# anhtu293/nndepth

Measured on AMD Instinct MI355X. Metric: stereo pairs/sec at 544x960, 32 iters (RAFT-Stereo), higher is better.
Workload: dtype f32 carried as 2 range-scaled fp16 pieces per operand (3 MFMA products, fp32 accumulate); 1 GPU; RAFT-Stereo base (ctx 64), 544x960, 32 iters, batch 1 per GPU, all 32 up_disp emitted; parallelism=single, launch=direct

## Files before the change

include/nndepth_amd.h:

```cpp
#ifndef NNDEPTH_AMD_H
#define NNDEPTH_AMD_H

#include <stddef.h>
#include <stdint.h>

#ifdef __cplusplus
extern "C" {
#endif

#define NND_VERSION 105

#define NND_FLAG_CALIBRATE 1
#define NND_FLAG_LAST_UPSAMPLE_ONLY 2

typedef enum {
    NND_OK = 0,
    NND_ERR_INVALID = -1,
    NND_ERR_HIP = -2,
    NND_ERR_UNSUPPORTED = -3,
    NND_ERR_NO_DEVICE = -4
} nnd_status;

int nnd_version(void);
const char* nnd_last_error(void);
// ... 187 lines not shown
                     void* stream);

int nnd_mbv3_depthwise(const float* x, const float* w, const float* bias, float* y, double* partial, int N, int C, int H, int W, int k,
                       int stride, int act, void* stream);
int64_t nnd_mbv3_se_partials(int N, int C, int H, int W);
int nnd_mbv3_se(float* y, const double* partial, const float* wr, const float* br, const float* we, const float* be, float* gate, int N,
                int C, int rd, int H, int W, void* stream);
int nnd_mbv3_stem(const float* x, const float* x1, int nsplit, const float* w, const float* bias, float* y, int N, int H, int W,
                  void* stream);
int64_t nnd_mbv3_pointwise_packed_floats(int Cout, int Cin, int k);
int nnd_mbv3_pointwise_pack(int Cout, int Cin, int k, const float* w, const float* bias, float* packed_host);
int nnd_mbv3_proj(const float* x, const float* w, const float* bias, float* y, int N, int Cin, int Cout, int H, int W, void* stream);
int nnd_mbv3_pointwise(int Cout, int Cin, int k, const float* packed_dev, const float* x, const float* residual, float* y, int N, int H,
                       int W, int act, void* stream);

#define NND_MIDAS_KEEP_PRE 1
typedef struct nnd_midas_desc {
    int32_t struct_size;
    int32_t feature_channels;
    int32_t flags;
} nnd_midas_desc;
int nnd_midas_num_tensors(const nnd_midas_desc* desc);
int64_t nnd_midas_packed_floats(const nnd_midas_desc* desc);
int64_t nnd_midas_workspace_floats(const nnd_midas_desc* desc, int B, int H, int W);
int64_t nnd_midas_workspace_offset(const nnd_midas_desc* desc, int which, int B, int H, int W);
int nnd_midas_pack(const nnd_midas_desc* desc, const float* const* tensors_host, float* packed_host);
int nnd_midas_forward(const nnd_midas_desc* desc, const float* packed_dev, const float* x, float* depth, float* workspace, int B, int H,
                      int W, void* stream);
int64_t nnd_midas_up2x_pw_packed_floats(int Cout, int Cin);
int nnd_midas_up2x_pw_pack(int Cout, int Cin, const float* w, const float* bias, float* packed_host);
int nnd_midas_up2x_pw(int Cout, int Cin, const float* packed_dev, const float* x, float* y, int N, int h, int w, void* stream);
int64_t nnd_midas_head_packed_floats(int C);
int nnd_midas_head_pack(int C, const float* w2, const float* b2, const float* w4, const float* b4, float* packed_host);
int nnd_midas_head(int C, const float* packed_dev, const float* t, float* depth, float* pre_relu, int N, int h, int w, void* stream);
int nnd_midas_conv_add(int Cout, int Cin, int k, const float* packed_dev, const float* x, const float* feat, float* y, int N, int H, int W,
                       void* stream);

int nnd_resize_normalize(const void* src, int src_is_u8_hwc, float* dst, int B, int C, int h, int w, int H, int W,
                         float sub, float div, void* stream);
int nnd_replicate_pad(const float* src, float* dst, int B, int C, int H, int W, int left, int right, int top, int bottom,
                      void* stream);

int64_t nnd_depth_eval_workspace_bytes(int B);
int nnd_depth_eval(const float* pred, const float* gt, const unsigned char* valid_mask, int B, int H, int W, float max_depth,
                   void* workspace, int64_t workspace_bytes, double* out, void* stream);
int nnd_depth_eval_accumulate(const double* metrics, double* sums, double* counts, void* stream);

int64_t nnd_midas_loss_workspace_bytes(int B, int H, int W);
int nnd_midas_loss(const float* pred, const float* target, const unsigned char* valid_mask, int B, int H, int W, int64_t pred_stride_b,
                   int64_t pred_stride_row, double trimmed_coef, double gradient_coef, void* workspace, int64_t workspace_bytes,
                   double* out, void* stream);
int nnd_midas_loss_accumulate(const double* values, double* sums, double* count, void* stream);

#define NND_STEREO_EVAL_MAX_OUTPUTS 64
#define NND_STEREO_EVAL_MAX_THRESHOLDS 8
typedef struct nnd_stereo_eval_output {
    const float* data;
    int32_t C, h, w;
    int32_t reserved;
    int64_t stride_b, stride_c, stride_row;
} nnd_stereo_eval_output;
typedef struct nnd_stereo_eval_desc {
    int32_t struct_size;
    int32_t flags;
    const float* gt;
    int32_t B, Cg, H, W;
    const unsigned char* mask;
    int32_t mask_h, mask_w;
    double gamma;
    float max_flow;
    int32_t n_above;
    float above[NND_STEREO_EVAL_MAX_THRESHOLDS];
    int32_t n_below;
    float below[NND_STEREO_EVAL_MAX_THRESHOLDS];
    int32_t num_outputs;
    nnd_stereo_eval_output outputs[NND_STEREO_EVAL_MAX_OUTPUTS];
} nnd_stereo_eval_desc;
int64_t nnd_stereo_eval_workspace_bytes(int num_outputs);
int nnd_stereo_eval(const nnd_stereo_eval_desc* desc, void* workspace, int64_t workspace_bytes, double* out, void* stream);
int nnd_stereo_eval_accumulate(const double* metrics, int n, double* sums, void* stream);
int nnd_min_pool_nearest(const float* gt, float* dst, int B, int C, int H, int W, int h, int w, void* stream);

int64_t nnd_view_range_workspace_bytes(int B);
int nnd_view_range(const float* data, const unsigned char* mask, int kind, int B, int C, int H, int W, void* workspace, float* range,
                   void* stream);
int nnd_colorize(const float* data, const unsigned char* mask, int kind, int B, int C, int H, int W, const float* range, int has_lo,
                 double lo, int has_hi, double hi, int reverse, const unsigned char* table, int N, unsigned char* out, void* stream);
int nnd_pool_abs(const float* src, float* dst, int64_t* indices, const unsigned char* mask, unsigned char* mask_out,
                 unsigned char* finite_out, int B, int C, int H, int W, int kh, int kw, int is_min, int negate, int rescale, float mul,
                 float div, void* stream);
int nnd_resize_bilinear(const void* src, int src_is_u8, float* dst, unsigned char* u8_out, int u8_mode, unsigned char* finite_out,
                        int planes, int h, int w, int H, int W, int align_corners, int rescale, float mul, float div, void* stream);
int nnd_depth_inverse(const float* src, float* dst, int64_t n, float eps, int has_max, float clip_max, int has_min, float clip_min,
                      void* stream);

int nnd_disparity_to_depth(const float* disp, int64_t disp_bstride, const unsigned char* mask_in, const float* cam, int cam_stride,
                           double baseline, int negative, float min_disp, int has_max, float max_depth, float* depth,
                           unsigned char* valid_out, int B, int H, int W, void* stream);
int nnd_depth_to_disparity(const float* depth, int64_t depth_bstride, const float* cam, int cam_stride, double baseline, int negative,
                           double eps, float* disp, int B, int H, int W, void* stream);
int nnd_depth_to_points(const float* depth, int64_t depth_bstride, const unsigned char* valid, const float* cam, int cam_stride,
                        float* points, int B, int H, int W, void* stream);
int64_t nnd_points_compact_workspace_bytes(int B, int H, int W);
int nnd_points_compact(const float* depth, int64_t depth_bstride, const unsigned char* valid, const float* cam, int cam_stride,
                       const float* features, int C, float* points, float* feats_out, int64_t* offsets, void* workspace,
                       int64_t workspace_bytes, int B, int H, int W, void* stream);
int nnd_lr_consistency(const float* disp_left, int64_t left_bstride, const float* disp_right, int64_t right_bstride, int left_negative,
                       int right_negative, int right_flipped, float threshold, unsigned char* occluded, float* err_out, int B, int H,
                       int W, void* stream);
int nnd_pair_both_views(const float* left, const float* right, float* frames1, float* frames2, int B, int C, int H, int W,
                        void* stream);

int64_t nnd_loftr_packed_floats(int d_model, int nhead);
int64_t nnd_loftr_workspace_floats(int d_model, int nhead, int N, int H, int W);
int nnd_loftr_pack(int d_model, int nhead, const float* const* tensors_host, float* packed_host);
int nnd_loftr_layer_forward(int d_model, int nhead, const float* packed_dev, const float* x, const float* source, float* out,
                            float* workspace, int N, int H, int W, void* stream);

int nnd_full_attention(const float* q, const float* k, const float* v, float* out, int N, int nhead, int L, int S, int64_t q_bs,
                       int64_t kv_bs, int64_t out_bs, void* stream);
int64_t nnd_loftr_full_workspace_floats(int d_model, int nhead, int N, int H, int W);
int nnd_loftr_full_layer_forward(int d_model, int nhead, const float* packed_dev, const float* x, const float* source, float* out,
                                 float* workspace, int N, int H, int W, void* stream);

typedef struct nnd_conv3d_desc {
    int32_t struct_size;
    int32_t Cout, Cin0, Cin1, stride;
    int32_t arithmetic;
    int32_t flags;
} nnd_conv3d_desc;
int64_t nnd_conv3d_packed_floats(const nnd_conv3d_desc* desc);
int nnd_conv3d_pack(const nnd_conv3d_desc* desc, const float* w_host, const float* bias_host, const float* bn_gamma,
                    const float* bn_beta, const float* bn_mean, const float* bn_var, float bn_eps, float* packed_host);
int nnd_conv3d_forward(const nnd_conv3d_desc* desc, const float* packed_dev, const float* x0, const float* x1, float* y,
                       int N, int D, int H, int W, float leaky_slope, void* stream);
int nnd_conv3d_calibration_finish(const nnd_conv3d_desc* desc, float* packed_dev, int32_t* status_dev, void* stream);
int nnd_conv3d_scale_slots(const nnd_conv3d_desc* desc, int64_t* offsets, int n);
const char* nnd_conv3d_scale_name(int which);
int nnd_volume_to_depth_major(const float* x, float* y, int N, int C, int D, int H, int W, void* stream);
int nnd_depth_major_to_volume(const float* x, float* y, int N, int C, int D, int H, int W, void* stream);
int nnd_volume_rows_to_depth_major(const float* x, float* y, int N, int C, int D, int H, int W, void* stream);
int nnd_depth_major_to_volume_rows(const float* x, float* y, int N, int C, int D, int H, int W, void* stream);
int nnd_volume_upsample2x(const float* x, float* y, int N, int C, int D, int H, int W, void* stream);
int nnd_volume_gate(float* vol, const float* logits, int N, int C, int D, int H, int W, void* stream);

int nnd_mask_upsample_forward(const float* packed_dev, const float* x, const float* flow, float* out,
                              int B, int Cin, int H, int W, int rate, void* stream);

int nnd_raft_stereo_refine(const nnd_update_block_desc* desc, const float* packed_dev,
                           const float* pyramid, int num_levels, int radius,
                           const float* net, const float* inp, const float* disp_init,
                           float* up_out, int64_t up_iter_stride, float* low_out, float* net_out,
                           float* workspace, int B, int H, int W, int rate, int iters, void* stream);
int nnd_raft_stereo_group_refine(const nnd_update_block_desc* desc, const float* packed_dev, const float* group_pyramid, int num_groups,
                                 int num_levels, int radius, const float* net, const float* inp, const float* disp_init, float* up_out,
                                 int64_t up_iter_stride, float* low_out, float* net_out, float* workspace, int B, int H, int W, int rate,
                                 int iters, void* stream);

int nnd_igev_refine_reads_interleaved(int num_groups, int num_levels, int radius);
int nnd_igev_stereo_refine(const nnd_update_block_desc* desc, const float* packed_dev,
                           const float* feat_pyramid, const float* geo_pyramid, const float* interleaved,
                           int num_groups, int num_levels, int radius,
                           const float* net, const float* inp, const float* disp_init,
                           float* up_out, int64_t up_iter_stride, float* low_out, float* net_out,
                           float* workspace, int B, int H, int W, int rate, int iters, void* stream);

int nnd_cre_stereo_refine(const nnd_update_block_desc* desc, const float* packed_dev,
                          const float* fmap1, const float* fmap2, int C, const float* extra_offset,
                          float* scratch, int64_t scratch_floats, const float* net, const float* inp, const float* flow_init,
                          float* up_out, int64_t up_iter_stride, float* low_out, float* net_out,
                          float* workspace, int B, int H, int W, int rate, int iters, void* stream);

int nnd_profile_conv(const nnd_update_block_desc* desc, const float* packed_dev, float* workspace,
                     int B, int H, int W, int which, int reps, void* stream,
                     float* ms_out, double* flops_out);
int nnd_profile_loop_conv(const nnd_update_block_desc* desc, const float* packed_dev, const float* pyramid,
                          int num_levels, int radius, const float* net, const float* inp, float* up_out,
                          float* workspace, int B, int H, int W, int rate, int iters, int which, void* stream,
                          float* ms_out);
int nnd_profile_loop_event_pair(const nnd_update_block_desc* desc, const float* packed_dev, const float* pyramid,
                                int num_levels, int radius, const float* net, const float* inp, float* up_out,
                                float* workspace, int B, int H, int W, int rate, int iters, int which, void* stream,
                                float* ms_out);
int nnd_profile_mfma_peak(int waves_per_simd, int iters, void* stream, float* scratch_dev, float* tflops_out);
int nnd_profile_mfma16_peak(int bf16, int waves_per_simd, float target_ms, void* stream, float* scratch_dev,
                            unsigned long long* clk_dev, float* tflops_out, float* ghz_out);
int nnd_num_convs(const nnd_update_block_desc* desc);
const char* nnd_conv_name(const nnd_update_block_desc* desc, int which);

#ifdef __cplusplus
}
#endif
#endif
```

nndepth_amd/_lib.py:

```python
import ctypes as C
import os

_HERE = os.path.dirname(os.path.abspath(__file__))
LIB_PATH = os.environ.get("NND_LIB") or os.path.join(_HERE, "libnndepth_amd.so")


class NndError(RuntimeError):
    pass


NND_FLAG_CALIBRATE = 1
NND_FLAG_LAST_UPSAMPLE_ONLY = 2


class _SizedDesc(C.Structure):

    def __init__(self, *args, **kwargs):
        super().__init__(C.sizeof(type(self)), *args, **kwargs)


class UpdateBlockDesc(_SizedDesc):
    _fields_ = [("struct_size", C.c_int32), ("hidden_dim", C.c_int32), ("context_dim", C.c_int32), ("cor_planes", C.c_int32),
                ("flow_channels", C.c_int32), ("mask_channels", C.c_int32), ("gru_kind", C.c_int32),
                ("arithmetic", C.c_int32), ("split_layers", C.c_int32), ("flags", C.c_int32)]


class ConvDesc(C.Structure):
    _fields_ = [("Cout", C.c_int32), ("Cin", C.c_int32), ("KH", C.c_int32), ("KW", C.c_int32), ("stride", C.c_int32)]


class Conv3dDesc(_SizedDesc):
    _fields_ = [("struct_size", C.c_int32), ("Cout", C.c_int32), ("Cin0", C.c_int32), ("Cin1", C.c_int32), ("stride", C.c_int32),
                ("arithmetic", C.c_int32), ("flags", C.c_int32)]


class EncoderDesc(_SizedDesc):
    _fields_ = [("struct_size", C.c_int32), ("output_dim", C.c_int32), ("norm", C.c_int32), ("cnet_dim", C.c_int32),
                ("arithmetic", C.c_int32), ("flags", C.c_int32)]


class RepViTDesc(_SizedDesc):
    _fields_ = [("struct_size", C.c_int32), ("stem_strides", C.c_int32 * 3), ("patch_size", C.c_int32),
                ("down_strides", C.c_int32 * 4), ("channels", C.c_int32 * 4), ("num_blocks", C.c_int32 * 4), ("mixer", C.c_int32 * 4),
                ("ffn_hidden", C.c_int32 * 4), ("cnet_dim", C.c_int32), ("fusion_dim", C.c_int32 * 2), ("flags", C.c_int32)]


class MobileNetV3Desc(_SizedDesc):
    _fields_ = [("struct_size", C.c_int32), ("fnet_dim", C.c_int32), ("cnet_dim", C.c_int32), ("flags", C.c_int32)]


NND_MIDAS_KEEP_PRE = 1


class MidasDesc(_SizedDesc):
    _fields_ = [("struct_size", C.c_int32), ("feature_channels", C.c_int32), ("flags", C.c_int32)]


NND_STEREO_EVAL_MAX_OUTPUTS = 64
NND_STEREO_EVAL_MAX_THRESHOLDS = 8


class StereoEvalOutput(C.Structure):
    _fields_ = [("data", C.c_void_p), ("C", C.c_int32), ("h", C.c_int32), ("w", C.c_int32), ("reserved", C.c_int32),
                ("stride_b", C.c_int64), ("stride_c", C.c_int64), ("stride_row", C.c_int64)]


class StereoEvalDesc(_SizedDesc):
    _fields_ = [("struct_size", C.c_int32), ("flags", C.c_int32), ("gt", C.c_void_p), ("B", C.c_int32), ("Cg", C.c_int32),
                ("H", C.c_int32), ("W", C.c_int32), ("mask", C.c_void_p), ("mask_h", C.c_int32), ("mask_w", C.c_int32),
                ("gamma", C.c_double), ("max_flow", C.c_float), ("n_above", C.c_int32),
                ("above", C.c_float * NND_STEREO_EVAL_MAX_THRESHOLDS), ("n_below", C.c_int32),
                ("below", C.c_float * NND_STEREO_EVAL_MAX_THRESHOLDS), ("num_outputs", C.c_int32),
                ("outputs", StereoEvalOutput * NND_STEREO_EVAL_MAX_OUTPUTS)]


_P = C.c_void_p
_I = C.c_int
SIGNATURES = {
    "nnd_version": (_I, []),
    "nnd_last_error": (C.c_char_p, []),
    "nnd_device_count": (_I, []),
    "nnd_corr1d_pyramid_layout": (_I, [_I, _I, _I, _I, C.POINTER(C.c_int64), C.POINTER(C.c_int32), C.POINTER(C.c_int64)]),
    "nnd_corr1d_build": (_I, [_P, _P, _P, _I, _I, _I, _I, _I, _P]),
    "nnd_corr1d_lookup": (_I, [_P, _P, _P, _I, _I, _I, _I, _I, _P]),
    "nnd_group_corr_build": (_I, [_P, _P, _P, _I, _I, _I, _I, _I, _I, _I, _P]),
    "nnd_group_corr_build_scaled": (_I, [_P, _P, _P, _I, _I, _I, _I, _I, _I, _I, C.c_float, _P]),
    "nnd_group_corr1d_lookup": (_I, [_P, _P, _P, _I, _I, _I, _I, _I, _I, _P]),
    "nnd_pyramid_from_level0": (_I, [_P, _I, _I, _I, _I, _P]),
    "nnd_igev_lookup": (_I, [_P, _P, _P, _P, _I, _I, _I, _I, _I, _I, _P]),
    "nnd_softargmin_disparity": (_I, [_P, _P, _I, _I, _I, _I, _P]),
    "nnd_igev_init_disparity": (_I, [_P, _P, _P, _P, _I, _I, _I, _I, _I, _P]),
    "nnd_igev_init_disparity_dev": (_I, [_P, _P, _P, _P, _I, _I, _I, _I, _I, _P]),
    "nnd_igev_init_disparity_supported": (_I, [_I, _I]),
    "nnd_igev_init_disparity_chunk": (_I, []),
    "nnd_igev_init_disparity_kernel": (C.c_char_p, [_I, _I, _I, _I, _I]),
    "nnd_convex_upsample": (_I, [_P, _P, _P, _I, _I, _I, _I, _I, _P]),
    "nnd_bilinear_sample": (_I, [_P, _P, _P, _I, _I, _I, _I, _I, _I, _P]),
    "nnd_agcl_corr_iter": (_I, [_P, _P, _P, _P, _P, _I, _I, _I, _I, _I, _P]),
    "nnd_agcl_corr_offset": (_I, [_P, _P, _P, _P, _P, _I, _I, _I, _I, _I, _P]),
    "nnd_agcl_corr_offset_nhwc": (_I, [_P, _P, _P, _P, _P, _I, _I, _I, _I, _I, _P]),
    "nnd_nchw_to_nhwc": (_I, [_P, _P, _I, _I, _I, _I, _P]),
    "nnd_update_block_num_tensors": (_I, [C.POINTER(UpdateBlockDesc)]),
    "nnd_update_block_packed_floats": (C.c_int64, [C.POINTER(UpdateBlockDesc)]),
    "nnd_update_block_pack": (_I, [C.POINTER(UpdateBlockDesc), C.POINTER(_P), _P]),
    "nnd_update_block_workspace_floats": (C.c_int64, [C.POINTER(UpdateBlockDesc), _I, _I, _I]),
    "nnd_update_block_forward": (_I, [C.POINTER(UpdateBlockDesc), _P, _P, _P, _P, _P, _P, _P, _P, _P, _I, _I, _I, _P]),
    "nnd_update_block_layer_forward": (_I, [C.POINTER(UpdateBlockDesc), _P, _I, _P, _P, _P, _I, _I, _I, _P]),
    "nnd_update_block_calibration_finish": (_I, [C.POINTER(UpdateBlockDesc), _P, _P, _P]),
    "nnd_update_block_scale_slots": (_I, [C.POINTER(UpdateBlockDesc), C.POINTER(C.c_int64), _I]),
    "nnd_conv2d_calibrate_ex": (_I, [_P, _P, _I, _I, _I, _I, _I, _I, _I, _I, _P, _P]),
    "nnd_conv2d_scale_slots_ex": (_I, [_I, _I, _I, _I, _I, C.POINTER(C.c_int64), _I]),
    "nnd_encoder_scale_slots": (_I, [C.POINTER(EncoderDesc), C.POINTER(C.c_int64), _I]),
    "nnd_encoder_scale_name": (C.c_char_p, [C.POINTER(EncoderDesc), _I]),
    "nnd_conv3d_scale_slots": (_I, [C.POINTER(Conv3dDesc), C.POINTER(C.c_int64), _I]),
    "nnd_conv3d_scale_name": (C.c_char_p, [_I]),
    "nnd_scales_read": (_I, [_P, C.POINTER(C.c_int64), _I, _P, _P, _I, _P]),
    "nnd_scales_write": (_I, [_P, C.POINTER(C.c_int64), _I, _P, _I, _P]),
    "nnd_nonfinite_flag": (_I, [_P, C.c_int64, _P, _P]),
    "nnd_encoder_forward2": (_I, [C.POINTER(EncoderDesc), _P, _P, _P, _I, _P, _P, _I, _P, _I, _I, _I, _P]),
    "nnd_pos_enc_sine_add": (_I, [_P, _P, _P, _P, _I, _I, _I, _I, _I, _P]),
    "nnd_encoder_calibration_finish": (_I, [C.POINTER(EncoderDesc), _P, _P, _P]),
    "nnd_conv3d_calibration_finish": (_I, [C.POINTER(Conv3dDesc), _P, _P, _P]),
    "nnd_conv2d_packed_floats": (C.c_int64, [_I, _I, _I, _I]),
    "nnd_conv2d_pack": (_I, [_P, _P, _I, _I, _I, _I, _P]),
    "nnd_conv2d_forward": (_I, [_P, _P, _P, _I, _I, _I, _I, _I, _I, _I, _I, _P]),
    "nnd_conv2d_packed_floats_ex": (C.c_int64, [_I, _I, _I, _I, _I]),
    "nnd_conv2d_pack_ex": (_I, [_P, _P, _I, _I, _I, _I, _I, _P]),
    "nnd_conv2d_forward_ex": (_I, [_P, _P, _P, _I, _I, _I, _I, _I, _I, _I, _I, _I, _P]),
    "nnd_conv2d_offset_forward": (_I, [_P, _P, _P, _I, _I, _I, _I, _I, _I, _I, C.c_float, _P]),
    "nnd_split_tanh_relu": (_I, [_P, _P, _P, _I, _I, _I, _I, _I, _P]),
    "nnd_avg_pool_2x_4x": (_I, [_P, _P, _P, _I, _I, _I, _I, _P]),
    "nnd_resize_bilinear_ac": (_I, [_P, _P, _I, _I, _I, _I, _I, _I, C.c_float, _P]),
    "nnd_resize_nearest_scaled": (_I, [_P, _P, _I, _I, _I, _I, _I, C.c_float, _P]),
    "nnd_mask_upsample_forward": (_I, [_P, _P, _P, _P, _I, _I, _I, _I, _I, _P]),
    "nnd_raft_stereo_refine": (_I, [C.POINTER(UpdateBlockDesc), _P, _P, _I, _I, _P, _P, _P, _P, C.c_int64, _P, _P, _P,
                                    _I, _I, _I, _I, _I, _P]),
    "nnd_raft_stereo_group_refine": (_I, [C.POINTER(UpdateBlockDesc), _P, _P, _I, _I, _I, _P, _P, _P, _P, C.c_int64, _P, _P, _P,
                                          _I, _I, _I, _I, _I, _P]),
    "nnd_igev_interleaved_floats": (C.c_int64, [_I, _I, _I, _I, _I]),
    "nnd_igev_interleave_pyramids": (_I, [_P, _P, _P, _I, _I, _I, _I, _I, _P]),
    "nnd_igev_interleave_level0_supported": (_I, [_I, _I, _I]),
    "nnd_igev_refine_reads_interleaved": (_I, [_I, _I, _I]),
    "nnd_igev_interleave_level0": (_I, [_P, _P, _P, _I, _I, _I, _I, _I, _P]),
    "nnd_igev_stereo_refine": (_I, [C.POINTER(UpdateBlockDesc), _P, _P, _P, _P, _I, _I, _I, _P, _P, _P, _P, C.c_int64, _P, _P, _P,
                                    _I, _I, _I, _I, _I, _P]),
    "nnd_cre_stereo_refine": (_I, [C.POINTER(UpdateBlockDesc), _P, _P, _P, _I, _P, _P, C.c_int64, _P, _P, _P, _P, C.c_int64, _P, _P, _P,
                                   _I, _I, _I, _I, _I, _P]),
    "nnd_conv_packed_floats": (C.c_int64, [C.POINTER(ConvDesc)]),
    "nnd_conv_pack": (_I, [C.POINTER(ConvDesc), _P, _P, _P, _P, _P, _P, C.c_float, _P]),
    "nnd_conv_forward": (_I, [C.POINTER(ConvDesc), _P, _P, _P, _P, _I, _I, _I, _I, _I, _P]),
    "nnd_conv_packed_floats_ex": (C.c_int64, [C.POINTER(ConvDesc), _I]),
    "nnd_conv_pack_ex": (_I, [C.POINTER(ConvDesc), _I, _P, _P, _P, _P, _P, _P, C.c_float, _P]),
    "nnd_conv_workspace_floats_ex": (C.c_int64, [C.POINTER(ConvDesc), _I, _I, _I]),
    "nnd_conv_forward_ex": (_I, [C.POINTER(ConvDesc), _I, _I, _P, _P, _P, _P, _P, _P, _I, _I, _I, _I, _I, _P]),
    "nnd_encoder_num_tensors": (_I, [C.POINTER(EncoderDesc)]),
    "nnd_encoder_packed_floats": (C.c_int64, [C.POINTER(EncoderDesc)]),
    "nnd_encoder_workspace_floats": (C.c_int64, [C.POINTER(EncoderDesc), _I, _I, _I]),
    "nnd_encoder_pack": (_I, [C.POINTER(EncoderDesc), C.POINTER(_P), C.c_float, _P]),
    "nnd_encoder_forward": (_I, [C.POINTER(EncoderDesc), _P, _P, _P, _P, _I, _P, _I, _I, _I, _P]),
    "nnd_repvit_num_tensors": (_I, [C.POINTER(RepViTDesc)]),
    "nnd_repvit_packed_floats": (C.c_int64, [C.POINTER(RepViTDesc)]),
    "nnd_repvit_workspace_floats": (C.c_int64, [C.POINTER(RepViTDesc), _I, _I, _I]),
    "nnd_repvit_pack": (_I, [C.POINTER(RepViTDesc), C.POINTER(_P), _P]),
    "nnd_repvit_forward": (_I, [C.POINTER(RepViTDesc), _P, _P, _P, _I, _P, _P, _P, _P, _P, _P, _P, _I, _I, _I, _P]),
    "nnd_repvit_depthwise": (_I, [_P, _P, _P, _P, _I, _I, _I, _I, _I, _I, _I, _P]),
    "nnd_repvit_stem": (_I, [_P, _P, _I, _P, _P, _P, _I, _I, _I, _I, _P]),
    "nnd_repvit_pointwise_packed_floats": (C.c_int64, [_I, _I, _I]),
    "nnd_repvit_pointwise_pack": (_I, [_I, _I, _I, _P, _P, _P, _P]),
    "nnd_repvit_pointwise": (_I, [_I, _I, _I, _P, _P, _P, _P, _I, _I, _I, _I, _P]),
    "nnd_repvit_linear_attention": (_I, [_P, _P, _I, _I, _I, _I, _P]),
    "nnd_repvit_upsample_add_relu": (_I, [_P, _P, _I, _I, _I, _I, _I, _I, _P]),
    "nnd_mbv3_num_tensors": (_I, [C.POINTER(MobileNetV3Desc)]),
    "nnd_mbv3_packed_floats": (C.c_int64, [C.POINTER(MobileNetV3Desc)]),
    "nnd_mbv3_workspace_floats": (C.c_int64, [C.POINTER(MobileNetV3Desc), _I, _I, _I]),
    "nnd_mbv3_pack": (_I, [C.POINTER(MobileNetV3Desc), C.POINTER(_P), _P]),
    "nnd_mbv3_forward": (_I, [C.POINTER(MobileNetV3Desc), _P, _P, _P, _P, _P, _P, _P, _P, _P, _P, _I, _I, _I, _P]),
    "nnd_mbv3_depthwise": (_I, [_P, _P, _P, _P, _P, _I, _I, _I, _I, _I, _I, _I, _P]),
    "nnd_mbv3_se_partials": (C.c_int64, [_I, _I, _I, _I]),
    "nnd_mbv3_se": (_I, [_P, _P, _P, _P, _P, _P, _P, _I, _I, _I, _I, _I, _P]),
    "nnd_mbv3_stem": (_I, [_P, _P, _I, _P, _P, _P, _I, _I, _I, _P]),
    "nnd_mbv3_proj": (_I, [_P, _P, _P, _P, _I, _I, _I, _I, _I, _P]),
    "nnd_mbv3_pointwise_packed_floats": (C.c_int64, [_I, _I, _I]),
    "nnd_mbv3_pointwise_pack": (_I, [_I, _I, _I, _P, _P, _P]),
    "nnd_mbv3_pointwise": (_I, [_I, _I, _I, _P, _P, _P, _P, _I, _I, _I, _I, _P]),
    "nnd_midas_num_tensors": (_I, [C.POINTER(MidasDesc)]),
    "nnd_midas_packed_floats": (C.c_int64, [C.POINTER(MidasDesc)]),
    "nnd_midas_workspace_floats": (C.c_int64, [C.POINTER(MidasDesc), _I, _I, _I]),
    "nnd_midas_workspace_offset": (C.c_int64, [C.POINTER(MidasDesc), _I, _I, _I, _I]),
    "nnd_midas_pack": (_I, [C.POINTER(MidasDesc), C.POINTER(_P), _P]),
    "nnd_midas_forward": (_I, [C.POINTER(MidasDesc), _P, _P, _P, _P, _I, _I, _I, _P]),
    "nnd_midas_up2x_pw_packed_floats": (C.c_int64, [_I, _I]),
    "nnd_midas_up2x_pw_pack": (_I, [_I, _I, _P, _P, _P]),
    "nnd_midas_up2x_pw": (_I, [_I, _I, _P, _P, _P, _I, _I, _I, _P]),
    "nnd_midas_head_packed_floats": (C.c_int64, [_I]),
    "nnd_midas_head_pack": (_I, [_I, _P, _P, _P, _P, _P]),
    "nnd_midas_head": (_I, [_I, _P, _P, _P, _P, _I, _I, _I, _P]),
    "nnd_midas_conv_add": (_I, [_I, _I, _I, _P, _P, _P, _P, _I, _I, _I, _P]),
    "nnd_resize_normalize": (_I, [_P, _I, _P, _I, _I, _I, _I, _I, _I, C.c_float, C.c_float, _P]),
    "nnd_replicate_pad": (_I, [_P, _P, _I, _I, _I, _I, _I, _I, _I, _I, _P]),
    "nnd_depth_eval_workspace_bytes": (C.c_int64, [_I]),
    "nnd_depth_eval": (_I, [_P, _P, _P, _I, _I, _I, C.c_float, _P, C.c_int64, _P, _P]),
    "nnd_depth_eval_accumulate": (_I, [_P, _P, _P, _P]),
    "nnd_midas_loss_workspace_bytes": (C.c_int64, [_I, _I, _I]),
    "nnd_midas_loss": (_I, [_P, _P, _P, _I, _I, _I, C.c_int64, C.c_int64, C.c_double, C.c_double, _P, C.c_int64, _P, _P]),
    "nnd_midas_loss_accumulate": (_I, [_P, _P, _P, _P]),
    "nnd_stereo_eval_workspace_bytes": (C.c_int64, [_I]),
    "nnd_stereo_eval": (_I, [C.POINTER(StereoEvalDesc), _P, C.c_int64, _P, _P]),
    "nnd_stereo_eval_accumulate": (_I, [_P, _I, _P, _P]),
    "nnd_min_pool_nearest": (_I, [_P, _P, _I, _I, _I, _I, _I, _I, _P]),
    "nnd_view_range_workspace_bytes": (C.c_int64, [_I]),
    "nnd_view_range": (_I, [_P, _P, _I, _I, _I, _I, _I, _P, _P, _P]),
    "nnd_colorize": (_I, [_P, _P, _I, _I, _I, _I, _I, _P, _I, C.c_double, _I, C.c_double, _I, _P, _I, _P, _P]),
    "nnd_pool_abs": (_I, [_P, _P, _P, _P, _P, _P, _I, _I, _I, _I, _I, _I, _I, _I, _I, C.c_float, C.c_float, _P]),
    "nnd_resize_bilinear": (_I, [_P, _I, _P, _P, _I, _P, _I, _I, _I, _I, _I, _I, _I, C.c_float, C.c_float, _P]),
    "nnd_depth_inverse": (_I, [_P, _P, C.c_int64, C.c_float, _I, C.c_float, _I, C.c_float, _P]),
    "nnd_disparity_to_depth": (_I, [_P, C.c_int64, _P, _P, _I, C.c_double, _I, C.c_float, _I, C.c_float, _P, _P, _I, _I, _I, _P]),
    "nnd_depth_to_disparity": (_I, [_P, C.c_int64, _P, _I, C.c_double, _I, C.c_double, _P, _I, _I, _I, _P]),
    "nnd_depth_to_points": (_I, [_P, C.c_int64, _P, _P, _I, _P, _I, _I, _I, _P]),
    "nnd_points_compact_workspace_bytes": (C.c_int64, [_I, _I, _I]),
    "nnd_points_compact": (_I, [_P, C.c_int64, _P, _P, _I, _P, _I, _P, _P, _P, _P, C.c_int64, _I, _I, _I, _P]),
    "nnd_lr_consistency": (_I, [_P, C.c_int64, _P, C.c_int64, _I, _I, _I, C.c_float, _P, _P, _I, _I, _I, _P]),
    "nnd_pair_both_views": (_I, [_P, _P, _P, _P, _I, _I, _I, _I, _P]),
    "nnd_loftr_packed_floats": (C.c_int64, [_I, _I]),
    "nnd_loftr_workspace_floats": (C.c_int64, [_I, _I, _I, _I, _I]),
    "nnd_loftr_pack": (_I, [_I, _I, C.POINTER(_P), _P]),
    "nnd_loftr_layer_forward": (_I, [_I, _I, _P, _P, _P, _P, _P, _I, _I, _I, _P]),
    "nnd_full_attention": (_I, [_P, _P, _P, _P, _I, _I, _I, _I, C.c_int64, C.c_int64, C.c_int64, _P]),
    "nnd_loftr_full_workspace_floats": (C.c_int64, [_I, _I, _I, _I, _I]),
    "nnd_loftr_full_layer_forward": (_I, [_I, _I, _P, _P, _P, _P, _P, _I, _I, _I, _P]),
    "nnd_conv3d_packed_floats": (C.c_int64, [C.POINTER(Conv3dDesc)]),
    "nnd_conv3d_pack": (_I, [C.POINTER(Conv3dDesc), _P, _P, _P, _P, _P, _P, C.c_float, _P]),
    "nnd_conv3d_forward": (_I, [C.POINTER(Conv3dDesc), _P, _P, _P, _P, _I, _I, _I, _I, C.c_float, _P]),
    "nnd_volume_to_depth_major": (_I, [_P, _P, _I, _I, _I, _I, _I, _P]),
    "nnd_depth_major_to_volume": (_I, [_P, _P, _I, _I, _I, _I, _I, _P]),
    "nnd_volume_rows_to_depth_major": (_I, [_P, _P, _I, _I, _I, _I, _I, _P]),
    "nnd_depth_major_to_volume_rows": (_I, [_P, _P, _I, _I, _I, _I, _I, _P]),
    "nnd_volume_upsample2x": (_I, [_P, _P, _I, _I, _I, _I, _I, _P]),
    "nnd_volume_gate": (_I, [_P, _P, _I, _I, _I, _I, _I, _P]),
    "nnd_profile_conv": (_I, [C.POINTER(UpdateBlockDesc), _P, _P, _I, _I, _I, _I, _I, _P, C.POINTER(C.c_float),
                              C.POINTER(C.c_double)]),
    "nnd_profile_loop_conv": (_I, [C.POINTER(UpdateBlockDesc), _P, _P, _I, _I, _P, _P, _P, _P, _I, _I, _I, _I, _I, _I, _P,
                                   C.POINTER(C.c_float)]),
    "nnd_profile_loop_event_pair": (_I, [C.POINTER(UpdateBlockDesc), _P, _P, _I, _I, _P, _P, _P, _P, _I, _I, _I, _I, _I, _I, _P,
                                         C.POINTER(C.c_float)]),
    "nnd_profile_mfma_peak": (_I, [_I, _I, _P, _P, C.POINTER(C.c_float)]),
    "nnd_profile_mfma16_peak": (_I, [_I, _I, C.c_float, _P, _P, _P, C.POINTER(C.c_float), C.POINTER(C.c_float)]),
    "nnd_reload_switches": (_I, []),
    "nnd_num_convs": (_I, [C.POINTER(UpdateBlockDesc)]),
    "nnd_conv_name": (C.c_char_p, [C.POINTER(UpdateBlockDesc), _I]),
}


def _load():
    if not os.path.exists(LIB_PATH):
        raise NndError(
            f"{LIB_PATH} not found: build it with `make -C nndepth_amd/csrc` (or __graft_entry__.build()). "
            "nndepth_amd has no CPU / PyTorch fallback.")
    lib = C.CDLL(LIB_PATH)
    for name, (res, args) in SIGNATURES.items():
        fn = getattr(lib, name)
        fn.restype = res
        fn.argtypes = args
    return lib


lib = _load()


def check(rc: int, what: str = ""):
    if rc != 0:
        msg = lib.nnd_last_error().decode("utf-8", "replace")
        raise NndError(f"{what or 'nndepth_amd'} failed (status {rc}): {msg}")
```

nndepth_amd/csrc/cascade.hip:

```cpp
#include "common.h"

#include <cmath>
#include "conv_epilogue.h"

namespace nnd {

__global__ void __launch_bounds__(256) split_tanh_relu_kernel(const float* __restrict__ x, float* __restrict__ net, float* __restrict__ inp,
                                                              int Cn, int Ci, long HW, long total) {
    const long idx = (long)blockIdx.x * 256 + threadIdx.x;
    if (idx >= total) return;
    const long per = (long)(Cn + Ci) * HW;
    const long b = idx / per, rem = idx - b * per;
    const float v = x[idx];
    if (rem < (long)Cn * HW) net[b * Cn * HW + rem] = tanhf_(v);
    else inp[b * Ci * HW + (rem - (long)Cn * HW)] = relu_nan(v);
}

__global__ void __launch_bounds__(256) avg_pool_2x_4x_kernel(const float* __restrict__ x, float* __restrict__ o2, float* __restrict__ o4,
                                                             int H, int W, int H2, int W2, int H4, int W4) {
    const int q4x = (W2 + 1) / 2, q4y = (H2 + 1) / 2;
    const long cell = (long)blockIdx.x * 256 + threadIdx.x;
    if (cell >= (long)q4x * q4y) return;
    const int cy = (int)(cell / q4x), cx = (int)(cell - (long)cy * q4x);
    const long plane = blockIdx.y;
    const float* src = x + plane * H * W;
#pragma unroll
    for (int iy = 0; iy < 2; ++iy)
#pragma unroll
        for (int ix = 0; ix < 2; ++ix) {
            const int y2 = cy * 2 + iy, x2 = cx * 2 + ix;
            if (y2 < H2 && x2 < W2) {
                const float* p = src + (long)(2 * y2) * W + 2 * x2;
                o2[plane * H2 * W2 + (long)y2 * W2 + x2] = (((p[0] + p[1]) + p[W]) + p[W + 1]) * 0.25f;
            }
        }
    if (cy < H4 && cx < W4) {
        const float* p = src + (long)(4 * cy) * W + 4 * cx;
        float s = 0.f;
#pragma unroll
        for (int iy = 0; iy < 4; ++iy)
#pragma unroll
            for (int ix = 0; ix < 4; ++ix) s += p[(long)iy * W + ix];
        o4[plane * H4 * W4 + (long)cy * W4 + cx] = s * 0.0625f;
    }
}

__global__ void __launch_bounds__(256) pos_enc_sine_add_kernel(const float* __restrict__ x0, const float* __restrict__ x1, float* __restrict__ y0,
                                                               float* __restrict__ y1, int C, int H, int W, float rate) {
    const long HW = (long)H * W;
    const long pix = (long)blockIdx.x * 256 + threadIdx.x;
    if (pix >= HW) return;
    const int c = blockIdx.y % C;
    const long off = (long)blockIdx.y * HW + pix;
    const float pos = (float)(((c & 2) ? (int)(pix / W) : (int)(pix % W)) + 1);
    const float arg = pos * expf((float)(2 * (c >> 2)) * rate);
    const float pe = (c & 1) ? cosf(arg) : sinf(arg);
    y0[off] = x0[off] + pe;
    if (x1) y1[off] = x1[off] + pe;
}

__global__ void __launch_bounds__(256) resize_bilinear_ac_kernel(const float* __restrict__ x, float* __restrict__ y, int h, int w, int H,
                                                                 int W, float mul) {
    const long idx = (long)blockIdx.x * 256 + threadIdx.x;
    if (idx >= (long)H * W) return;
    const long plane = blockIdx.y;
    const int oy = (int)(idx / W), ox = (int)(idx - (long)oy * W);
    const float sy = H > 1 ? (float)(h - 1) / (float)(H - 1) : 0.f, sx = W > 1 ? (float)(w - 1) / (float)(W - 1) : 0.f;
    const float ry = sy * (float)oy, rx = sx * (float)ox;
    const int y0 = min((int)ry, h - 1), x0 = min((int)rx, w - 1);
    const int y1 = y0 + (y0 < h - 1 ? 1 : 0), x1 = x0 + (x0 < w - 1 ? 1 : 0);
    const float ly1 = ry - (float)y0, lx1 = rx - (float)x0, ly0 = 1.f - ly1, lx0 = 1.f - lx1;
    const float* s = x + plane * h * w;
    const float t0 = fmaf(s[(long)y0 * w + x1], lx1, s[(long)y0 * w + x0] * lx0);
    const float t1 = fmaf(s[(long)y1 * w + x1], lx1, s[(long)y1 * w + x0] * lx0);
    y[plane * H * W + idx] = mul * fmaf(t1, ly1, t0 * ly0);
}

template <int V>
__global__ void __launch_bounds__(256) resize_nearest_scaled_kernel(const float* __restrict__ x, float* __restrict__ y, int h, int w, int H,
                                                                    int W, float mul, long total) {
    const long idx = (long)blockIdx.x * 256 + threadIdx.x;
    if (idx >= total) return;
    const int WV = W / V;
    const long row = idx / WV;
    const int ox = (int)(idx - row * WV) * V, oy = (int)(row % H);
    const long n = row / H;
    const float sy = (float)h / (float)H, sx = (float)w / (float)W;
    const float* src = x + (n * h + min((int)floorf((float)oy * sy), h - 1)) * w;
    float v[V];
#pragma unroll
    for (int i = 0; i < V; ++i) v[i] = mul * src[min((int)floorf((float)(ox + i) * sx), w - 1)];
    float* dst = y + row * W + ox;
    if (V == 4) *reinterpret_cast<float4*>(dst) = make_float4(v[0], v[1], v[2], v[3]);
    else dst[0] = v[0];
}

}

using namespace nnd;

extern "C" {

int nnd_split_tanh_relu(const float* x, float* net, float* inp, int B, int Cnet, int Cinp, int H, int W, void* stream) {
    NND_REQUIRE(x && net && inp && B > 0 && Cnet > 0 && Cinp > 0 && H > 0 && W > 0, "split_tanh_relu: bad argument");
    const long total = (long)B * (Cnet + Cinp) * H * W;
    hipLaunchKernelGGL(split_tanh_relu_kernel, dim3((unsigned)cdiv64(total, 256)), dim3(256), 0, (hipStream_t)stream, x, net, inp, Cnet,
                       Cinp, (long)H * W, total);
    NND_LAUNCH_CHECK();
    return NND_OK;
}

int nnd_avg_pool_2x_4x(const float* x, float* out2, float* out4, int N, int C, int H, int W, void* stream) {
    NND_REQUIRE(x && out2 && out4 && N > 0 && C > 0 && H >= 4 && W >= 4, "avg_pool_2x_4x: bad argument (H, W >= 4)");
    const int H2 = H / 2, W2 = W / 2, H4 = H / 4, W4 = W / 4;
    const long cells = (long)((W2 + 1) / 2) * ((H2 + 1) / 2);
    hipLaunchKernelGGL(avg_pool_2x_4x_kernel, dim3((unsigned)cdiv64(cells, 256), (unsigned)(N * C)), dim3(256), 0, (hipStream_t)stream, x,
                       out2, out4, H, W, H2, W2, H4, W4);
    NND_LAUNCH_CHECK();
    return NND_OK;
}

int nnd_pos_enc_sine_add(const float* x0, const float* x1, float* y0, float* y1, int N, int C, int H, int W, int temp_bug_fix,
                         void* stream) {
    NND_REQUIRE(x0 && y0 && (!x1 == !y1) && N > 0 && C > 0 && C % 4 == 0 && H > 0 && W > 0, "pos_enc_sine_add: bad argument (C %% 4 == 0)");
    const double q = -std::log(10000.0) / (temp_bug_fix ? (double)(C / 2) : (double)C);
    const float rate = (float)(temp_bug_fix ? q : std::floor(q / 2.0));
    hipLaunchKernelGGL(pos_enc_sine_add_kernel, dim3((unsigned)cdiv64((long)H * W, 256), (unsigned)(N * C)), dim3(256), 0, (hipStream_t)stream,
                       x0, x1, y0, y1, C, H, W, rate);
    NND_LAUNCH_CHECK();
    return NND_OK;
}

int nnd_resize_bilinear_ac(const float* x, float* y, int N, int C, int h, int w, int H, int W, float mul, void* stream) {
    NND_REQUIRE(x && y && N > 0 && C > 0 && h > 0 && w > 0 && H > 0 && W > 0, "resize_bilinear_ac: bad argument");
    hipLaunchKernelGGL(resize_bilinear_ac_kernel, dim3((unsigned)cdiv64((long)H * W, 256), (unsigned)(N * C)), dim3(256), 0,
                       (hipStream_t)stream, x, y, h, w, H, W, mul);
    NND_LAUNCH_CHECK();
    return NND_OK;
}

int nnd_resize_nearest_scaled(const float* x, float* y, int N, int h, int w, int H, int W, float mul, void* stream) {
    NND_REQUIRE(x && y, "resize_nearest_scaled: null pointer");
    NND_REQUIRE(N > 0 && h > 0 && w > 0 && H > 0 && W > 0, "resize_nearest_scaled: bad shape");
    NND_REQUIRE(H % h == 0 && W % w == 0, "resize_nearest_scaled: %dx%d -> %dx%d is not an integer ratio in both axes", h, w, H, W);
    const int V = (W & 3) == 0 ? 4 : 1;
    const long total = (long)N * H * (W / V);
    NND_REQUIRE(cdiv64(total, 256) < (1L << 31), "resize_nearest_scaled: grid of %ld workgroups too large (max 2^31 - 1)",
                (long)cdiv64(total, 256));
    if (V == 4)
        hipLaunchKernelGGL(resize_nearest_scaled_kernel<4>, dim3((unsigned)cdiv64(total, 256)), dim3(256), 0, (hipStream_t)stream, x, y, h, w,
                           H, W, mul, total);
    else
        hipLaunchKernelGGL(resize_nearest_scaled_kernel<1>, dim3((unsigned)cdiv64(total, 256)), dim3(256), 0, (hipStream_t)stream, x, y, h, w,
                           H, W, mul, total);
    NND_LAUNCH_CHECK();
    return NND_OK;
}

}
```

nndepth_amd/csrc/common.h:

```cpp
#pragma once
#include <hip/hip_runtime.h>
#include <atomic>
#include <cstdarg>
#include <cstdio>
#include "../../include/nndepth_amd.h"
#include "split_arith.h"

namespace nnd {

void set_error(const char* fmt, ...);

#define NND_HIP_CHECK(expr)                                                              \
    do {                                                                                 \
        hipError_t _e = (expr);                                                          \
        if (_e != hipSuccess) {                                                          \
            nnd::set_error("%s failed: %s (%s:%d)", #expr, hipGetErrorString(_e), __FILE__, __LINE__); \
            return NND_ERR_HIP;                                                          \
        }                                                                                \
    } while (0)

#define NND_LAUNCH_CHECK()                                                               \
    do {                                                                                 \
        hipError_t _e = hipGetLastError();                                               \
        if (_e != hipSuccess) {                                                          \
            nnd::set_error("kernel launch failed: %s (%s:%d)", hipGetErrorString(_e), __FILE__, __LINE__); \
            return NND_ERR_HIP;                                                          \
        }                                                                                \
    } while (0)

#define NND_REQUIRE(cond, ...)                                                           \
    do {                                                                                 \
        if (!(cond)) {                                                                   \
            nnd::set_error(__VA_ARGS__);                                                 \
            return NND_ERR_INVALID;                                                      \
        }                                                                                \
    } while (0)

#define NND_TRY(x)                           \
    do {                                     \
        if ((rc = (x)) != NND_OK) return rc; \
    } while (0)

template <class Desc>
static inline int check_desc(const Desc* d, unsigned allowed_flags, const char* name) {
    NND_REQUIRE(d, "%s: null descriptor", name);
    NND_REQUIRE(d->struct_size == (int32_t)sizeof(Desc), "%s: descriptor of %d bytes, this library expects %d (struct_size)", name,
                d->struct_size, (int)sizeof(Desc));
    NND_REQUIRE((d->flags & ~allowed_flags) == 0, "%s: unknown flags 0x%x", name, d->flags);
    return NND_OK;
}

struct Switches {
    bool no_fused_upsample, no_fused_lookup, no_fused_flow_branch, no_c4, agcl_v1, no_thin3d, corr_build_v1, corr_build_no_ksplit, igev_squeeze_v1, igev_squeeze_walk, no_folded_flow_head, no_conv1x1_stream,
        conv_verbose, debug_sync;
    int split_ny, split_ks, split_p;
    bool split_no_fast;
    bool no_merged_fb_lookup;
    int conv_p, conv_ks, conv_wco;
    int agcl_pb;
    bool lds_poison_on;
    unsigned lds_poison;
    int lds_slack;
    bool enc_no_c4;
    bool no_slab3d;
    int slab3d_rounds;
    bool no_fused_enc_block;
};
const Switches& switches();

static inline int raise_lds_limit(const void* kern, std::atomic<unsigned>& done, int bytes = 160 * 1024) {
    int dev = 0;
    NND_HIP_CHECK(hipGetDevice(&dev));
    const unsigned bit = 1u << (dev & 31);
    if (!(done.load(std::memory_order_relaxed) & bit)) {
        NND_HIP_CHECK(hipFuncSetAttribute(kern, hipFuncAttributeMaxDynamicSharedMemorySize, bytes));
        done.fetch_or(bit, std::memory_order_relaxed);
    }
    return NND_OK;
}

bool calibrating();
struct CalibScope {
    explicit CalibScope(bool on);
    ~CalibScope();
    CalibScope(const CalibScope&) = delete;
    CalibScope& operator=(const CalibScope&) = delete;
    bool on;
};
struct Act;
struct Lay;
int calib_amax_act(const Act& a, const Lay& lay, int B, int H, int W, const float* tail, hipStream_t s);
int calib_amax_flat(const float* x, int64_t n, const float* tail, hipStream_t s);
int calib_finish(float* blob, const int64_t* tail_offs, int n, int32_t* status_dev, hipStream_t s);

#ifdef __HIPCC__
__device__ __forceinline__ void fmac_scalar(float& acc, float a, float b) { asm("v_fmac_f32 %0, %1, %2" : "+v"(acc) : "v"(a), "v"(b)); }

__device__ __forceinline__ float relu_nan(float v) { return __builtin_elementwise_maximum(v, 0.f); }
__device__ __forceinline__ float clamp_nan(float v, float lo, float hi) {
    return __builtin_elementwise_minimum(__builtin_elementwise_maximum(v, lo), hi);
}
#endif

int to_tiled(const float* src, float* dst, int64_t dbs, int B, int C, int H, int W, hipStream_t s, int c0 = 0, bool c4 = false);
int from_tiled(const float* src, int64_t sbs, float* dst, int B, int C, int H, int W, hipStream_t s, int c0 = 0, bool c4 = false);

static inline int cdiv(int a, int b) { return (a + b - 1) / b; }
static inline int64_t cdiv64(int64_t a, int64_t b) { return (a + b - 1) / b; }

enum ConvEpilogue {
    EPI_LINEAR = 0,
    EPI_RELU = 1,
    EPI_GRU_ZR = 2,
    EPI_GRU_Q = 3,
    EPI_SCALE = 4,
    EPI_AFFINE = 5,
    EPI_SIGMOID_RANGE = 6,
    EPI_GELU = 7,
    EPI_HSWISH = 8
};

struct ConvLayer {
    int KH, KW, Cin, Cout, CI_T;
    int stride = 1;
    int arith = 0;
    bool range_scaled() const { return split_range_scaled(arith); }
    int64_t s_off = -1;
    int nchunks;
    int ncb;
    int64_t w_off, b_off;
    int64_t w_floats() const {
        return arith ? (int64_t)ncb * nchunks * KH * KW * arith * 256
                     : (int64_t)ncb * nchunks * KH * KW * CI_T * 32;
    }
    int64_t b_floats() const { return (int64_t)ncb * 32 + (range_scaled() ? 4 : 0); }
    double flops(int B, int H, int W) const { return 2.0 * B * H * W * (double)Cout * Cin * KH * KW; }
    int64_t tail_off() const { return b_off + (int64_t)ncb * 32; }
};

struct Act {
    float* ptr;
    int64_t bstride;
    int C;
};

struct ConvIO {
    Act src0, src1;
    Act out0, out1;
    Act aux0, aux1;
    Act bmap;
    int hidden = 0;
    float scale = 1.f;
    int Hin = 0, Win = 0;
    int flags = 0;
    bool src_tiled = false;
    bool dst_tiled = false;
    bool src_c4 = false;
    bool dst_c4 = false;
    int cout_need = 0;
    int force_ks = 0;
};

static inline bool conv_shape_built(int KH, int KW) { return (KH == 1 && (KW == 1 || KW == 5)) || (KW == 1 && KH == 5) || (KH == 3 && KW == 3); }

int conv_ci_t(int KH, int KW, int Cin, int stride = 1, int Cout = 0);

int launch_conv(const ConvLayer& L, const float* blob, const ConvIO& io, int epi,
                int B, int H, int W, hipStream_t stream);

void pack_conv(const ConvLayer& L, int nparts, const float* const* w, const float* const* b,
               const int* cout, float* blob, const int* ci_map = nullptr, int cin_src = 0);

bool conv_split_supported(int KH, int KW, int Cin, int stride, int arith, int Cout = 0);
int launch_conv_split(const ConvLayer& L, const float* blob, const ConvIO& io, int epi, int B, int H, int W, hipStream_t stream);
bool conv_split_no_split_k(const ConvLayer& L, int B, int H, int W);
bool flow_branch_supported(const ConvLayer& f2, int fc);
int launch_flow_branch(const ConvLayer& f2, const float* blob, const float* w7t, const float* b7, const float* flow, int64_t fbs,
                       int fc, const ConvIO& io, int B, int H, int W, hipStream_t stream);
void pack_conv_split(const ConvLayer& L, int nparts, const float* const* w, const float* const* b, const int* cout, float* blob,
                     const int* ci_map, int cin_src);

bool enc_block_supported(const ConvLayer& c1, const ConvLayer& c2, const ConvLayer& ds);
int enc_block_launch(const ConvLayer& c1, const float* blob1, const ConvLayer& c2, const float* blob2, const ConvLayer& ds, const float* blobd,
                     const float* x, float* out, int N, int Hx, int Wx, hipStream_t stream);

bool thin3d_supported(int Cout, int stride);
bool slab3d_supported(int Cout, int C0, int C1, int stride, int arith);
int64_t slab3d_packed_floats(int Cout, int Ct, int stride);
void slab3d_pack(int Cout, int Ct, int stride, const float* w, const float* scale, const float* shift, float* out);
int slab3d_forward(int Cout, int C0, int C1, int stride, const float* packed, const float* x0, const float* x1, float* y, int N, int D,
                   int H, int W, float slope, hipStream_t s);
int64_t thin3d_packed_floats(int Cout, int Ct);
void thin3d_pack(int Cout, int Ct, const float* w, const float* scale, const float* shift, float* out);
int thin3d_forward(int Cout, int C0, int C1, int stride, const float* packed, const float* x0, const float* x1, float* y, int N, int D,
                   int H, int W, float slope, hipStream_t s);

int corr1d_lookup_launch(const float* pyr, const float* coords, float* out, int B, int H, int W, int num_levels,
                         int radius, hipStream_t stream, bool tiled);
int group_lookup_flat_launch(const float* pyr, const float* coords, float* out, int B, int G, int H, int W, int num_levels, int radius,
                             hipStream_t stream, bool tiled);
int igev_lookup_launch(const float* feat_pyramid, const float* geo_pyramid, const float* coords, float* out, int B, int G, int H,
                       int W, int num_levels, int radius, hipStream_t stream, bool tiled);
int convex_upsample_launch(const float* flow, const float* mask, float* out, int B, int C, int H, int W, int rate,
                           hipStream_t stream, bool tiled);

int agcl_iter_launch(const float* f1, const float* f2, const float* flow, float* warped, float* out, int N, int C, int H,
                     int W, int small_patch, hipStream_t s, bool tiled);
int agcl_offset_launch(const float* f1, const float* f2, const float* flow, const float* extra, float* out, int N, int C, int H,
                       int W, int small_patch, hipStream_t s, bool tiled);
int agcl_check(const char* what, int N, int C, int H, int W);
bool agcl_offset_cl_supported(int C);
int agcl_offset_cl_launch(const float* f1c, const float* f2c, const float* flow, const float* extra, float* out, int N, int C,
                          int H, int W, int small_patch, hipStream_t s, bool tiled);
int nchw_to_nhwc_launch(const float* in, float* out, int N, int C, int P, hipStream_t s);
int lookup_convc1_launch(const float* pyr, const float* geo, int G, const float* coords, const ConvLayer& L, const float* blob,
                         float* c1, int64_t c1_bs, int B, int H, int W, int num_levels, int radius, hipStream_t stream, bool c1_c4);
bool flow_branch_lookup_supported(int arith);
int flow_branch_lookup_launch(const ConvLayer& f2, const float* blob, const float* w7t, const float* b7, const float* flow, int64_t fbs,
                              int fc, const ConvIO& io, const float* pyr, const float* coords, const ConvLayer& Lc1, float* c1,
                              int64_t c1_bs, int B, int H, int W, int num_levels, int radius, hipStream_t stream, bool c1_c4);
bool igev_lookup_convc1_il_supported(int G, int num_levels, int radius);
int igev_lookup_convc1_il_launch(const float* il, int G, const float* coords, const ConvLayer& L, const float* blob, float* c1,
                                 int64_t c1_bs, int B, int H, int W, int num_levels, int radius, hipStream_t stream, bool c1_c4);
struct MaskUpFlowHead {
    const float* x;
    long xbs;
    int hid;
    const float* w;
    const float* bias;
    const float* coords_in;
    float *coords_out, *flow_out, *delta_out;
    float* hx_flow;
    long hx_bs;
    int hx_pm;
    int absolute;
};

bool mask_upsample_supported(int rate, int cin, int flow_channels);
bool mask_upsample_fold_supported(const ConvLayer& L, int hid);
int mask_upsample_launch(const ConvLayer& L, const float* blob, const float* x, int64_t xbs, const float* flow, float* out,
                         int B, int H, int W, int rate, hipStream_t stream, bool tiled, int flow_channels = 1, bool x_c4 = false,
                         const MaskUpFlowHead* fh = nullptr);

}
```

nndepth_amd/csrc/conv_split.hip:

```cpp
#include "conv_launch.h"
#include "conv_split_kernel.h"
#include "flow_branch.h"

#include <atomic>
#include <cmath>
#include <cstdlib>
#include <cstring>

namespace nnd {

namespace {
uint16_t f16_rn(float x) {
    const _Float16 h = (_Float16)x;
    uint16_t u;
    memcpy(&u, &h, 2);
    return u;
}
float f16_to_f(uint16_t u) {
    _Float16 h;
    memcpy(&h, &u, 2);
    return (float)h;
}
uint16_t bf16_rn(float x) {
    uint32_t u;
// ... 8 lines not shown
    memcpy(&f, &u, 4);
    return f;
}

bool pick_split(const ConvLayer& L, int c0, int c1, int B, int H, int W, bool fast_ok, SplitCfg* out) {
    const int NS = L.arith, STR = L.stride;
    const int npos = split_patch(L.KH, L.KW, NS, STR).NPOS;
    const size_t subb = split_patch(L.KH, L.KW, NS, STR).SUBB;
    int tiles_x, ntiles = split_tiles(H, W, &tiles_x);
    int force_ny = switches().split_ny, force_ks = switches().split_ks, force_p = switches().split_p;
    const bool forced = force_ny > 0 || force_ks > 0 || force_p > 0;
    const long px_wgs2 = (long)cdiv(ntiles, 2) * B;
    bool rule = false;
    if (L.nchunks <= 4 && !forced && L.ncb <= SPLIT_MAX_WAVES) {
        force_ny = 1;
        while (force_ny < L.ncb && (L.ncb % force_ny != 0 || L.ncb / force_ny > 4)) ++force_ny;
        force_ks = 1;
        force_p = 2;
        rule = true;
    }
    bool try_ks2 = false;
    if (!rule && px_wgs2 >= 448 && !forced) {
        rule = true;
        force_ks = 1;
        force_ny = 1;
        force_p = 2;
        const int max_wco = L.nchunks >= 16 ? 4 : SPLIT_MAX_WAVES;
        while (force_ny < L.ncb && (L.ncb % force_ny != 0 || L.ncb / force_ny > max_wco)) ++force_ny;
        try_ks2 = px_wgs2 * force_ny * (L.ncb / force_ny) < 256 * SPLIT_MAX_WAVES / 2;
    }
    auto search = [&](int f_ny, int f_ks, int f_p) {
        double best = 1e30;
        bool found = false;
        for (int P : {2, 3, 4}) {
            if ((f_p > 0 && P != f_p) || (f_p <= 0 && P != 2)) continue;
            const long px_wgs = (long)cdiv(ntiles, P) * B;
            for (int ny = 1; ny <= L.ncb; ++ny) {
                if (L.ncb % ny != 0 || (f_ny > 0 && ny != f_ny)) continue;
                const int wco = L.ncb / ny;
                for (int ks : {1, 2, 4}) {
                    if (f_ks > 0 && ks != f_ks) continue;
                    const int waves = wco * ks;
                    if (waves > SPLIT_MAX_WAVES || ks > L.nchunks) continue;
                    if (c1 > 0 && c0 % (ks * 16) != 0) continue;
                    const bool fast = fast_ok && L.nchunks % ks == 0;
                    if (P > 2) continue;
                    if (STR == 2 && !fast) continue;
                    const int nu = split_staging_units(P, npos, ks, waves);
                    if (nu > 4 || (P == 3 && nu > 3)) continue;
                    size_t lds = (size_t)2 * ks * P * subb;
                    const size_t red = ks > 1 ? (size_t)waves * P * 4096 : 0;
                    if (red > lds) lds = red;
                    if (lds > 160 * 1024) continue;
                    const int max_waves = P > 2 ? 8 : SPLIT_MAX_WAVES;
                    int wg_per_cu = (int)((160 * 1024) / lds);
                    if (wg_per_cu > max_waves / waves) wg_per_cu = max_waves / waves;
                    if (wg_per_cu < 1) wg_per_cu = 1;
                    const double rounds = std::ceil((double)px_wgs * ny / (256.0 * wg_per_cu));
                    const double simd_waves = std::ceil(waves * wg_per_cu / 4.0);
                    double t = rounds * simd_waves * cdiv(L.nchunks, ks) * P / 2.0;
                    t *= 1.0 + 0.03 * (ks - 1);
                    t *= 1.0 + 0.02 * (4 - (wco < 4 ? wco : 4));
                    if (nu > 2 && P == 2) t *= 1.2;
                    if (t < best) {
                        best = t;
                        *out = {ny, wco, ks, P, ntiles, tiles_x, split_nu_variant(nu), fast, lds, STR};
                        found = true;
                    }
                }
            }
        }
        return found;
    };
    if (try_ks2 && search(force_ny, 2, force_p)) return true;
    if (search(force_ny, force_ks, force_p)) return true;
    return rule && search(-1, -1, -1);
}

bool restrict_split(const ConvLayer& L, int cout_need, SplitCfg* cfg) {
    const int npos = split_patch(L.KH, L.KW, L.arith, L.stride).NPOS;
    auto units = [&](int wco) { return split_staging_units(cfg->P, npos, cfg->ks, wco * cfg->ks); };
    if (!conv_restrict_cout(L, cout_need, &cfg->ny, &cfg->wco, [&](int wco) { return cfg->P == 2 && units(wco) <= 4; })) return false;
    cfg->nu = split_nu_variant(units(cfg->wco));
    return true;
}

bool split_fast_ok(const ConvLayer& L) { return !switches().split_no_fast || L.stride == 2; }
bool plan_split(const ConvLayer& L, const ConvIO& io, int B, int H, int W, SplitCfg* cfg) {
    if (!pick_split(L, io.src0.C, io.src1.C, B, H, W, split_fast_ok(L), cfg)) return false;
    cfg->restricted = restrict_split(L, io.cout_need, cfg);
    cfg->grid = dim3(cdiv(cfg->ntiles, cfg->P), cfg->ny, B), cfg->block = dim3(64 * cfg->wco * cfg->ks);
    return true;
}

void print_split_plan(const ConvLayer& L, const ConvIO& io, const SplitCfg& cfg) {
    fprintf(stderr, "[nnd] conv_split %dx%d Cin=%d Cout=%d pieces=%d: ny=%d, wco=%d, ks=%d, P=%d, nu=%d%s, grid %ux%ux%u, lds %zu B%s%s\n", L.KH,
            L.KW, L.Cin, L.Cout, L.arith, cfg.ny, cfg.wco, cfg.ks, cfg.P, cfg.nu, cfg.fast ? ", fast" : "", cfg.grid.x, cfg.grid.y, cfg.grid.z, cfg.lds,
            io.cout_need > 0 ? (cfg.restricted ? ", restricted to the wanted output channels" : ", whole layer (not restrictable)") : "",
            L.stride == 2 ? ", stride 2" : "");
}
}

bool conv_split_no_split_k(const ConvLayer& L, int B, int H, int W) {
    SplitCfg cfg;
    return pick_split(L, L.Cin, 0, B, H, W, split_fast_ok(L), &cfg) && cfg.ks == 1;
}

extern template int launch_split_ns<1>(const ConvArgs&, const SplitCfg&, int, int, hipStream_t);
extern template int launch_split_ns<2>(const ConvArgs&, const SplitCfg&, int, int, hipStream_t);
extern template int launch_split_ns<3>(const ConvArgs&, const SplitCfg&, int, int, hipStream_t);

bool conv_split_supported(int KH, int KW, int Cin, int stride, int arith, int Cout) {
    if ((arith != 3 && arith != 2 && arith != 1) || (stride != 1 && stride != 2) || Cin % 16 != 0) return false;
    if (stride == 2) return ((KH == 3 && KW == 3) || (KH == 1 && KW == 1)) && Cout >= 96;
    return conv_shape_built(KH, KW);
}

int launch_conv_split(const ConvLayer& L, const float* blob, const ConvIO& io, int epi, int B, int H, int W, hipStream_t stream) {
    int rc, Hin, Win;
    NND_REQUIRE(conv_split_supported(L.KH, L.KW, L.Cin, L.stride, L.arith, L.Cout), "conv_split: %dx%d Cin=%d Cout=%d stride %d arith %d not built",
                L.KH, L.KW, L.Cin, L.Cout, L.stride, L.arith);
    NND_TRY(conv_check_io("conv_split", L, io, epi, H, W, &Hin, &Win));
    NND_REQUIRE(L.CI_T == 16 && L.nchunks * 16 == L.Cin, "conv_split: layer was not planned for 16-channel chunks");
    NND_REQUIRE(L.stride == 1 || io.src1.C == 0, "conv_split: stride 2 is built for one source");
    NND_REQUIRE((long)(L.Cin + 64) * tiled_plane(Hin, Win) < (1L << 31), "conv_split: plane offsets exceed 32 bits");
    SplitCfg cfg;
    NND_REQUIRE(plan_split(L, io, B, H, W, &cfg),
                "conv_split: no configuration for %dx%d Cin=%d (%d+%d) Cout=%d stride %d (NND_SPLIT_CFG ny=%d ks=%d P=%d%s)", L.KH, L.KW,
                L.Cin, io.src0.C, io.src1.C, L.Cout, L.stride, switches().split_ny, switches().split_ks, switches().split_p,
                split_fast_ok(L) ? "" : ", NND_SPLIT_NO_FAST");
    ConvArgs a;
    conv_fill_args(L, blob, io, epi, H, W, Hin, Win, &a);
    a.tiles_x = cfg.tiles_x; a.wco = cfg.wco; a.ks = cfg.ks; a.npos = cfg.ntiles;
#ifdef NND_DBG_STAMPS
    {
        static std::atomic<int> launches{0};
        static const int only = getenv("NND_DBG_STAMP_LAUNCH") ? atoi(getenv("NND_DBG_STAMP_LAUNCH")) : -1;
        const int idx = launches.fetch_add(1);
        a.dbg_stamp = only < 0 || idx == only;
    }
#endif
    if (calibrating() && split_range_scaled(L.arith))
        for (const Act* src : {&io.src0, &io.src1}) NND_TRY(calib_amax_act(*src, a.ls, B, Hin, Win, blob + L.tail_off(), stream));
    if (switches().conv_verbose) print_split_plan(L, io, cfg);
    rc = L.arith == 3   ? launch_split_ns<3>(a, cfg, L.KH, L.KW, stream)
         : L.arith == 2 ? launch_split_ns<2>(a, cfg, L.KH, L.KW, stream)
                        : launch_split_ns<1>(a, cfg, L.KH, L.KW, stream);
    NND_REQUIRE(rc != NND_ERR_UNSUPPORTED, "conv_split: shape %dx%d P=%d nu=%d %s is not instantiated", L.KH, L.KW, cfg.P, cfg.nu, cfg.fast ? "fast" : "generic");
    if (rc != NND_OK) return rc;
    NND_LAUNCH_CHECK();
    return NND_OK;
}

void pack_conv_split(const ConvLayer& L, int nparts, const float* const* w, const float* const* bvec, const int* cout, float* blob,
                     const int* ci_map, int cin_src) {
    if (!ci_map) cin_src = L.Cin;
    const int NT = L.KH * L.KW, NS = L.arith;
    uint16_t* wp = reinterpret_cast<uint16_t*>(blob + L.w_off);
    float* bp = blob + L.b_off;
    memset(wp, 0, sizeof(float) * L.w_floats());
    memset(bp, 0, sizeof(float) * L.b_floats());
    const bool f16 = split_range_scaled(NS);
    float wscale = 1.f;
    if (f16) {
        float wmax = 0.f;
        for (int part = 0; part < nparts; ++part)
            for (int col = 0; col < cout[part]; ++col)
                for (int ci = 0; ci < L.Cin; ++ci)
                    for (int t = 0; t < NT; ++t) {
                        const float v = std::fabs(w[part][((size_t)col * cin_src + (ci_map ? ci_map[ci] : ci)) * NT + t]);
                        if (std::isfinite(v) && v > wmax) wmax = v;
                    }
        int e = 0;
        if (wmax > 0.f) std::frexp(wmax, &e);
        const int s = wmax > 0.f ? 14 - e : 0;
        wscale = std::ldexp(1.f, s);
        float* tail = bp + L.ncb * 32;
        tail[SPLIT_TAIL_OSCALE] = std::ldexp(1.f, -(s + SPLIT_F16_XSHIFT));
        tail[SPLIT_TAIL_XSCALE] = std::ldexp(1.f, SPLIT_F16_XSHIFT);
        tail[SPLIT_TAIL_AMAX] = 0.f;
        tail[SPLIT_TAIL_WSINV] = std::ldexp(1.f, -s);
    }
    int co0 = 0;
    for (int part = 0; part < nparts; ++part) {
        for (int col = 0; col < cout[part]; ++col) {
            const int co = co0 + col, cb = co / 32, i = co % 32;
            bp[co] = bvec[part] ? bvec[part][col] : 0.f;
            for (int ci = 0; ci < L.Cin; ++ci) {
                const int chunk = ci / 16, cl = ci % 16, h = cl / 8, j = cl % 8, lane = h * 32 + i;
                for (int t = 0; t < NT; ++t) {
                    float res = w[part][((size_t)col * cin_src + (ci_map ? ci_map[ci] : ci)) * NT + t] * wscale;
                    for (int s = 0; s < NS; ++s) {
                        const uint16_t piece = f16 ? f16_rn(res) : bf16_rn(res);
                        res -= f16 ? f16_to_f(piece) : bf16_to_f(piece);
                        wp[((((((size_t)cb * L.nchunks + chunk) * NT + t) * NS + s) * 64 + lane) * 8) + j] = piece;
                    }
                }
            }
        }
        co0 += cout[part];
    }
}

template <int FC, int NS>
static int launch_fb(const FlowBranchArgs& a, dim3 grid, dim3 block, hipStream_t stream) {
    auto kern = flow_branch_kernel<FC, NS>;
    static std::atomic<unsigned> raised{0};
    if (int rc = raise_lds_limit(reinterpret_cast<const void*>(kern), raised)) return rc;
    const size_t lds = (size_t)(fb_lds_bytes<FC, NS>()) + switches().lds_slack;
    hipLaunchKernelGGL(kern, grid, block, lds, stream, a);
    return NND_OK;
}

bool flow_branch_supported(const ConvLayer& f2, int fc) {
    return (f2.arith == 3 || f2.arith == 2 || f2.arith == 1) && f2.KH == 3 && f2.KW == 3 && f2.Cin == FB_C1 && f2.Cout == 64 && f2.stride == 1 && (fc == 1 || fc == 2);
}

int make_flow_branch_args(const ConvLayer& f2, const float* blob, const float* w7t, const float* b7, const float* flow, int64_t fbs,
                          int fc, const ConvIO& io, int B, int H, int W, FlowBranchArgs* out) {
    NND_REQUIRE(flow_branch_supported(f2, fc), "flow_branch: built for convf1 7x7 (1 or 2 -> 128) + convf2 3x3 (128 -> 64) in split arithmetic");
    NND_REQUIRE(io.dst_tiled && f2.CI_T == 16 && f2.nchunks == FB_NCH, "flow_branch: tile-major destination, 16-channel chunks");
    NND_REQUIRE((long)(fc + 64) * tiled_plane(H, W) < (1L << 31), "flow_branch: plane offsets exceed 32 bits");
    FlowBranchArgs& a = *out;
    memset(&a, 0, sizeof(a));
    a.flow = flow; a.fbs = (long)fbs; a.w7t = w7t; a.b7 = b7;
    a.lf = make_lay(H, W, true);
    a.c.wpk = blob + f2.w_off;
    a.c.bias = blob + f2.b_off;
    a.c.out0 = io.out0.ptr; a.c.obs0 = io.out0.bstride;
    a.c.ld = make_lay(H, W, true, io.dst_c4);
    a.c.H = H; a.c.W = W; a.c.Hin = H; a.c.Win = W; a.c.Cout = f2.Cout; a.c.epi = EPI_RELU;
    a.c.npos = split_tiles(H, W, &a.c.tiles_x);
    a.c.scale = 1.f;
    return NND_OK;
}

int launch_flow_branch(const ConvLayer& f2, const float* blob, const float* w7t, const float* b7, const float* flow, int64_t fbs,
                       int fc, const ConvIO& io, int B, int H, int W, hipStream_t stream) {
    FlowBranchArgs a;
    int rc0 = make_flow_branch_args(f2, blob, w7t, b7, flow, fbs, fc, io, B, H, W, &a);
    if (rc0 != NND_OK) return rc0;
    dim3 grid(a.c.npos, 1, B), block(512);
    int rc;
    if (fc == 1) rc = f2.arith == 3 ? launch_fb<1, 3>(a, grid, block, stream) : f2.arith == 2 ? launch_fb<1, 2>(a, grid, block, stream) : launch_fb<1, 1>(a, grid, block, stream);
    else rc = f2.arith == 3 ? launch_fb<2, 3>(a, grid, block, stream) : f2.arith == 2 ? launch_fb<2, 2>(a, grid, block, stream) : launch_fb<2, 1>(a, grid, block, stream);
    if (rc != NND_OK) return rc;
    NND_LAUNCH_CHECK();
    return NND_OK;
}

#ifdef NND_DBG_STAMPS
extern "C" int nnd_debug_read_fb_stamps(unsigned long long* host, int n) {
    return hipMemcpyFromSymbol(host, HIP_SYMBOL(g_fb_stamps), sizeof(unsigned long long) * n) == hipSuccess ? 0 : -1;
}
#endif
}
```

nndepth_amd/csrc/conv_split_kernel.h:

```cpp
#pragma once
#include "common.h"
#include "conv_epilogue.h"
#include "layout.h"
#include "split_arith.h"

#include <type_traits>
#include <utility>

namespace nnd {

#ifndef NND_SPLIT_BSLOTS
#define NND_SPLIT_BSLOTS 2
#endif

#ifdef NND_DBG_STAMPS
static __device__ unsigned long long g_split_stamps[4096 * 8];
#define NND_SSTAMP(i)                                                                                  \
    do {                                                                                               \
        if (threadIdx.x == 0 && a.dbg_stamp) {                                                         \
            const unsigned lin_ = blockIdx.x + gridDim.x * (blockIdx.y + gridDim.y * blockIdx.z);      \
            if (lin_ < 4096) g_split_stamps[lin_ * 8 + (i)] = __builtin_amdgcn_s_memrealtime();        \
        }                                                                                              \
    } while (0)
#define NND_SCLOCK(i)                                                                                  \
    do {                                                                                               \
        if (threadIdx.x == 0 && a.dbg_stamp) {                                                         \
            const unsigned lin_ = blockIdx.x + gridDim.x * (blockIdx.y + gridDim.y * blockIdx.z);      \
            if (lin_ < 4096) g_split_stamps[lin_ * 8 + (i)] = __builtin_amdgcn_s_memtime();            \
        }                                                                                              \
    } while (0)
#else
#define NND_SSTAMP(i)
#define NND_SCLOCK(i)
#endif
#if defined(NND_DBG_STAMPS) && defined(NND_DBG_PROLOGUE)
#undef NND_SCLOCK
#define NND_SCLOCK(i)
#define NND_PSTAMP(i) NND_SSTAMP(i)
#else
#define NND_PSTAMP(i)
#endif

__host__ __device__ constexpr int split_pos_bytes(int NS) { return NS * 32 + 16; }
__host__ __device__ constexpr int split_row_bytes(int PC, int NS) {
    int rb = (PC * split_pos_bytes(NS) + 15) / 16;
    while (rb % 16 != 8) ++rb;
    return rb * 16;
}

__device__ __forceinline__ int lane_pixel(int l31) {
    const bool g0 = (l31 < 4) || (l31 >= 12 && l31 < 16) || (l31 >= 20 && l31 < 28);
    const int idx = g0 ? (l31 < 4 ? l31 : (l31 < 16 ? l31 - 8 : l31 - 12)) : (l31 < 12 ? l31 - 4 : (l31 < 20 ? l31 - 8 : l31 - 16));
    return (g0 ? 0 : 16) + idx;
}

__host__ __device__ constexpr int split_gcd(int a, int b) { return b == 0 ? a : split_gcd(b, a % b); }

template <int N, typename F, int... I>
__device__ __forceinline__ void split_static_for_impl(F&& f, std::integer_sequence<int, I...>) {
    (f(std::integral_constant<int, I>{}), ...);
}
template <int N, typename F>
__device__ __forceinline__ void split_static_for(F&& f) {
    split_static_for_impl<N>(static_cast<F&&>(f), std::make_integer_sequence<int, N>{});
}

struct SplitPatch {
    int PRI, PCI, NPH, PRP, PCP, NPOS, PS, ROWB, PHB, SUBB;
};
__host__ __device__ constexpr SplitPatch split_patch(int KH, int KW, int NS, int STR) {
    const int PRI = 3 * STR + KH, PCI = 7 * STR + KW;
    const int NPH = STR == 1 ? 1 : (KH * KW == 1 ? 1 : 4);
    const int PRP = STR == 1 ? PRI : (KH == 1 ? 4 : (PRI + 1) / 2);
    const int PCP = STR == 1 ? PCI : (KW == 1 ? 8 : (PCI + 1) / 2);
    const int NPOS = STR == 1 ? PRI * PCI : (KH * KW == 1 ? 32 : PRI * PCI);
    const int ROWB = split_row_bytes(PCP, NS);
    return {PRI, PCI, NPH, PRP, PCP, NPOS, split_pos_bytes(NS), ROWB, PRP * ROWB, NPH * PRP * ROWB};
}
template <int KH, int KW, int NS, int STR>
struct SplitGeom {
    static constexpr SplitPatch G = split_patch(KH, KW, NS, STR);
    static constexpr int PRI = G.PRI, PCI = G.PCI, NPH = G.NPH, PRP = G.PRP, PCP = G.PCP, NPOS = G.NPOS;
    static constexpr int PS = G.PS, ROWB = G.ROWB, PHB = G.PHB, SUBB = G.SUBB;
};
__host__ __device__ constexpr int split_staging_units(int P, int npos, int ks, int waves) { return (P * npos * 2 * ks + 64 * waves - 1) / (64 * waves); }
__host__ __device__ constexpr int split_nu_variant(int nu) { return nu <= 2 ? 2 : 4; }

__host__ __device__ constexpr int split_pipe_spu(int nunit, int nsteps, int ul) {
    int v = 1;
    while (v < nsteps && nunit - 1 - (nsteps + v - 1) / v < ul + 3) ++v;
    return v;
}
template <int NT, int P, int NU>
struct SplitPipe {
    static constexpr int NUNIT = NT * P, NSTEPS = NU * 4 + 3, UL = 1;
    static constexpr int SPU = split_pipe_spu(NUNIT, NSTEPS, UL), U0 = NUNIT - 1 - (NSTEPS + SPU - 1) / SPU;
    static constexpr bool ON = NT >= 5 && P == 2;
};

template <int KH, int KW, int NS, int P, int NU, bool FAST, bool SRC4, int AD_, int MAXT, int STR = 1>
__global__ void __launch_bounds__(MAXT) conv_split_kernel(ConvArgs a) {
    static_assert(STR == 1 || (FAST && (KH * KW == 9 || KH * KW == 1)), "stride 2: 3x3 / 1x1, FAST regime");
    using Geo = SplitGeom<KH, KW, NS, STR>;
    constexpr int NT = KH * KW, PH = KH / 2, PW = KW / 2;
    constexpr int PC = Geo::PCI, NPOS = Geo::NPOS;
#ifndef NND_SPLIT_NO_PIPE
    constexpr bool PIPE = FAST && SRC4 && SplitPipe<NT, P, NU>::ON && NS != 1;
#else
    constexpr bool PIPE = false;
#endif
    constexpr int PS = Geo::PS, ROWB = Geo::ROWB, SUBB = Geo::SUBB, PHB = Geo::PHB;
    extern __shared__ __attribute__((aligned(16))) unsigned char lds_raw[];
    NND_SSTAMP(0);

    const int tid = threadIdx.x, lane = tid & 63, nthreads = blockDim.x;
    const int wave = __builtin_amdgcn_readfirstlane(tid >> 6);
    const int wco = a.wco, ks = a.ks;
    const int cbi = wave % wco, kj = wave / wco;
    const int h2 = lane >> 5, l31 = lane & 31;
    const int pxl = lane_pixel(l31), r = pxl >> 3, c = pxl & 7;
    const int cb = blockIdx.y * wco + cbi;
    const bool active = cb * 32 < a.Cout;
    const int b = blockIdx.z;
    const int Hin = a.Hin, Win = a.Win;
    const long SP = a.ls.plane;
    const int SCH = ks * 16;
    float oscale = 1.f, xscale = 1.f;
    if constexpr (split_range_scaled(NS)) {
        const float* tail = a.bias + (((a.Cout + 31) >> 5) << 5);
        oscale = tail[SPLIT_TAIL_OSCALE];
        xscale = tail[SPLIT_TAIL_XSCALE];
    }

    int ty0[P], tx0[P];
#pragma unroll
    for (int pp = 0; pp < P; ++pp) {
        const int t = blockIdx.x * P + pp;
        const bool valid = t < a.npos;
        ty0[pp] = valid ? (t / a.tiles_x) * 4 : (1 << 20);
        tx0[pp] = valid ? (t % a.tiles_x) * 8 : 0;
    }

    const int nunits = P * NPOS * 2 * ks;
    int goff[NU], loff[NU], cho[NU];
    bool inimg[NU], own[NU];
#pragma unroll
    for (int i = 0; i < NU; ++i) {
        const int u = PIPE ? min(tid + i * nthreads, nunits - 1) : tid + i * nthreads;
        own[i] = u < nunits;
        const int pos = u % NPOS, rest = u / NPOS;
        const int pp = rest % P, oct = rest / P;
        int pr, pc, lpos;
        if constexpr (STR == 1) {
            pr = pos / PC;
            pc = pos - pr * PC;
            lpos = pr * ROWB + pc * PS;
        } else if constexpr (KH * KW == 1) {
            pr = (pos >> 3) * 2;
            pc = (pos & 7) * 2;
            lpos = (pos >> 3) * ROWB + (pos & 7) * PS;
        } else {
            pr = pos / PC;
            pc = pos - pr * PC;
            lpos = ((pr & 1) * 2 + (pc & 1)) * PHB + (pr >> 1) * ROWB + (pc >> 1) * PS;
        }
        int gy = 0, gx = 0;
#pragma unroll
        for (int q = 0; q < P; ++q)
            if (q == pp) {
                gy = ty0[q] * STR + pr - PH;
                gx = tx0[q] * STR + pc - PW;
            }
        inimg[i] = own[i] && gy >= 0 && gy < Hin && gx >= 0 && gx < Win;
        goff[i] = inimg[i] ? (int)pix_off(a.ls, gy, gx) : 0;
        loff[i] = (oct >> 1) * (P * SUBB) + pp * SUBB + lpos + (oct & 1) * 16;
        cho[i] = oct * 8;
        if constexpr (FAST) goff[i] = inimg[i] ? cho[i] * (int)SP + goff[i] : 0;
        if constexpr (PIPE) goff[i] = cho[i] * (int)SP + (int)pix_off(a.ls, min(max(gy, 0), Hin - 1), min(max(gx, 0), Win - 1));
    }

    NND_PSTAMP(5);
    f32x16 acc[P];
#pragma unroll
    for (int pp = 0; pp < P; ++pp)
#pragma unroll
        for (int i = 0; i < 16; ++i) acc[pp][i] = 0.f;

    const int nchunks = a.nchunks;
    const int nsuper = (nchunks + ks - 1) / ks;
    const uint4* wbase = reinterpret_cast<const uint4*>(a.wpk) + (size_t)(active ? cb : 0) * nchunks * (NT * NS * 64) + lane;
    float stage[NU][8];

    auto chunk_src = [&](int K, const float*& src, int& climit) {
        const int cbase = K * SCH;
        if constexpr (FAST) {
            const bool first = cbase < a.c0;
            const float* s0 = a.src0 + b * a.bs0 + (long)cbase * SP;
            const float* s1 = a.src1 + b * a.bs1 + (long)(cbase - a.c0) * SP;
            src = first ? s0 : s1;
            climit = SCH;
        } else if (cbase < a.c0) {
            src = a.src0 + b * a.bs0 + (long)cbase * SP;
            climit = a.c0 - cbase;
        } else {
            const int cc = cbase - a.c0;
            src = a.src1 + b * a.bs1 + (long)cc * SP;
            climit = a.c1 - cc;
        }
    };
    const bool c4s = FAST ? SRC4 : a.ls.ci == 4;
    auto load_unit = [&](int K, int i) {
        const float* src;
        int climit;
        chunk_src(K, src, climit);
        if constexpr (FAST && SRC4) {
#pragma unroll
            for (int g = 0; g < 2; ++g) {
                const float4 t = *reinterpret_cast<const float4*>(src + (unsigned)(goff[i] + ((PIPE || inimg[i]) ? 4 * g * (int)SP : 0)));
                stage[i][4 * g] = t.x; stage[i][4 * g + 1] = t.y; stage[i][4 * g + 2] = t.z; stage[i][4 * g + 3] = t.w;
            }
        } else if constexpr (FAST) {
            const int step = inimg[i] ? (int)SP : 0;
#pragma unroll
            for (int j = 0; j < 8; ++j) stage[i][j] = src[(unsigned)(goff[i] + j * step)];
        } else if (c4s) {
#pragma unroll
            for (int g = 0; g < 2; ++g) {
                const int ci = cho[i] + 4 * g;
                const float4 t = *reinterpret_cast<const float4*>(src + ((inimg[i] && ci < climit) ? (unsigned)(ci * (int)SP + goff[i]) : 0u));
                stage[i][4 * g] = t.x; stage[i][4 * g + 1] = t.y; stage[i][4 * g + 2] = t.z; stage[i][4 * g + 3] = t.w;
            }
        } else {
#pragma unroll
            for (int j = 0; j < 8; ++j) {
                const int ci = cho[i] + j;
                stage[i][j] = src[(inimg[i] && ci < climit) ? (unsigned)(ci * (int)SP + goff[i]) : 0u];
            }
        }
    };
    auto store_unit = [&](int K, int i) {
        const float* src;
        int climit;
        chunk_src(K, src, climit);
        unsigned char* buf = lds_raw + (K & 1) * (ks * P * SUBB);
        float v[8];
#pragma unroll
        for (int j = 0; j < 8; ++j) v[j] = (inimg[i] && (FAST || cho[i] + j < climit)) ? stage[i][j] : 0.f;
        uint4 pieces[NS];
        split_pieces<NS>(v, pieces, xscale);
        if (own[i]) {
#pragma unroll
            for (int s = 0; s < NS; ++s) *reinterpret_cast<uint4*>(buf + loff[i] + s * 32) = pieces[s];
        }
    };
    auto load_x = [&](int K) {
#pragma unroll
        for (int i = 0; i < NU; ++i) load_unit(K, i);
    };
    auto store_x = [&](int K) {
#pragma unroll
        for (int i = 0; i < NU; ++i) store_unit(K, i);
    };
    auto a_ptr = [&](int K) {
        int ch = K * ks + kj;
        ch = ch < nchunks ? ch : 0;
        return wbase + (size_t)ch * (NT * NS * 64);
    };
    auto load_a = [&](uint4 (&dst)[NS], const uint4* wc, int t) {
#pragma unroll
        for (int s = 0; s < NS; ++s) dst[s] = wc[(t * NS + s) * 64];
    };

    const int lane_base = kj * (P * SUBB) + r * ROWB + c * PS + h2 * 16;

// ... 153 lines not shown
                if (mine && acc[0][0] == 123.f)
#endif
                    split_mfma_step<NS>(ac, bq[u % NSLOT], acc[pp]);
#ifndef NND_SPLIT_NO_PIN
                if constexpr (FAST) __builtin_amdgcn_sched_barrier(0);
#endif
            }
        }
#ifndef NND_SPLIT_NO_STAGE
        if (more) store_x(K + 1);
#endif
        __syncthreads();
    };
    auto chunk = [&](int K, auto par_c) {
        if constexpr (FAST) {
            chunk_body(K, par_c, std::true_type{});
        } else {
            if (K * ks + kj < nchunks) chunk_body(K, par_c, std::true_type{});
            else chunk_body(K, par_c, std::false_type{});
        }
    };
    constexpr int STEP = NT % NA, PERIOD = NA / split_gcd(STEP, NA);
    if constexpr (PIPE) read_b2(lds_raw + lane_base, 0, bq2[0]);
    if constexpr (PIPE) {
        const int last = nsuper - 1;
        for (int K0 = 0; K0 < last; K0 += PERIOD)
            split_static_for<PERIOD>([&](auto j) {
                constexpr int jj = decltype(j)::value;
                if (jj == 0 || K0 + jj < last) chunk_pipe(K0 + jj, std::integral_constant<int, (jj * STEP) % NA>{}, std::true_type{});
            });
        split_static_for<PERIOD>([&](auto j) {
            constexpr int jj = decltype(j)::value;
            if (PERIOD == 1 || last % PERIOD == jj) chunk_pipe(last, std::integral_constant<int, (jj * STEP) % NA>{}, std::false_type{});
        });
    } else {
        for (int K0 = 0; K0 < nsuper; K0 += PERIOD)
            split_static_for<PERIOD>([&](auto j) {
                constexpr int jj = decltype(j)::value;
                if (jj == 0 || K0 + jj < nsuper) chunk(K0 + jj, std::integral_constant<int, (jj * STEP) % NA>{});
            });
    }

    NND_SSTAMP(2);
    NND_SCLOCK(6);
    if constexpr (split_range_scaled(NS)) {
#pragma unroll
        for (int pp = 0; pp < P; ++pp)
#pragma unroll
            for (int i = 0; i < 16; ++i) acc[pp][i] *= oscale;
    }
    int ys[P], xs[P];
#pragma unroll
    for (int pp = 0; pp < P; ++pp) {
        ys[pp] = ty0[pp] + r;
        xs[pp] = tx0[pp] + c;
    }
    float* red_all = reinterpret_cast<float*>(lds_raw);
    constexpr int TS = P * 1024;
    auto exchange = [&]() {
        if (active) {
            float* red = red_all + (size_t)(cbi * ks + kj) * TS + lane;
#pragma unroll
            for (int pp = 0; pp < P; ++pp)
#pragma unroll
                for (int reg = 0; reg < 16; ++reg) red[pp * 1024 + reg * 64] = acc[pp][reg];
        }
        __syncthreads();
    };
    auto finish_c4 = [&](auto ng_c) {
        constexpr int NG = decltype(ng_c)::value;
        const int q0 = kj * NG;
        EpiOpsC4<P, NG> eo;
#ifndef NND_SPLIT_NO_EPI
        if (active) epi_c4_load<P, NG>(a, cb, b, h2, q0, ys, xs, eo);
#endif
        exchange();
        if (!active) return;
        float4 cacc[P][NG];
#pragma unroll
        for (int pp = 0; pp < P; ++pp)
#pragma unroll
            for (int j = 0; j < NG; ++j) {
                float v[4];
#pragma unroll
                for (int i = 0; i < 4; ++i) {
                    const float* red = red_all + (size_t)(cbi * ks) * TS + pp * 1024 + (4 * (q0 + j) + i) * 64 + lane;
                    float sum = red[0];
#pragma unroll
                    for (int sl = 1; sl < 4 / NG; ++sl) sum += red[(size_t)sl * TS];
                    v[i] = sum;
                }
                cacc[pp][j] = make_float4(v[0], v[1], v[2], v[3]);
            }
        NND_SSTAMP(3);
#ifdef NND_SPLIT_NO_EPI
        if (cacc[0][0].x != 123.456f) return;
#endif
        epi_c4_store<P, NG>(a, cacc, cb, b, h2, q0, eo);
    };
    if (a.ld.ci == 4) {
        if (ks == 4) finish_c4(std::integral_constant<int, 1>{});
        else if (ks == 2) finish_c4(std::integral_constant<int, 2>{});
        else {
            if (!active) return;
            NND_SSTAMP(3);
#ifdef NND_SPLIT_NO_EPI
            if (acc[0][0] != 123.456f) return;
#endif
            conv_epilogue_c4<P>(a, acc, cb, b, h2, 0, 16, ys, xs);
        }
    } else {
        if (ks > 1) exchange();
        if (!active) return;
        const int nreg = 16 / ks, reg0 = kj * nreg;
        if (ks > 1) {
            const float* red = red_all + (size_t)(cbi * ks) * TS + lane;
#pragma unroll
            for (int pp = 0; pp < P; ++pp)
#pragma unroll
                for (int reg = 0; reg < 16; ++reg) {
                    if (reg < reg0 || reg >= reg0 + nreg) continue;
                    float sum = red[pp * 1024 + reg * 64];
                    for (int j = 1; j < ks; ++j) sum += red[(size_t)j * TS + pp * 1024 + reg * 64];
                    acc[pp][reg] = sum;
                }
        }
        NND_SSTAMP(3);
#ifdef NND_SPLIT_NO_EPI
        if (acc[0][0] != 123.456f) return;
#endif
        conv_epilogue_planar<P>(a, acc, cb, b, h2, reg0, nreg, ys, xs);
    }
#ifdef NND_DBG_STAMPS
    __builtin_amdgcn_s_waitcnt(0);
#endif
    NND_SSTAMP(4);
}

struct SplitCfg {
    int ny, wco, ks, P, ntiles, tiles_x, nu;
    bool fast;
    size_t lds;
    int stride;
    bool restricted;
    dim3 grid, block;
};

constexpr int SPLIT_MAX_WAVES = 12;

inline int split_tiles(int H, int W, int* tiles_x) { return (*tiles_x = cdiv(W, 8)) * cdiv(H, 4); }

template <int KH, int KW, int NS, int P, int NU, bool FAST, bool SRC4, int AD, int MAXT, int STR = 1>
int launch_split_kernel(const ConvArgs& a, dim3 grid, dim3 block, size_t lds, hipStream_t stream) {
    auto kern = conv_split_kernel<KH, KW, NS, P, NU, FAST, SRC4, AD, MAXT, STR>;
    if ((int)block.x > MAXT) {
        set_error("conv_split: %u threads exceed the %d-thread bound of this instantiation", block.x, MAXT);
        return NND_ERR_INVALID;
    }
    lds += switches().lds_slack;
    if (lds > 64 * 1024) {
        static std::atomic<unsigned> raised{0};
        if (int rc = raise_lds_limit(reinterpret_cast<const void*>(kern), raised)) return rc;
    }
    hipLaunchKernelGGL(kern, grid, block, lds, stream, a);
    return NND_OK;
}

template <int KH, int KW, int NS>
constexpr int split_fast_ad() {
#ifdef NND_SPLIT_FAST_AD
    return NND_SPLIT_FAST_AD;
#else
    return KH * KW == 9 ? 2 : (KH * KW == 5 ? (NS <= 2 ? 4 : 2) : 1);
#endif
}

template <int KH, int KW, int NS, bool FAST, bool SRC4, int STR>
int launch_split_nu(const ConvArgs& a, const SplitCfg& cfg, hipStream_t stream) {
    constexpr int AD = FAST ? split_fast_ad<KH, KW, NS>() : 1;
    if (split_nu_variant(cfg.nu) == 2) return launch_split_kernel<KH, KW, NS, 2, 2, FAST, SRC4, AD, 768, STR>(a, cfg.grid, cfg.block, cfg.lds, stream);
    return launch_split_kernel<KH, KW, NS, 2, 4, FAST, SRC4, AD, 768, STR>(a, cfg.grid, cfg.block, cfg.lds, stream);
}
template <int KH, int KW, int NS>
int launch_split_shape(const ConvArgs& a, const SplitCfg& cfg, hipStream_t stream) {
    if (cfg.P != 2) return NND_ERR_UNSUPPORTED;
    const bool src4 = a.ls.ci == 4;
    if (cfg.stride == 2) {
        if constexpr (KH * KW == 9 || KH * KW == 1) {
            if (!cfg.fast) return NND_ERR_UNSUPPORTED;
            return src4 ? launch_split_nu<KH, KW, NS, true, true, 2>(a, cfg, stream) : launch_split_nu<KH, KW, NS, true, false, 2>(a, cfg, stream);
        } else {
            return NND_ERR_UNSUPPORTED;
        }
    }
    if (!cfg.fast) return launch_split_nu<KH, KW, NS, false, false, 1>(a, cfg, stream);
    return src4 ? launch_split_nu<KH, KW, NS, true, true, 1>(a, cfg, stream) : launch_split_nu<KH, KW, NS, true, false, 1>(a, cfg, stream);
}

template <int NS>
int launch_split_ns(const ConvArgs& a, const SplitCfg& cfg, int KH, int KW, hipStream_t stream) {
    if (KH == 3 && KW == 3) return launch_split_shape<3, 3, NS>(a, cfg, stream);
    if (KH == 1 && KW == 5) return launch_split_shape<1, 5, NS>(a, cfg, stream);
    if (KH == 5 && KW == 1) return launch_split_shape<5, 1, NS>(a, cfg, stream);
    if (KH == 1 && KW == 1) return launch_split_shape<1, 1, NS>(a, cfg, stream);
    return NND_ERR_UNSUPPORTED;
}

}
```

nndepth_amd/csrc/conv_split_ns1.hip:

```cpp
#include "conv_split_kernel.h"

namespace nnd {
template int launch_split_ns<1>(const ConvArgs&, const SplitCfg&, int, int, hipStream_t);
#ifdef NND_DBG_STAMPS
extern "C" int nnd_debug_read_split_stamps_ns1(unsigned long long* host, int n) {
    return hipMemcpyFromSymbol(host, HIP_SYMBOL(g_split_stamps), sizeof(unsigned long long) * n) == hipSuccess ? 0 : -1;
}
#endif
}
```

nndepth_amd/csrc/conv_split_ns2.hip:

```cpp
#include "conv_split_kernel.h"

namespace nnd {
template int launch_split_ns<2>(const ConvArgs&, const SplitCfg&, int, int, hipStream_t);
#ifdef NND_DBG_STAMPS
extern "C" int nnd_debug_read_split_stamps_ns2(unsigned long long* host, int n) {
    return hipMemcpyFromSymbol(host, HIP_SYMBOL(g_split_stamps), sizeof(unsigned long long) * n) == hipSuccess ? 0 : -1;
}
#endif
}
```

nndepth_amd/csrc/conv_split_ns3.hip:

```cpp
#include "conv_split_kernel.h"

namespace nnd {
template int launch_split_ns<3>(const ConvArgs&, const SplitCfg&, int, int, hipStream_t);
#ifdef NND_DBG_STAMPS
extern "C" int nnd_debug_read_split_stamps_ns3(unsigned long long* host, int n) {
    return hipMemcpyFromSymbol(host, HIP_SYMBOL(g_split_stamps), sizeof(unsigned long long) * n) == hipSuccess ? 0 : -1;
}
#endif
}
```

nndepth_amd/csrc/error.cpp:

```cpp
#include "common.h"

#include <cstdlib>

namespace nnd {
static thread_local char g_err[512] = "";
void set_error(const char* fmt, ...) {
    va_list ap;
    va_start(ap, fmt);
    vsnprintf(g_err, sizeof(g_err), fmt, ap);
    va_end(ap);
}

static Switches g_sw;
static void load_switches() {
    Switches s{};
    auto on = [](const char* n) { return getenv(n) != nullptr; };
    s.no_fused_upsample = on("NND_NO_FUSED_UPSAMPLE");
    s.no_fused_lookup = on("NND_NO_FUSED_LOOKUP");
    s.no_fused_flow_branch = on("NND_NO_FUSED_FLOW_BRANCH");
    s.no_c4 = on("NND_NO_C4");
    s.agcl_v1 = on("NND_AGCL_V1");
    s.no_thin3d = on("NND_NO_THIN3D");
    s.corr_build_v1 = on("NND_CORR_BUILD_V1");
    s.corr_build_no_ksplit = on("NND_CORR_BUILD_NO_KSPLIT");
    s.igev_squeeze_v1 = on("NND_IGEV_SQUEEZE_V1");
    s.igev_squeeze_walk = on("NND_IGEV_SQUEEZE_WALK");
    s.no_folded_flow_head = on("NND_NO_FOLDED_FLOW_HEAD");
    s.no_conv1x1_stream = on("NND_NO_CONV1X1_STREAM");
    s.conv_verbose = on("NND_CONV_VERBOSE");
    s.debug_sync = on("NND_DEBUG_SYNC");
    s.split_ny = s.split_ks = s.split_p = -1;
    if (const char* e = getenv("NND_SPLIT_CFG")) sscanf(e, "%d,%d,%d", &s.split_ny, &s.split_ks, &s.split_p);
    s.split_no_fast = on("NND_SPLIT_NO_FAST");
    s.no_merged_fb_lookup = on("NND_NO_MERGED_FB_LOOKUP");
    s.conv_p = s.conv_ks = s.conv_wco = -1;
    if (const char* e = getenv("NND_CONV_CFG")) sscanf(e, "%d,%d,%d", &s.conv_p, &s.conv_ks, &s.conv_wco);
    if (const char* e = getenv("NND_CONV_P")) s.conv_p = atoi(e);
    s.agcl_pb = getenv("NND_AGCL_PB") ? atoi(getenv("NND_AGCL_PB")) : 0;
    s.lds_poison_on = on("NND_DEBUG_LDS_POISON");
    s.lds_poison = s.lds_poison_on ? (unsigned)strtoul(getenv("NND_DEBUG_LDS_POISON"), nullptr, 0) : 0u;
    s.lds_slack = getenv("NND_DEBUG_LDS_SLACK") ? atoi(getenv("NND_DEBUG_LDS_SLACK")) : 0;
    s.enc_no_c4 = on("NND_ENC_NO_C4");
    s.no_slab3d = on("NND_NO_SLAB3D");
    s.slab3d_rounds = getenv("NND_SLAB3D_ROUNDS") ? atoi(getenv("NND_SLAB3D_ROUNDS")) : 0;
    s.no_fused_enc_block = on("NND_NO_FUSED_ENC_BLOCK");
    g_sw = s;
}
namespace {
struct SwitchInit {
    SwitchInit() { load_switches(); }
} g_switch_init;
}
const Switches& switches() { return g_sw; }
}

extern "C" {
int nnd_reload_switches(void) {
    nnd::load_switches();
    return NND_OK;
}
int nnd_version(void) { return NND_VERSION; }
const char* nnd_last_error(void) { return nnd::g_err; }
int nnd_device_count(void) {
    int n = 0;
    if (hipGetDeviceCount(&n) != hipSuccess) {
        (void)hipGetLastError();
        return 0;
    }
    return n;
}
}
```

nndepth_amd/csrc/update_block.hip:

```cpp
#include "common.h"
#include "conv_layer.h"
#include "layout.h"

#include <cstdlib>
#include <cstring>
#include <vector>

namespace nnd {

enum ConvId { C_C1 = 0, C_C2, C_F2, C_CV, C_ZR1X, C_Q1X, C_ZR2X, C_Q2X, C_FHM, C_M2, C_LOOP_COUNT,
              C_ZR1 = C_LOOP_COUNT, C_Q1, C_ZR2, C_Q2, C_ZR1C, C_Q1C, C_ZR2C, C_Q2C, C_COUNT };
static const char* kConvNames[C_COUNT] = {"encoder.convc1", "encoder.convc2", "encoder.convf2", "encoder.conv",
                                          "gru.convz1+convr1[h,motion]", "gru.convq1[rh,motion]", "gru.convz2+convr2[h,motion]",
                                          "gru.convq2[rh,motion]", "flow_head.conv1+mask.0", "mask.2",
                                          "gru.convz1+convr1", "gru.convq1", "gru.convz2+convr2", "gru.convq2",
                                          "gru.convz1+convr1[inp]", "gru.convq1[inp]", "gru.convz2+convr2[inp]", "gru.convq2[inp]"};

struct Plan {
    nnd_update_block_desc d;
    bool sep;
    int num_tensors;
    ConvLayer L[C_COUNT];
    int64_t f1_w, f1_b;
    int64_t f1_wt;
// ... 530 lines not shown
    one(C_F2, 6);
    one(C_CV, 8);
    const int ctx = p.d.context_dim, gin = 2 * hid + ctx;
    std::vector<int> map_x(2 * hid), map_c(ctx);
    for (int i = 0; i < hid; ++i) {
        map_x[i] = i;
        map_x[hid + i] = hid + ctx + i;
    }
    for (int i = 0; i < ctx; ++i) map_c[i] = hid + i;
    auto gru = [&](int pass, int tz, int tr, int tq) {
        const int zr = pass == 0 ? C_ZR1 : C_ZR2, q = pass == 0 ? C_Q1 : C_Q2;
        two(zr, tz, tr, hid, hid);
        one(q, tq);
        const float* wzr[2] = {t[tz], t[tr]};
        const float* bzr[2] = {t[tz + 1], t[tr + 1]};
        const float* nob[2] = {nullptr, nullptr};
        int czr[2] = {hid, hid};
        pack_conv(p.L[zr - C_ZR1 + C_ZR1X], 2, wzr, nob, czr, out, map_x.data(), gin);
        pack_conv(p.L[zr - C_ZR1 + C_ZR1C], 2, wzr, bzr, czr, out, map_c.data(), gin);
        const float* wq[1] = {t[tq]};
        const float* bq[1] = {t[tq + 1]};
        int cq[1] = {hid};
        pack_conv(p.L[q - C_ZR1 + C_ZR1X], 1, wq, nob, cq, out, map_x.data(), gin);
        pack_conv(p.L[q - C_ZR1 + C_ZR1C], 1, wq, bq, cq, out, map_c.data(), gin);
    };
    gru(0, 10, 12, 14);
    int k = 16;
    if (p.sep) {
        gru(1, 16, 18, 20);
        k = 22;
    }
    two(C_FHM, k, k + 4, hid, 2 * hid);
    memcpy(out + p.fc2_w, t[k + 2], sizeof(float) * fc * hid * 9);
    memcpy(out + p.fc2_b, t[k + 3], sizeof(float) * fc);
    one(C_M2, k + 6);
    return NND_OK;
}

int nnd_update_block_scale_slots(const nnd_update_block_desc* desc, int64_t* offsets, int n) {
    Plan p;
    int rc = make_plan(desc, &p);
    if (rc != NND_OK) return rc;
    for (int i = 0; offsets && i < n && i < C_COUNT; ++i) offsets[i] = p.L[i].range_scaled() ? p.L[i].tail_off() : -1;
    return C_COUNT;
}

int nnd_update_block_calibration_finish(const nnd_update_block_desc* desc, float* packed_dev, int32_t* status_dev, void* stream) {
    Plan p;
    int rc = make_plan(desc, &p);
    if (rc != NND_OK) return rc;
    NND_REQUIRE(packed_dev, "update_block_calibration_finish: null blob");
    int64_t offs[C_COUNT];
    int n = 0;
    for (int i = 0; i < C_COUNT; ++i)
        if (p.L[i].range_scaled() && (p.sep || (i != C_ZR2 && i != C_Q2 && i != C_ZR2X && i != C_Q2X && i != C_ZR2C && i != C_Q2C))) offs[n++] = p.L[i].tail_off();
    return calib_finish(packed_dev, offs, n, status_dev, (hipStream_t)stream);
}

int nnd_update_block_layer_forward(const nnd_update_block_desc* desc, const float* packed, int which, const float* const* in,
                                   float* const* out, float* workspace, int B, int H, int W, void* stream) {
    Plan p;
    int rc = make_plan(desc, &p);
    if (rc != NND_OK) return rc;
    if ((rc = refuse_last_only(desc, "update_block_layer_forward")) != NND_OK) return rc;
    NND_REQUIRE(packed && in && out && workspace && B > 0 && H > 0 && W > 0, "update_block_layer_forward: bad argument");
    NND_REQUIRE(which > C_C1 && which < C_COUNT && which != C_F2, "update_block_layer_forward: convolution %d has no stand-alone launch here", which);
    NND_REQUIRE(p.sep || (which != C_ZR2 && which != C_Q2 && which != C_ZR2X && which != C_Q2X && which != C_ZR2C && which != C_Q2C),
                "update_block_layer_forward: conv_gru has no second GRU pass");
    CalibScope calib((p.d.flags & NND_FLAG_CALIBRATE) && split_range_scaled(p.d.arithmetic));
    hipStream_t s = (hipStream_t)stream;
    Bufs w;
    carve(p, B, H, W, workspace, &w);
    const int hid = p.d.hidden_dim, ctx = p.d.context_dim;
    const int64_t n = tiled_plane(H, W);
    struct { float* buf; int C; bool c4; } t[NND_UB_TENSORS] = {
        {w.c1, 256, ws_c4()}, {w.cf, 256, ws_c4()}, {w.hx, 2 * hid + ctx, ws_c4()}, {w.z, hid, ws_c4()}, {w.rh, hid, ws_c4()},
        {w.fm, 3 * hid, ws_c4()}, {w.ctxb, 6 * hid, ws_c4()}, {w.mask, p.d.mask_channels, false}};
    for (int i = 0; i < NND_UB_TENSORS; ++i)
        if (in[i]) NND_TRY(to_tiled(in[i], t[i].buf, (int64_t)t[i].C * n, B, t[i].C, H, W, s, 0, t[i].c4));
    NND_TRY(run_conv(p, packed, w, which, act(w.corr, p.d.cor_planes * n, p.d.cor_planes), w.mask, w.delta, B, H, W, s));
    for (int i = 0; i < NND_UB_TENSORS; ++i)
        if (out[i]) NND_TRY(from_tiled(t[i].buf, (int64_t)t[i].C * n, out[i], B, t[i].C, H, W, s, 0, t[i].c4));
    return NND_OK;
}

int64_t nnd_update_block_workspace_floats(const nnd_update_block_desc* desc, int B, int H, int W) {
    Plan p;
    if (make_plan(desc, &p) != NND_OK || B <= 0 || H <= 0 || W <= 0) return NND_ERR_INVALID;
    Bufs b;
    carve(p, B, H, W, nullptr, &b);
    return b.total;
}

int nnd_update_block_forward(const nnd_update_block_desc* desc, const float* packed, const float* net, const float* inp,
                             const float* corr, const float* flow, float* net_out, float* mask_out, float* delta_out,
                             float* workspace, int B, int H, int W, void* stream) {
    Plan p;
    int rc = make_plan(desc, &p);
    if (rc != NND_OK) return rc;
    if ((rc = refuse_last_only(desc, "update_block_forward")) != NND_OK) return rc;
    NND_REQUIRE(packed && net && inp && corr && flow && net_out && delta_out && workspace, "update_block_forward: null pointer");
    NND_REQUIRE(B > 0 && H > 0 && W > 0, "update_block_forward: bad shape");
    CalibScope calib((p.d.flags & NND_FLAG_CALIBRATE) && split_range_scaled(p.d.arithmetic));
    hipStream_t s = (hipStream_t)stream;
    Bufs w;
    carve(p, B, H, W, workspace, &w);
    const int hid = p.d.hidden_dim, ctx = p.d.context_dim, fc = p.d.flow_channels, hxC = 2 * hid + ctx;
    const int64_t n = tiled_plane(H, W);
    NND_TRY(to_tiled(net, w.hx, hxC * n, B, hid, H, W, s, 0, ws_c4()));
    NND_TRY(to_tiled(inp, w.hx, hxC * n, B, ctx, H, W, s, hid, ws_c4()));
    NND_TRY(to_tiled(flow, w.hx, hxC * n, B, fc, H, W, s, hxC - fc, ws_c4()));
    NND_TRY(to_tiled(flow, w.flow, fc * n, B, fc, H, W, s));
    NND_TRY(to_tiled(corr, w.corr, p.d.cor_planes * n, B, p.d.cor_planes, H, W, s));
    Act c = act(w.corr, p.d.cor_planes * n, p.d.cor_planes);
    NND_TRY(run_update(p, packed, w, c, w.flow, mask_out ? w.mask : nullptr, w.delta, B, H, W, s));
    NND_TRY(from_tiled(w.hx, hxC * n, net_out, B, hid, H, W, s, 0, ws_c4()));
    NND_TRY(from_tiled(w.delta, fc * n, delta_out, B, fc, H, W, s));
    if (mask_out) NND_TRY(from_tiled(w.mask, p.d.mask_channels * n, mask_out, B, p.d.mask_channels, H, W, s));
    return NND_OK;
}

struct CreArgs {
    const float* f1;
    const float* f2;
    const float* extra;
    float* warped;
    int64_t warped_floats;
    int C;
};

struct LoopProbe {
    int which;
    bool empty = false;
    int marks = 0;
    std::vector<hipEvent_t> ev;
};
static thread_local LoopProbe* t_probe = nullptr;
static void probe_mark(int id, hipStream_t s) {
    if (!t_probe || t_probe->which != id) return;
    const bool opening = (t_probe->marks++ & 1) == 0;
    if (t_probe->empty && !opening) return;
    for (int k = 0; k < (t_probe->empty ? 2 : 1); ++k) {
        hipEvent_t e = nullptr;
        if (hipEventCreate(&e) != hipSuccess) return;
        (void)hipEventRecord(e, s);
        t_probe->ev.push_back(e);
    }
}

static int enqueue_refine(const nnd_update_block_desc* desc, const float* packed, const float* pyramid, int num_levels,
                          int radius, const float* net, const float* inp, const float* disp_init, float* up_out,
                          int64_t up_iter_stride, float* low_out, float* net_out, float* workspace, int B, int H, int W,
                          int rate, int iters, void* stream, const float* geo_pyramid = nullptr, int groups = 1,
                          const CreArgs* cre = nullptr, const float* interleaved = nullptr, int flat_groups = 0) {
    Plan p;
    int rc = make_plan(desc, &p);
    if (rc != NND_OK) return rc;
    const bool last_flag = (p.d.flags & NND_FLAG_LAST_UPSAMPLE_ONLY) != 0;
    NND_REQUIRE(!last_flag || up_iter_stride == 0,
                "refine: NND_FLAG_LAST_UPSAMPLE_ONLY writes one upsampled map, so up_iter_stride must be 0 (got %lld)", (long long)up_iter_stride);
    const bool last_only = last_flag && !(p.d.flags & NND_FLAG_CALIBRATE);
    NND_REQUIRE(packed && (pyramid || cre) && net && inp && up_out && workspace, "refine: null pointer");
    const bool igev = geo_pyramid != nullptr;
    const int fc = p.d.flow_channels;
    if (cre) {
        NND_REQUIRE(fc == 2 && p.d.cor_planes == 36, "cre_stereo_refine: needs flow_channels 2 and cor_planes 36");
        NND_REQUIRE(cre->f1 && cre->f2 && (cre->extra || cre->warped), "cre_stereo_refine: null feature map / scratch");
        NND_REQUIRE(cre->extra || cre->warped_floats >= (int64_t)B * cre->C * H * W,
                    "cre_stereo_refine: iter mode needs a scratch of B*C*H*W = %lld floats, got %lld", (long long)B * cre->C * H * W,
                    (long long)cre->warped_floats);
    } else {
        NND_REQUIRE(fc == 1, "raft_stereo_refine: flow_channels must be 1");
        NND_REQUIRE(p.d.cor_planes == num_levels * (2 * radius + 1) * (igev ? 2 * groups : (flat_groups > 0 ? flat_groups : 1)),
                    "refine: cor_planes %d does not match levels*(2r+1)%s", p.d.cor_planes, igev ? "*2*groups" : (flat_groups > 0 ? "*groups" : ""));
        NND_REQUIRE(!(igev && flat_groups > 0), "refine: the IGEV and the group-RAFT lookups exclude each other");
    }

    NND_REQUIRE(p.d.mask_channels == 9 * rate * rate, "raft_stereo_refine: mask_channels %d != 9*rate^2", p.d.mask_channels);
    NND_REQUIRE(B > 0 && H > 0 && W > 0 && iters > 0, "raft_stereo_refine: bad shape");
    CalibScope calib((p.d.flags & NND_FLAG_CALIBRATE) && split_range_scaled(p.d.arithmetic));
    hipStream_t s = (hipStream_t)stream;
    Bufs w;
    carve(p, B, H, W, workspace, &w);
    const int hid = p.d.hidden_dim, ctx = p.d.context_dim, hxC = 2 * hid + ctx;
    const Lay lay = make_lay(H, W, true);
    const int64_t n = lay.plane;
    NND_TRY(to_tiled(net, w.hx, hxC * n, B, hid, H, W, s, 0, ws_c4()));
    NND_TRY(to_tiled(inp, w.hx, hxC * n, B, ctx, H, W, s, hid, ws_c4()));
    float* hx_flow = w.hx + ws_chan(hxC - fc, n);
    const unsigned eg = (unsigned)cdiv64((int64_t)B * H * W, 256);
    if (cre) {
        if (disp_init) {
            NND_TRY(to_tiled(disp_init, w.flow, fc * n, B, fc, H, W, s));
            NND_TRY(to_tiled(disp_init, w.hx, hxC * n, B, fc, H, W, s, hxC - fc, ws_c4()));
        } else {
            NND_HIP_CHECK(hipMemsetAsync(w.flow, 0, sizeof(float) * B * fc * n, s));
            NND_TRY(to_tiled(nullptr, w.hx, hxC * n, B, fc, H, W, s, hxC - fc, ws_c4()));
        }
    } else {
        hipLaunchKernelGGL(init_coords_kernel, dim3(eg), dim3(256), 0, s, w.coords, w.flow, hx_flow, (long)(hxC * n), ws_pm(), disp_init, B, H,
                           W, igev ? 1 : 0, lay);
        NND_LAUNCH_CHECK();
    }
    const bool cre_cl = cre && cre->extra && cre->warped && cre->warped_floats >= 2 * (int64_t)B * cre->C * H * W &&
                        agcl_offset_cl_supported(cre->C) && !switches().agcl_v1;
    if (cre_cl) {
        NND_TRY(nchw_to_nhwc_launch(cre->f1, cre->warped, B, cre->C, H * W, s));
        NND_TRY(nchw_to_nhwc_launch(cre->f2, cre->warped + (int64_t)B * cre->C * H * W, B, cre->C, H * W, s));
    }
    Act c = act(w.corr, p.d.cor_planes * n, p.d.cor_planes);
    auto lookup = [&](hipStream_t st_, int it) -> int {
        if (cre) {
            if (cre->extra && cre_cl)
                return agcl_offset_cl_launch(cre->warped, cre->warped + (int64_t)B * cre->C * H * W, w.flow, cre->extra, w.corr, B, cre->C,
                                             H, W, it & 1, st_, true);
            if (cre->extra) return agcl_offset_launch(cre->f1, cre->f2, w.flow, cre->extra, w.corr, B, cre->C, H, W, it & 1, st_, true);
            return agcl_iter_launch(cre->f1, cre->f2, w.flow, cre->warped, w.corr, B, cre->C, H, W, it & 1, st_, true);
        }
        if (igev) return igev_lookup_launch(pyramid, geo_pyramid, w.coords, w.corr, B, groups, H, W, num_levels, radius, st_, true);
        if (flat_groups > 0) return group_lookup_flat_launch(pyramid, w.coords, w.corr, B, flat_groups, H, W, num_levels, radius, st_, true);
        return corr1d_lookup_launch(pyramid, w.coords, w.corr, B, H, W, num_levels, radius, st_, true);
    };
    for (int id : {(int)C_ZR1C, (int)C_Q1C, (int)C_ZR2C, (int)C_Q2C})
        if (p.sep || id < C_ZR2C) NND_TRY(run_conv(p, packed, w, id, c, nullptr, nullptr, B, H, W, s));
    const bool no_fuse_up = switches().no_fused_upsample;
    const bool no_fuse_lk = switches().no_fused_lookup;
    const bool fused_up = !no_fuse_up && mask_upsample_supported(rate, 2 * hid, fc);
    const bool fold_fh = fused_up && !cre && fc == 1 && mask_upsample_fold_supported(p.L[C_M2], hid) &&
                         (long)B * cdiv(H, 4) * cdiv(W, 8) <= 256 && !switches().no_folded_flow_head;
    float* coords_alt = w.mask;
    float* flow_alt = w.mask + ((int64_t)B * n + 63) / 64 * 64;
    const bool fused_lk = !cre && !no_fuse_lk && flat_groups == 0;
    const bool merged_fbl = fused_lk && !igev && !switches().no_merged_fb_lookup && !switches().no_fused_flow_branch &&
                            flow_branch_supported(p.L[C_F2], fc) && flow_branch_lookup_supported(p.L[C_F2].arith);
    auto loop_conv = [&](int id) -> int {
        probe_mark(id, s);
        const int rc_ = run_conv(p, packed, w, id, c, nullptr, nullptr, B, H, W, s);
        probe_mark(id, s);
        return rc_;
    };
    if (calibrating() && fused_lk && interleaved && p.L[C_C1].range_scaled() && igev_lookup_convc1_il_supported(groups, num_levels, radius))
        NND_TRY(calib_amax_flat(interleaved, nnd_igev_interleaved_floats(B, groups, H, W, num_levels), packed + p.L[C_C1].tail_off(), s));
    for (int it = 0; it < iters; ++it) {
        if (merged_fbl) {
            probe_mark(C_F2, s);
            NND_TRY(calib_flow_branch(p, packed, w, w.flow, B, H, W, s));
            const ConvIO fio = conv_io(p, w, C_F2, c, n, nullptr, nullptr);
            NND_TRY(flow_branch_lookup_launch(p.L[C_F2], packed, packed + p.f1_wt, packed + p.f1_b, w.flow, (int64_t)fc * n, fc, fio, pyramid,
                                              w.coords, p.L[C_C1], w.c1, 256 * n, B, H, W, num_levels, radius, s, ws_c4()));
            NND_TRY(debug_sync("encoder.convf1+convf2 | lookup+convc1", s));
            probe_mark(C_F2, s);
        } else {
        probe_mark(C_F2, s);
        NND_TRY(run_flow_branch(p, packed, w, w.flow, c, B, H, W, s));
        probe_mark(C_F2, s);
        if (fused_lk && interleaved && igev_lookup_convc1_il_supported(groups, num_levels, radius)) {
            NND_TRY(igev_lookup_convc1_il_launch(interleaved, groups, w.coords, p.L[C_C1], packed, w.c1, 256 * n, B, H, W, num_levels,
                                                 radius, s, ws_c4()));
            NND_TRY(debug_sync("lookup+convc1 (interleaved)", s));
        } else if (fused_lk && p.L[C_C1].arith == 0) {
            NND_TRY(lookup_convc1_launch(pyramid, geo_pyramid, groups, w.coords, p.L[C_C1], packed, w.c1, 256 * n, B, H, W,
                                         num_levels, radius, s, ws_c4()));
            NND_TRY(debug_sync("lookup+convc1", s));
        } else {
            NND_TRY(lookup(s, it));
            NND_TRY(debug_sync("lookup", s));
            NND_TRY(run_conv(p, packed, w, C_C1, c, nullptr, nullptr, B, H, W, s));
        }
        }
        NND_TRY(loop_conv(C_C2));
        NND_TRY(loop_conv(C_CV));
        NND_TRY(loop_conv(C_ZR1X));
        NND_TRY(loop_conv(C_Q1X));
        if (p.sep) {
            NND_TRY(loop_conv(C_ZR2X));
            NND_TRY(loop_conv(C_Q2X));
        }
        if (last_only && it + 1 < iters) {
            ConvIO io = conv_io(p, w, C_FHM, c, n, nullptr, nullptr);
            io.cout_need = hid;
            NND_TRY(launch_conv(p.L[C_FHM], packed, io, conv_epi(C_FHM), B, H, W, s));
            NND_TRY(debug_sync("flow_head.conv1", s));
            NND_TRY(run_fc2(p, packed, w, w.delta, cre ? 2 : 1, igev, B, H, W, s));
            continue;
        }
        NND_TRY(loop_conv(C_FHM));
        float* up_it = up_out + (int64_t)it * up_iter_stride;
        if (fold_fh) {
            MaskUpFlowHead fh;
            fh.x = w.fm; fh.xbs = (int64_t)3 * hid * n; fh.hid = hid;
            fh.w = packed + p.fc2_w; fh.bias = packed + p.fc2_b;
            fh.coords_in = w.coords; fh.coords_out = coords_alt; fh.flow_out = flow_alt; fh.delta_out = w.delta;
            fh.hx_flow = hx_flow; fh.hx_bs = (long)(hxC * n); fh.hx_pm = ws_pm(); fh.absolute = igev ? 1 : 0;
            NND_TRY(mask_upsample_launch(p.L[C_M2], packed, w.fm + hid * n, (int64_t)3 * hid * n, w.flow, up_it, B, H, W, rate, s,
                                         true, fc, ws_c4(), &fh));
            NND_TRY(debug_sync("flow_head.conv2 + mask.2 + upsample", s));
            std::swap(w.coords, coords_alt);
            std::swap(w.flow, flow_alt);
            continue;
        }
        NND_TRY(run_fc2(p, packed, w, w.delta, cre ? 2 : 1, igev, B, H, W, s));
        if (fused_up) {
            NND_TRY(mask_upsample_launch(p.L[C_M2], packed, w.fm + hid * n, (int64_t)3 * hid * n, w.flow, up_it, B, H, W, rate, s,
                                         true, fc, ws_c4()));
            NND_TRY(debug_sync("mask.2 + upsample", s));
        } else {
            NND_TRY(run_conv(p, packed, w, C_M2, c, w.mask, nullptr, B, H, W, s));
            NND_TRY(convex_upsample_launch(w.flow, w.mask, up_it, B, fc, H, W, rate, s, true));
            NND_TRY(debug_sync("convex upsample", s));
        }
    }
    if (low_out) NND_TRY(from_tiled(w.flow, fc * n, low_out, B, fc, H, W, s));
    if (net_out) NND_TRY(from_tiled(w.hx, hxC * n, net_out, B, hid, H, W, s, 0, ws_c4()));
    return NND_OK;
}

static int conv2d_layer(int Cout, int Cin, int KH, int KW, int arithmetic, ConvLayer* L, int64_t* total) {
    NND_REQUIRE(Cout > 0 && Cin > 0, "conv2d: bad channel counts");
    NND_REQUIRE(conv_shape_built(KH, KW), "conv2d: kernel %dx%d not built (1x1, 3x3, 1x5, 5x1)", KH, KW);
    NND_REQUIRE(arithmetic == 0 || conv_split_supported(KH, KW, Cin, 1, arithmetic),
                "conv2d: arithmetic %d not built for %dx%d with %d input channels (3 = bf16x3, 2 = fp16x2, 1 = fp16: Cin %% 16 == 0)", arithmetic, KH, KW, Cin);
    int64_t off = 0;
    *L = mk(KH, KW, Cin, Cout, &off, arithmetic);
    if (total) *total = off;
    return NND_OK;
}

int64_t nnd_conv2d_packed_floats_ex(int Cout, int Cin, int KH, int KW, int arithmetic) {
    ConvLayer L;
    int64_t total;
    if (conv2d_layer(Cout, Cin, KH, KW, arithmetic, &L, &total) != NND_OK) return NND_ERR_INVALID;
    return total;
}
int64_t nnd_conv2d_packed_floats(int Cout, int Cin, int KH, int KW) { return nnd_conv2d_packed_floats_ex(Cout, Cin, KH, KW, 0); }

int nnd_conv2d_pack_ex(const float* w_host, const float* b_host, int Cout, int Cin, int KH, int KW, int arithmetic, float* packed_host) {
    ConvLayer L;
    int rc = conv2d_layer(Cout, Cin, KH, KW, arithmetic, &L, nullptr);
    if (rc != NND_OK) return rc;
    NND_REQUIRE(w_host && b_host && packed_host, "conv2d_pack: null pointer");
    const float* w[1] = {w_host};
    const float* b[1] = {b_host};
    int co[1] = {Cout};
    pack_conv(L, 1, w, b, co, packed_host);
    return NND_OK;
}
int nnd_conv2d_pack(const float* w_host, const float* b_host, int Cout, int Cin, int KH, int KW, float* packed_host) {
    return nnd_conv2d_pack_ex(w_host, b_host, Cout, Cin, KH, KW, 0, packed_host);
}

int nnd_conv2d_forward_ex(const float* packed_dev, const float* x, float* y, int B, int Cin, int H, int W, int Cout, int KH,
                          int KW, int relu, int arithmetic, void* stream) {
    ConvLayer L;
    int rc = conv2d_layer(Cout, Cin, KH, KW, arithmetic, &L, nullptr);
    if (rc != NND_OK) return rc;
    NND_REQUIRE(packed_dev && x && y && B > 0 && H > 0 && W > 0, "conv2d_forward: bad argument");
    const int64_t n = (int64_t)H * W;
    ConvIO io{};
    io.src0 = act(const_cast<float*>(x), Cin * n, Cin);
    io.out0 = act(y, Cout * n, Cout);
    return launch_conv(L, packed_dev, io, relu ? EPI_RELU : EPI_LINEAR, B, H, W, (hipStream_t)stream);
}
int nnd_conv2d_calibrate_ex(float* packed_dev, const float* x, int B, int Cin, int H, int W, int Cout, int KH, int KW, int arithmetic,
                            int32_t* status_dev, void* stream) {
    ConvLayer L;
    int rc = conv2d_layer(Cout, Cin, KH, KW, arithmetic, &L, nullptr);
    if (rc != NND_OK) return rc;
    NND_REQUIRE(packed_dev && x && B > 0 && H > 0 && W > 0, "conv2d_calibrate: bad argument");
    if (!L.range_scaled()) return NND_OK;
    const int64_t n = (int64_t)H * W;
    rc = calib_amax_act(act(const_cast<float*>(x), Cin * n, Cin), make_lay(H, W, false), B, H, W, packed_dev + L.tail_off(), (hipStream_t)stream);
    if (rc != NND_OK) return rc;
    const int64_t off = L.tail_off();
    return calib_finish(packed_dev, &off, 1, status_dev, (hipStream_t)stream);
}

int nnd_conv2d_scale_slots_ex(int Cout, int Cin, int KH, int KW, int arithmetic, int64_t* offsets, int n) {
    ConvLayer L;
    int rc = conv2d_layer(Cout, Cin, KH, KW, arithmetic, &L, nullptr);
    if (rc != NND_OK) return rc;
    if (!offsets) return 1;
    NND_REQUIRE(n >= 1, "conv2d_scale_slots: room for %d offsets, a layer has 1 slot", n);
    offsets[0] = L.range_scaled() ? L.tail_off() : -1;
    return 1;
}

int nnd_conv2d_forward(const float* packed_dev, const float* x, float* y, int B, int Cin, int H, int W, int Cout, int KH,
                       int KW, int relu, void* stream) {
    return nnd_conv2d_forward_ex(packed_dev, x, y, B, Cin, H, W, Cout, KH, KW, relu, 0, stream);
}

int nnd_conv2d_offset_forward(const float* packed_dev, const float* x, float* y, int B, int Cin, int H, int W, int Cout, int KH,
                              int KW, float range, void* stream) {
    ConvLayer L;
    int rc = conv2d_layer(Cout, Cin, KH, KW, 0, &L, nullptr);
    if (rc != NND_OK) return rc;
    NND_REQUIRE(packed_dev && x && y && B > 0 && H > 0 && W > 0, "conv2d_offset_forward: bad argument");
    const int64_t n = (int64_t)H * W;
    ConvIO io{};
    io.src0 = act(const_cast<float*>(x), Cin * n, Cin);
    io.out0 = act(y, Cout * n, Cout);
    io.scale = range;
    return launch_conv(L, packed_dev, io, EPI_SIGMOID_RANGE, B, H, W, (hipStream_t)stream);
}

int nnd_raft_stereo_refine(const nnd_update_block_desc* desc, const float* packed, const float* pyramid, int num_levels,
                           int radius, const float* net, const float* inp, const float* disp_init, float* up_out,
                           int64_t up_iter_stride, float* low_out, float* net_out, float* workspace, int B, int H, int W,
                           int rate, int iters, void* stream) {
    return enqueue_refine(desc, packed, pyramid, num_levels, radius, net, inp, disp_init, up_out, up_iter_stride, low_out,
                          net_out, workspace, B, H, W, rate, iters, stream);
}

int nnd_raft_stereo_group_refine(const nnd_update_block_desc* desc, const float* packed, const float* group_pyramid, int num_groups,
                                 int num_levels, int radius, const float* net, const float* inp, const float* disp_init, float* up_out,
                                 int64_t up_iter_stride, float* low_out, float* net_out, float* workspace, int B, int H, int W, int rate,
                                 int iters, void* stream) {
    NND_REQUIRE(num_groups > 0, "raft_stereo_group_refine: num_groups must be positive");
    return enqueue_refine(desc, packed, group_pyramid, num_levels, radius, net, inp, disp_init, up_out, up_iter_stride, low_out, net_out,
                          workspace, B, H, W, rate, iters, stream, nullptr, 1, nullptr, nullptr, num_groups);
}

int nnd_igev_refine_reads_interleaved(int num_groups, int num_levels, int radius) {
    return !switches().no_fused_lookup && igev_lookup_convc1_il_supported(num_groups, num_levels, radius);
}

int nnd_igev_stereo_refine(const nnd_update_block_desc* desc, const float* packed, const float* feat_pyramid,
                           const float* geo_pyramid, const float* interleaved, int num_groups, int num_levels, int radius,
                           const float* net, const float* inp,
                           const float* disp_init, float* up_out, int64_t up_iter_stride, float* low_out, float* net_out,
                           float* workspace, int B, int H, int W, int rate, int iters, void* stream) {
    NND_REQUIRE(geo_pyramid && num_groups > 0, "igev_stereo_refine: geometry pyramid / groups missing");
    return enqueue_refine(desc, packed, feat_pyramid, num_levels, radius, net, inp, disp_init, up_out, up_iter_stride, low_out,
                          net_out, workspace, B, H, W, rate, iters, stream, geo_pyramid, num_groups, nullptr, interleaved);
}

int nnd_cre_stereo_refine(const nnd_update_block_desc* desc, const float* packed, const float* fmap1, const float* fmap2,
                          int C, const float* extra_offset, float* scratch, int64_t scratch_floats, const float* net, const float* inp,
                          const float* flow_init, float* up_out, int64_t up_iter_stride, float* low_out, float* net_out,
                          float* workspace, int B, int H, int W, int rate, int iters, void* stream) {
    NND_REQUIRE(fmap1 && fmap2, "cre_stereo_refine: null feature map");
    NND_REQUIRE(extra_offset || scratch, "cre_stereo_refine: iter mode (extra_offset == NULL) needs the scratch for the warped map");
    NND_REQUIRE(scratch_floats >= 0 && (scratch || scratch_floats == 0), "cre_stereo_refine: scratch_floats without a scratch");
    int rc = agcl_check("cre_stereo_refine", B, C, H, W);
    if (rc != NND_OK) return rc;
    CreArgs cre{fmap1, fmap2, extra_offset, scratch, scratch_floats, C};
    return enqueue_refine(desc, packed, nullptr, 0, 0, net, inp, flow_init, up_out, up_iter_stride, low_out, net_out, workspace,
                          B, H, W, rate, iters, stream, nullptr, 1, &cre);
}

int nnd_mask_upsample_forward(const float* packed_dev, const float* x, const float* flow, float* out, int B, int Cin, int H,
                              int W, int rate, void* stream) {
    ConvLayer L;
    int rc = conv2d_layer(9 * rate * rate, Cin, 1, 1, 0, &L, nullptr);
    if (rc != NND_OK) return rc;
    NND_REQUIRE(packed_dev && x && flow && out && B > 0 && H > 0 && W > 0, "mask_upsample_forward: bad argument");
    NND_REQUIRE(mask_upsample_supported(rate, Cin, 1), "mask_upsample_forward: rate %d / Cin %d not built", rate, Cin);
    return mask_upsample_launch(L, packed_dev, x, (int64_t)Cin * H * W, flow, out, B, H, W, rate, (hipStream_t)stream, false);
}

int nnd_num_convs(const nnd_update_block_desc* desc) {
    Plan p;
    if (make_plan(desc, &p) != NND_OK) return NND_ERR_INVALID;
    return C_LOOP_COUNT;
}

const char* nnd_conv_name(const nnd_update_block_desc* desc, int which) {
    (void)desc;
    return (which >= 0 && which < C_COUNT) ? kConvNames[which] : "";
}

int nnd_profile_conv(const nnd_update_block_desc* desc, const float* packed, float* workspace, int B, int H, int W, int which,
                     int reps, void* stream, float* ms_out, double* flops_out) {
    Plan p;
    int rc = make_plan(desc, &p);
    if (rc != NND_OK) return rc;
    if ((rc = refuse_last_only(desc, "profile_conv")) != NND_OK) return rc;
    NND_REQUIRE(packed && workspace && ms_out && flops_out, "profile_conv: null pointer");
    NND_REQUIRE(which >= 0 && which < C_LOOP_COUNT && reps > 0, "profile_conv: bad conv index / reps");
    NND_REQUIRE(p.sep || (which != C_ZR2X && which != C_Q2X), "profile_conv: conv_gru has no second GRU pass");
    hipStream_t s = (hipStream_t)stream;
    Bufs w;
    carve(p, B, H, W, workspace, &w);
    const int64_t n = tiled_plane(H, W);
    Act c = act(w.corr, p.d.cor_planes * n, p.d.cor_planes);
    hipEvent_t e0, e1;
    NND_HIP_CHECK(hipEventCreate(&e0));
    NND_HIP_CHECK(hipEventCreate(&e1));
    rc = run_conv(p, packed, w, which, c, w.mask, w.delta, B, H, W, s);
    if (rc == NND_OK) {
        (void)hipEventRecord(e0, s);
        for (int i = 0; i < reps && rc == NND_OK; ++i) rc = run_conv(p, packed, w, which, c, w.mask, w.delta, B, H, W, s);
        (void)hipEventRecord(e1, s);
        (void)hipEventSynchronize(e1);
        float ms = 0.f;
        (void)hipEventElapsedTime(&ms, e0, e1);
        *ms_out = ms / reps;
        *flops_out = p.L[which].flops(B, H, W);
    }
    (void)hipEventDestroy(e0);
    (void)hipEventDestroy(e1);
    return rc;
}
}

static int profile_loop(const nnd_update_block_desc* desc, const float* packed, const float* pyramid, int num_levels, int radius,
                        const float* net, const float* inp, float* up_out, float* workspace, int B, int H, int W, int rate, int iters,
                        int which, void* stream, float* ms_out, bool empty) {
    NND_REQUIRE(ms_out && which >= 0 && which < C_LOOP_COUNT && which != C_C1 && which != C_M2 && iters > 0,
                "profile_loop_conv: conv %d is not a stand-alone launch of the recurrence", which);
    if (int rc = refuse_last_only(desc, "profile_loop_conv")) return rc;
    LoopProbe probe;
    probe.which = which;
    probe.empty = empty;
    t_probe = &probe;
    int rc = enqueue_refine(desc, packed, pyramid, num_levels, radius, net, inp, nullptr, up_out, 0, nullptr, nullptr, workspace, B,
                            H, W, rate, iters, stream);
    t_probe = nullptr;
    if (rc == NND_OK && hipStreamSynchronize((hipStream_t)stream) != hipSuccess) rc = NND_ERR_HIP;
    double sum = 0.0;
    int n = 0;
    for (size_t i = 0; i + 1 < probe.ev.size(); i += 2) {
        float ms = 0.f;
        if (rc == NND_OK && i >= 2 && hipEventElapsedTime(&ms, probe.ev[i], probe.ev[i + 1]) == hipSuccess) {
            sum += ms;
            ++n;
        }
    }
    for (hipEvent_t e : probe.ev) (void)hipEventDestroy(e);
    if (rc != NND_OK) return rc;
    NND_REQUIRE(n > 0, "profile_loop_conv: needs at least 2 iterations");
    *ms_out = (float)(sum / n);
    return NND_OK;
}

extern "C" int nnd_profile_loop_conv(const nnd_update_block_desc* desc, const float* packed, const float* pyramid, int num_levels,
                                     int radius, const float* net, const float* inp, float* up_out, float* workspace, int B, int H,
                                     int W, int rate, int iters, int which, void* stream, float* ms_out) {
    return profile_loop(desc, packed, pyramid, num_levels, radius, net, inp, up_out, workspace, B, H, W, rate, iters, which, stream, ms_out,
                        false);
}

extern "C" int nnd_profile_loop_event_pair(const nnd_update_block_desc* desc, const float* packed, const float* pyramid, int num_levels,
                                           int radius, const float* net, const float* inp, float* up_out, float* workspace, int B, int H,
                                           int W, int rate, int iters, int which, void* stream, float* ms_out) {
    return profile_loop(desc, packed, pyramid, num_levels, radius, net, inp, up_out, workspace, B, H, W, rate, iters, which, stream, ms_out,
                        true);
}

namespace nnd {
typedef float f32x16_ __attribute__((ext_vector_type(16)));
__global__ void __launch_bounds__(256) mfma_probe_kernel(float* out, int iters, float seed) {
    f32x16_ acc0, acc1;
    for (int i = 0; i < 16; ++i) { acc0[i] = 0.f; acc1[i] = 0.f; }
    float av = seed + threadIdx.x * 1e-3f, bv = seed * 0.5f + threadIdx.x * 2e-3f;
    for (int i = 0; i < iters; ++i) {
#pragma unroll
        for (int j = 0; j < 8; ++j) {
            acc0 = __builtin_amdgcn_mfma_f32_32x32x2f32(av, bv, acc0, 0, 0, 0);
            acc1 = __builtin_amdgcn_mfma_f32_32x32x2f32(bv, av, acc1, 0, 0, 0);
        }
    }
    float s = 0.f;
    for (int i = 0; i < 16; ++i) s += acc0[i] + acc1[i];
    if (s == 12345.678f) out[0] = s;
}
// ... 98 lines not shown
```

nndepth_amd/ops.py:

```python
import contextlib
import ctypes as C
import itertools
import os
import threading
from typing import Callable, Dict, List, NamedTuple, Optional, Sequence, Tuple

import torch

from ._lib import (NND_FLAG_CALIBRATE, NND_FLAG_LAST_UPSAMPLE_ONLY, NND_MIDAS_KEEP_PRE, Conv3dDesc, ConvDesc, EncoderDesc, MidasDesc,
                   MobileNetV3Desc, NndError, RepViTDesc,
                   UpdateBlockDesc,
                   check, lib)


def _dev(*tensors: torch.Tensor) -> torch.device:
    d = tensors[0].device
    for t in tensors:
        if t.device.type != "cuda":
            raise NndError("nndepth_amd ops run on the HIP device only; got a tensor on "
                           f"{t.device} (no CPU fallback exists)")
        if t.dtype != torch.float32:
            raise NndError(f"nndepth_amd ops are fp32; got {t.dtype}")
        if t.device != d:
            raise NndError("all tensors must live on the same device")
# ... 255 lines not shown
    def __init__(self, weight: torch.Tensor, bias: torch.Tensor, device="cuda", arithmetic: str = "fp32"):
        self.Cout, self.Cin, self.KH, self.KW = (int(s) for s in weight.shape)
        self.arith = arithmetic_id(arithmetic)
        n = int(lib.nnd_conv2d_packed_floats_ex(self.Cout, self.Cin, self.KH, self.KW, self.arith))
        if n <= 0:
            check(n, "conv2d_packed_floats")
        w, b = _host(weight), _host(bias)
        blob = torch.empty(n, dtype=torch.float32)
        check(lib.nnd_conv2d_pack_ex(_p(w), _p(b), self.Cout, self.Cin, self.KH, self.KW, self.arith, _p(blob)), "conv2d_pack")
        self.packed_host = blob
        self.packed = blob.to(device) if device is not None else None
        self.calibrated = False

    def calibrate(self, x: torch.Tensor) -> "Conv2d":
        d = _dev(x, self.packed)
        x = x.contiguous()
        B, Cin, H, W = x.shape
        if Cin != self.Cin:
            raise NndError(f"conv2d: input has {Cin} channels, weights expect {self.Cin}")
        with torch.cuda.device(d):
            check(lib.nnd_conv2d_calibrate_ex(_p(self.packed), _p(x), B, Cin, H, W, self.Cout, self.KH, self.KW, self.arith, None,
                                              _stream(d)), "conv2d_calibrate")
        self.calibrated = True
        return self

    def activation_range(self) -> float:
        if self.arith not in (1, 2):
            return float("inf")
        ncb = (self.Cout + 31) // 32
        n = self.packed.numel()
        return 65504.0 / float(self.packed[n - 4 + 1].item()) if ncb else float("inf")

    def __call__(self, x: torch.Tensor, relu: bool = False) -> torch.Tensor:
        d = _dev(x, self.packed)
        x = x.contiguous()
        B, Cin, H, W = x.shape
        if Cin != self.Cin:
            raise NndError(f"conv2d: input has {Cin} channels, weights expect {self.Cin}")
        if self.arith in (1, 2):
            if getattr(_calib_tls, "active", None) is not None:
                self.calibrate(x)
            else:
                _calib_flags(self)
        y = torch.empty((B, self.Cout, H, W), dtype=torch.float32, device=d)
        with torch.cuda.device(d):
            check(lib.nnd_conv2d_forward_ex(_p(self.packed), _p(x), _p(y), B, Cin, H, W, self.Cout, self.KH, self.KW,
                                            int(relu), self.arith, _stream(d)), "conv2d_forward")
        return y


def conv2d_offset(conv: "Conv2d", x: torch.Tensor, rng: float) -> torch.Tensor:
    d = _dev(x, conv.packed)
    if conv.arith != 0:
        raise NndError("conv2d_offset: exact fp32 packing expected")
    x = x.contiguous()
    B, Cin, H, W = x.shape
    if Cin != conv.Cin:
        raise NndError(f"conv2d_offset: input has {Cin} channels, weights expect {conv.Cin}")
    y = torch.empty((B, conv.Cout, H, W), dtype=torch.float32, device=d)
    with torch.cuda.device(d):
        check(lib.nnd_conv2d_offset_forward(_p(conv.packed), _p(x), _p(y), B, Cin, H, W, conv.Cout, conv.KH, conv.KW, float(rng),
                                            _stream(d)), "conv2d_offset_forward")
    return y


def split_tanh_relu(x: torch.Tensor, c_net: int) -> Tuple[torch.Tensor, torch.Tensor]:
    d = _dev(x)
    x = x.contiguous()
    B, Cc, H, W = x.shape
    if not 0 < c_net < Cc:
        raise NndError(f"split_tanh_relu: cannot split {Cc} channels at {c_net}")
    net = torch.empty((B, c_net, H, W), dtype=torch.float32, device=d)
    inp = torch.empty((B, Cc - c_net, H, W), dtype=torch.float32, device=d)
    with torch.cuda.device(d):
        check(lib.nnd_split_tanh_relu(_p(x), _p(net), _p(inp), B, c_net, Cc - c_net, H, W, _stream(d)), "split_tanh_relu")
    return net, inp


def pos_enc_sine_add(x0: torch.Tensor, x1: Optional[torch.Tensor] = None, temp_bug_fix: bool = False):
    d = _dev(x0) if x1 is None else _dev(x0, x1)
    x0 = x0.contiguous()
    N, Cc, H, W = x0.shape
    y0 = torch.empty_like(x0)
    y1 = None
    if x1 is not None:
        x1 = x1.contiguous()
        if tuple(x1.shape) != tuple(x0.shape):
            raise NndError(f"pos_enc_sine_add: second map {tuple(x1.shape)} != {tuple(x0.shape)}")
        y1 = torch.empty_like(x1)
    with torch.cuda.device(d):
        check(lib.nnd_pos_enc_sine_add(_p(x0), _p(x1), _p(y0), _p(y1), N, Cc, H, W, int(temp_bug_fix), _stream(d)), "pos_enc_sine_add")
    return y0 if x1 is None else (y0, y1)


def avg_pool_2x_4x(x: torch.Tensor) -> Tuple[torch.Tensor, torch.Tensor]:
    d = _dev(x)
    x = x.contiguous()
    N, Cc, H, W = x.shape
    o2 = torch.empty((N, Cc, H // 2, W // 2), dtype=torch.float32, device=d)
    o4 = torch.empty((N, Cc, H // 4, W // 4), dtype=torch.float32, device=d)
    with torch.cuda.device(d):
        check(lib.nnd_avg_pool_2x_4x(_p(x), _p(o2), _p(o4), N, Cc, H, W, _stream(d)), "avg_pool_2x_4x")
    return o2, o4


def resize_bilinear_ac(x: torch.Tensor, size: Tuple[int, int], mul: float = 1.0) -> torch.Tensor:
    d = _dev(x)
    x = x.contiguous()
    N, Cc, h, w = x.shape
    H, W = int(size[0]), int(size[1])
    y = torch.empty((N, Cc, H, W), dtype=torch.float32, device=d)
    with torch.cuda.device(d):
        check(lib.nnd_resize_bilinear_ac(_p(x), _p(y), N, Cc, h, w, H, W, float(mul), _stream(d)), "resize_bilinear_ac")
    return y


def resize_nearest_scaled(x: torch.Tensor, size: Tuple[int, int], mul: float = 1.0) -> torch.Tensor:
    d = _dev(x)
    x = x.contiguous()
    if x.dim() < 3 or x.shape[-3] != 1:
        raise NndError(f"resize_nearest_scaled: single-channel maps (..., 1, h, w) expected, got {tuple(x.shape)}")
    h, w = x.shape[-2:]
    H, W = int(size[0]), int(size[1])
    y = torch.empty(tuple(x.shape[:-2]) + (H, W), dtype=torch.float32, device=d)
    with torch.cuda.device(d):
        check(lib.nnd_resize_nearest_scaled(_p(x), _p(y), x.numel() // (h * w), h, w, H, W, float(mul), _stream(d)),
              "resize_nearest_scaled")
    return y


def mask_upsample(conv: "Conv2d", x: torch.Tensor, flow: torch.Tensor, rate: int) -> torch.Tensor:
    d = _dev(x, flow, conv.packed)
    x, flow = x.contiguous(), flow.contiguous()
    B, Cin, H, W = x.shape
    out = torch.empty((B, 1, rate * H, rate * W), dtype=torch.float32, device=d)
    with torch.cuda.device(d):
        check(lib.nnd_mask_upsample_forward(_p(conv.packed), _p(x), _p(flow), _p(out), B, Cin, H, W, rate, _stream(d)),
              "mask_upsample_forward")
    return out


def update_block_keys(gru: str = "sep_conv") -> List[str]:
    names = ["encoder.convc1", "encoder.convc2", "encoder.convf1", "encoder.convf2", "encoder.conv",
             "gru.convz1", "gru.convr1", "gru.convq1"]
    if gru == "sep_conv":
        names += ["gru.convz2", "gru.convr2", "gru.convq2"]
    names += ["flow_head.conv1", "flow_head.conv2", "mask.0", "mask.2"]
    return [f"{n}.{s}" for n in names for s in ("weight", "bias")]


class _RefineCall(NamedTuple):
    desc: UpdateBlockDesc
    d: torch.device
    net: torch.Tensor
    inp: torch.Tensor
    init: Optional[torch.Tensor]
    up: torch.Tensor
    stride: int
    low: torch.Tensor
    net_out: torch.Tensor
    ws: torch.Tensor
    B: int
    H: int
    W: int


class UpdateBlockEngine(ScaleSlots):

    def _scale_slots(self) -> List[Tuple[str, int]]:
        offs = _enumerate_slots(lambda o, n: lib.nnd_update_block_scale_slots(C.byref(self.desc), o, n), "update_block_scale_slots")
        out, seen = [], set()
        for i, o in enumerate(offs):
            if o >= 0 and o not in seen:
                seen.add(o)
                out.append((lib.nnd_conv_name(C.byref(self.desc), i).decode() or f"conv{i}", o))
        return out

    ARITHMETIC = {"fp32": 0, "bf16x3": 3, "fp16x2": 2, "fp16": 1}

    def __init__(self, hidden_dim: int, context_dim: int, cor_planes: int, flow_channels: int,
                 mask_channels: int, gru: str = "sep_conv", arithmetic: str = "fp32"):
        if gru not in ("sep_conv", "conv_gru"):
            raise NndError(f"unknown gru kind {gru!r}")
        arithmetic_id(arithmetic)
        self.gru = gru
        self.arithmetic = arithmetic
        self.desc = UpdateBlockDesc(hidden_dim, context_dim, cor_planes, flow_channels, mask_channels,
                                    0 if gru == "sep_conv" else 1, self.ARITHMETIC[arithmetic],
                                    int(os.environ.get("NND_SPLIT_MASK", "0"), 0) & 0x7fffffff, 0)
        self.calibrated = False
        n = lib.nnd_update_block_packed_floats(C.byref(self.desc))
        if n <= 0:
            check(int(n), "update_block_packed_floats")
        self.packed_floats = int(n)
        self.packed: Optional[torch.Tensor] = None
        self._ws: Optional[torch.Tensor] = None

    def pack_host(self, state: dict, prefix: str = "") -> torch.Tensor:
        keys = update_block_keys(self.gru)
        assert len(keys) == lib.nnd_update_block_num_tensors(C.byref(self.desc))
        hold = [state[prefix + k].detach().to("cpu", torch.float32).contiguous() for k in keys]
        ptrs = (C.c_void_p * len(hold))(*[t.data_ptr() for t in hold])
        out = torch.empty(self.packed_floats, dtype=torch.float32)
        check(lib.nnd_update_block_pack(C.byref(self.desc), ptrs, _p(out)), "update_block_pack")
        return out

    def load(self, state: dict, prefix: str = "", device="cuda") -> "UpdateBlockEngine":
        self.packed = self.pack_host(state, prefix).to(device)
        self.calibrated = False
        return self

    @staticmethod
    def _keep_all(keep_all: Optional[bool], last_only: bool) -> bool:
        if last_only and keep_all:
            raise NndError("refine: last_only=True computes one upsampled map; it cannot be combined with keep_all=True")
        return (not last_only) if keep_all is None else bool(keep_all)

    def _calibration_finish(self, status: Optional[torch.Tensor]) -> None:
        check(lib.nnd_update_block_calibration_finish(C.byref(self.desc), _p(self.packed), _p(status), _stream(self.packed.device)),
              "update_block_calibration_finish")

    def activation_ranges(self) -> Dict[str, float]:
        n = int(lib.nnd_update_block_scale_slots(C.byref(self.desc), None, 0))
        offs = (C.c_int64 * n)()
        check(min(0, int(lib.nnd_update_block_scale_slots(C.byref(self.desc), offs, n))), "update_block_scale_slots")
        blob = self.packed.cpu() if self.packed is not None else None
        out = {}
        for i in range(n):
            if offs[i] >= 0 and blob is not None:
                name = lib.nnd_conv_name(C.byref(self.desc), i).decode()
                if self.gru != "sep_conv" and ("convz2+convr2" in name or "convq2" in name):
                    continue
                out[name or f"conv{i}"] = 65504.0 / float(blob[offs[i] + 1])
        return out

    def workspace(self, B: int, H: int, W: int, device) -> torch.Tensor:
        n = int(lib.nnd_update_block_workspace_floats(C.byref(self.desc), B, H, W))
        if n <= 0:
            check(n, "update_block_workspace_floats")
        if self._ws is None or self._ws.numel() < n or self._ws.device != torch.device(device):
            self._ws = torch.empty(n, dtype=torch.float32, device=device)
        return self._ws

    def _check_state(self, what: str, net, inp, init, init_channels: int):
        ds = self.desc
        B, _, H, W = net.shape
        if tuple(net.shape) != (B, ds.hidden_dim, H, W):
            raise NndError(f"{what}: net shape {tuple(net.shape)} != {(B, ds.hidden_dim, H, W)}")
        if tuple(inp.shape) != (B, ds.context_dim, H, W):
            raise NndError(f"{what}: inp shape {tuple(inp.shape)} != {(B, ds.context_dim, H, W)}")
        if init is not None and tuple(init.shape) != (B, init_channels, H, W):
            raise NndError(f"{what}: initial disparity / flow shape {tuple(init.shape)} != {(B, init_channels, H, W)}")

    def forward(self, net, inp, corr, flow, want_mask: bool = True):
        if self.packed is None:
            raise NndError("UpdateBlockEngine: parameters not loaded")
        d = _dev(net, inp, corr, flow, self.packed)
        net, inp, corr, flow = (t.contiguous() for t in (net, inp, corr, flow))
        B, _, H, W = net.shape
        ds = self.desc
        exp = {"net": (B, ds.hidden_dim, H, W), "inp": (B, ds.context_dim, H, W),
               "corr": (B, ds.cor_planes, H, W), "flow": (B, ds.flow_channels, H, W)}
        for name, t in (("net", net), ("inp", inp), ("corr", corr), ("flow", flow)):
            if tuple(t.shape) != exp[name]:
                raise NndError(f"update_block: {name} shape {tuple(t.shape)} != {exp[name]}")
        net_out = torch.empty_like(net)
        mask = torch.empty((B, ds.mask_channels, H, W), dtype=torch.float32, device=d) if want_mask else None
        delta = torch.empty_like(flow)
        ws = self.workspace(B, H, W, d)
        with torch.cuda.device(d):
            check(lib.nnd_update_block_forward(C.byref(_call_desc(self)), _p(self.packed), _p(net), _p(inp), _p(corr), _p(flow),
                                               _p(net_out), _p(mask), _p(delta), _p(ws), B, H, W, _stream(d)),
                  "update_block_forward")
        return net_out, mask, delta

    def _refine_call(self, what: str, tensors, net, inp, init, channels: int, rate: int, iters: int,
                     keep_all: Optional[bool], last_only: bool) -> "_RefineCall":
        if self.packed is None:
            raise NndError("UpdateBlockEngine: parameters not loaded")
        keep_all = self._keep_all(keep_all, last_only)
        desc = _call_desc(self, NND_FLAG_LAST_UPSAMPLE_ONLY if last_only else 0)
        d = _dev(*tensors, net, inp, self.packed)
        net, inp = net.contiguous(), inp.contiguous()
        B, _, H, W = net.shape
        self._check_state(what, net, inp, init, channels)
        if init is not None:
            _dev(init)
            init = init.contiguous()
        up = torch.empty((iters if keep_all else 1, B, channels, rate * H, rate * W), dtype=torch.float32, device=d)
        low = torch.empty((B, channels, H, W), dtype=torch.float32, device=d)
        return _RefineCall(desc, d, net, inp, init, up, up[0].numel() if keep_all else 0, low, torch.empty_like(net),
                           self.workspace(B, H, W, d), B, H, W)

    def refine(self, pyr, num_levels: int, radius: int, net, inp, rate: int, iters: int,
               disp_init=None, keep_all: Optional[bool] = None, last_only: bool = False):
        c = self._refine_call("refine", (pyr,), net, inp, disp_init, 1, rate, iters, keep_all, last_only)
        B, H, W = c.B, c.H, c.W
        if pyr.numel() != pyramid_layout(B, H, W, num_levels)[2]:
            raise NndError(f"refine: pyramid holds {pyr.numel()} floats, a {B}x{H}x{W} pyramid of {num_levels} levels has "
                           f"{pyramid_layout(B, H, W, num_levels)[2]}")
        with torch.cuda.device(c.d):
            check(lib.nnd_raft_stereo_refine(C.byref(c.desc), _p(self.packed), _p(pyr), num_levels, radius,
                                             _p(c.net), _p(c.inp), _p(c.init), _p(c.up), c.stride, _p(c.low), _p(c.net_out),
                                             _p(c.ws), B, H, W, rate, iters, _stream(c.d)), "raft_stereo_refine")
        return c.up, c.low, c.net_out

    def refine_group(self, group_pyr, num_groups: int, num_levels: int, radius: int, net, inp, rate: int, iters: int,
                     disp_init=None, keep_all: Optional[bool] = None, last_only: bool = False):
        c = self._refine_call("refine_group", (group_pyr,), net, inp, disp_init, 1, rate, iters, keep_all, last_only)
        B, H, W = c.B, c.H, c.W
        need = pyramid_layout(B * num_groups, H, W, num_levels)[2]
        if group_pyr.numel() != need:
            raise NndError(f"refine_group: pyramid holds {group_pyr.numel()} floats, expected {need} for B*G={B * num_groups}, "
                           f"{H}x{W}, {num_levels} levels")
        with torch.cuda.device(c.d):
            check(lib.nnd_raft_stereo_group_refine(C.byref(c.desc), _p(self.packed), _p(group_pyr), num_groups, num_levels, radius,
                                                   _p(c.net), _p(c.inp), _p(c.init), _p(c.up), c.stride, _p(c.low), _p(c.net_out),
                                                   _p(c.ws), B, H, W, rate, iters, _stream(c.d)), "raft_stereo_group_refine")
        return c.up, c.low, c.net_out

    def refine_igev(self, feat_pyr, geo_pyr, num_groups: int, num_levels: int, radius: int, net, inp, rate: int,
                    iters: int, disp_init=None, keep_all: Optional[bool] = None, interleaved=None, last_only: bool = False):
        c = self._refine_call("refine_igev", (feat_pyr, geo_pyr), net, inp, disp_init, 1, rate, iters, keep_all, last_only)
        B, H, W = c.B, c.H, c.W
        need = pyramid_layout(B * num_groups, H, W, num_levels)[2]
        if feat_pyr.numel() != need or geo_pyr.numel() != need:
            raise NndError(f"refine_igev: pyramids hold {feat_pyr.numel()} / {geo_pyr.numel()} floats, expected {need} "
                           f"for B*G={B * num_groups}, {H}x{W}, {num_levels} levels")
        if interleaved is not None:
            _dev(interleaved)
            need_il = int(lib.nnd_igev_interleaved_floats(B, num_groups, H, W, num_levels))
            if interleaved.numel() != need_il:
                raise NndError(f"refine_igev: interleaved copy holds {interleaved.numel()} floats, expected {need_il}")
        with torch.cuda.device(c.d):
            check(lib.nnd_igev_stereo_refine(C.byref(c.desc), _p(self.packed), _p(feat_pyr), _p(geo_pyr), _p(interleaved), num_groups,
                                             num_levels, radius, _p(c.net), _p(c.inp), _p(c.init), _p(c.up), c.stride, _p(c.low),
                                             _p(c.net_out), _p(c.ws), B, H, W, rate, iters, _stream(c.d)), "igev_stereo_refine")
        return c.up, c.low, c.net_out

    def refine_cre(self, fmap1, fmap2, net, inp, rate: int, iters: int, flow_init=None, extra_offset=None,
                   scratch=None, keep_all: Optional[bool] = None, last_only: bool = False):
        c = self._refine_call("refine_cre", (fmap1, fmap2), net, inp, flow_init, 2, rate, iters, keep_all, last_only)
        B, H, W = c.B, c.H, c.W
        fmap1, fmap2 = fmap1.contiguous(), fmap2.contiguous()
        Cf = fmap1.shape[1]
        if fmap2.shape != fmap1.shape or tuple(fmap1.shape) != (B, Cf, H, W):
            raise NndError(f"refine_cre: shapes fmap {tuple(fmap1.shape)} / {tuple(fmap2.shape)}, net {tuple(net.shape)}")
        if extra_offset is not None and extra_offset.numel() != B * 18 * H * W:
            raise NndError(f"refine_cre: extra_offset shape {tuple(extra_offset.shape)} != {(B, 18, H, W)}")
        if extra_offset is not None:
            extra_offset = extra_offset.contiguous()
            _dev(extra_offset)
        if scratch is None or scratch.numel() < fmap2.numel():
            need = fmap2.numel() if extra_offset is None else 2 * fmap2.numel()
            scratch = torch.empty(need, dtype=torch.float32, device=c.d)
        else:
            _dev(fmap2, scratch)
            if not scratch.is_contiguous():
                raise NndError("refine_cre: `scratch` must be contiguous")
        with torch.cuda.device(c.d):
            check(lib.nnd_cre_stereo_refine(C.byref(c.desc), _p(self.packed), _p(fmap1), _p(fmap2), Cf, _p(extra_offset),
                                            _p(scratch), scratch.numel(), _p(c.net), _p(c.inp), _p(c.init), _p(c.up), c.stride,
                                            _p(c.low), _p(c.net_out), _p(c.ws), B, H, W, rate, iters, _stream(c.d)), "cre_stereo_refine")
        return c.up, c.low, c.net_out

    def conv_names(self) -> List[str]:
        n = lib.nnd_num_convs(C.byref(self.desc))
        names = [lib.nnd_conv_name(C.byref(self.desc), i).decode() for i in range(n)]
        if self.gru != "sep_conv":
            names = [x for x in names if not x.endswith("2+convr2") and not x.endswith("convq2")]
        return names

    def profile_conv(self, which: int, B: int, H: int, W: int, reps: int, device) -> Tuple[float, float]:
        ws = self.workspace(B, H, W, device)
        ms, fl = C.c_float(), C.c_double()
        d = torch.device(device)
        with torch.cuda.device(d):
            check(lib.nnd_profile_conv(C.byref(self.desc), _p(self.packed), _p(ws), B, H, W, which, reps, _stream(d),
                                       C.byref(ms), C.byref(fl)), "profile_conv")
        return ms.value, fl.value


    def profile_loop_conv(self, which: int, pyr, num_levels: int, radius: int, net, inp, rate: int, iters: int,
                          event_pair_only: bool = False) -> float:
        d = _dev(pyr, net, inp, self.packed)
        net, inp = net.contiguous(), inp.contiguous()
        B, _, H, W = net.shape
        self._check_state("profile_loop_conv", net, inp, None, 1)
        up = torch.empty((B, 1, rate * H, rate * W), dtype=torch.float32, device=d)
        ws = self.workspace(B, H, W, d)
        ms = C.c_float()
        with torch.cuda.device(d):
            fn = lib.nnd_profile_loop_event_pair if event_pair_only else lib.nnd_profile_loop_conv
            check(fn(C.byref(self.desc), _p(self.packed), _p(pyr), num_levels, radius, _p(net), _p(inp),
                     _p(up), _p(ws), B, H, W, rate, iters, which, _stream(d), C.byref(ms)), "profile_loop_conv")
        return ms.value


def group_corr_build(fmap1: torch.Tensor, fmap2: torch.Tensor, num_groups: int, group_channels: int,
                     num_levels: int, pooled: bool = True) -> torch.Tensor:
    d = _dev(fmap1, fmap2)
    fmap1, fmap2 = fmap1.contiguous(), fmap2.contiguous()
    B, Ctot, H, W = fmap1.shape
    _, _, total = pyramid_layout(B * num_groups, H, W, num_levels)
    pyr = torch.empty(total, dtype=torch.float32, device=d)
    with torch.cuda.device(d):
        check(lib.nnd_group_corr_build(_p(fmap1), _p(fmap2), _p(pyr), B, Ctot, H, W, num_groups, group_channels,
                                       num_levels if pooled else 0, _stream(d)), "group_corr_build")
    return pyr


def raft_group_corr_build(fmap1: torch.Tensor, fmap2: torch.Tensor, num_groups: int, num_levels: int) -> torch.Tensor:
    d = _dev(fmap1, fmap2)
    fmap1, fmap2 = fmap1.contiguous(), fmap2.contiguous()
    B, Ctot, H, W = fmap1.shape
    if num_groups * num_groups > Ctot:
        raise NndError(f"raft_group_corr_build: {num_groups} chunks of {num_groups} channels exceed the {Ctot} channels of the maps")
    _, _, total = pyramid_layout(B * num_groups, H, W, num_levels)
    pyr = torch.empty(total, dtype=torch.float32, device=d)
    with torch.cuda.device(d):
        check(lib.nnd_group_corr_build_scaled(_p(fmap1), _p(fmap2), _p(pyr), B, Ctot, H, W, num_groups, num_groups, num_levels,
                                              float(Ctot) ** 0.5, _stream(d)), "group_corr_build_scaled")
    return pyr


def group_corr1d_lookup(pyr: torch.Tensor, coords: torch.Tensor, num_groups: int, num_levels: int, radius: int) -> torch.Tensor:
    d = _dev(pyr, coords)
    coords = coords.contiguous()
    B, one, H, W = coords.shape
    if one != 1:
        raise NndError("group_corr1d_lookup: coords must be (B,1,H,W)")
    if pyr.numel() != pyramid_layout(B * num_groups, H, W, num_levels)[2]:
        raise NndError(f"group_corr1d_lookup: pyramid holds {pyr.numel()} floats, expected "
                       f"{pyramid_layout(B * num_groups, H, W, num_levels)[2]} for B*G={B * num_groups}, {H}x{W}, {num_levels} levels")
    out = torch.empty((B, num_levels * num_groups * (2 * radius + 1), H, W), dtype=torch.float32, device=d)
    if out.numel() == 0:
        return out
    with torch.cuda.device(d):
        check(lib.nnd_group_corr1d_lookup(_p(pyr), _p(coords), _p(out), B, num_groups, H, W, num_levels, radius, _stream(d)),
              "group_corr1d_lookup")
    return out


def pyramid_from_level0(level0: torch.Tensor, B: int, H: int, W: int, num_levels: int) -> torch.Tensor:
    d = _dev(level0)
    offs, widths, total = pyramid_layout(B, H, W, num_levels)
    pyr = torch.empty(total, dtype=torch.float32, device=d)
    pyr[:B * H * W * W].copy_(level0.reshape(-1))
    with torch.cuda.device(d):
        check(lib.nnd_pyramid_from_level0(_p(pyr), B, H, W, num_levels, _stream(d)), "pyramid_from_level0")
    return pyr


# ... 1210 lines not shown
```

nndepth_amd/raft_stereo.py:

```python
import contextlib
import functools
import json
import os
from typing import Dict, List, Optional

import torch
import torch.nn as nn

from . import ops
from ._lib import NndError
from .blocks import BasicUpdateBlock
from .cost_volume import CorrBlock1D, GroupCorrBlock1D
from .encoder import BasicEncoder
from .upsample import convex_upsample


def load_weights(model: nn.Module, weights: str, strict_load: bool = True) -> nn.Module:
    if weights.endswith(".safetensors"):
        from safetensors.torch import load_file
        state = load_file(weights, device="cpu")
    else:
        state = torch.load(weights, map_location="cpu")
    model.load_state_dict(state, strict=strict_load)
    return model
# ... 149 lines not shown
            calibration_passes(lambda: self._forward(*args, **kwargs), max_passes,
                               f"{type(self).__name__}.calibrate: activations still overflow fp16 after {max_passes} passes "
                               "(non-finite inputs or weights?)")
        for eng, blob, xs in before:
            if eng.packed is blob:
                eng.widen_scales(xs)
        return self

    def _forward_calibrated(self, *args, **kwargs):
        check_outputs(getattr(self, "outputs", "all"))
        if self.arithmetic not in ops.RANGE_SCALED or not self.auto_calibrate or self._calib_pinned is not None:
            return self._watched(self._forward(*args, **kwargs))
        try:
            with ops.require_calibrated():
                return self._watched(self._forward(*args, **kwargs))
        except ops.NeedsCalibration:
            self.calibrate(*args, **kwargs)
            return self._watched(self._forward(*args, **kwargs))

    def _calibration_sites(self) -> Dict[str, "ops.ScaleSite"]:
        return {"update_block": self.update_block.calibration_site()}

    def _encoder_site(self, cache: "ops.ParamCache", output_dim: int, cnet_dim: int) -> "ops.ScaleSite":
        names = ops.EncoderEngine(output_dim, self.fnet.norm_fn, cnet_dim, self.arithmetic).scale_names()
        return ops.ScaleSite(names, lambda: cache.value, cache)

    def calibration_state(self) -> dict:
        return calibration_state(self)

    def load_calibration_state(self, state: dict):
        return load_calibration_state(self, state)

    def clear_calibration_state(self):
        return clear_calibration_state(self)

    def save_calibration(self, path: str) -> None:
        save_calibration(self, path)

    def load_calibration(self, path: str):
        return load_calibration(self, path)

    def _watched(self, outs):
        if self.watch_range:
            final = outs if torch.is_tensor(outs) else outs[-1]["up_disp"]
            if self._range_word is None or self._range_word.device != final.device:
                self._range_word = torch.zeros(1, dtype=torch.int32, device=final.device)
            ops.nonfinite_flag(final, self._range_word)
            self._range_forwards += 1
        return outs

    def range_status(self) -> dict:
        word = 0 if self._range_word is None else int(self._range_word.item())
        return {"overflow": bool(word & 1), "forwards": self._range_forwards}

    def reset_range_status(self) -> None:
        if self._range_word is not None:
            self._range_word.zero_()
        self._range_forwards = 0

    def range_report(self, *args, **kwargs) -> Dict[str, Dict[str, float]]:
        require_eval(self)
        if self.arithmetic not in ops.RANGE_SCALED:
            return {}
        try:
            with self._all_outputs(), ops.calibration(finish=False), torch.no_grad():
                self._forward(*args, **kwargs)
        finally:
            sites = [(p, s, _site_engine(s)) for p, s in calibration_sites(self).items() if s.names]
            sites = [(p, s, e) for p, s, e in sites if e is not None]
            got = [(p, s, e.read_scales(), e.read_records(clear=True)) for p, s, e in sites]
        report = {}
        for path, site, xs, seen in got:
            for n, e, m in zip(site.names, xs.cpu().tolist(), seen.cpu().tolist()):
                report[_layer_key(path, n)] = {"seen": float(m), "limit": 65504.0 / 2.0 ** e}
        return report

    def activation_ranges(self):
        eng = self.update_block.engine
        return eng.activation_ranges() if eng.packed is not None else {}


def hip_encoder_blocker(fnet: nn.Module, norms) -> Optional[str]:
    if fnet.norm_fn not in norms:
        return f"norm_fn={fnet.norm_fn!r} is not built in HIP (built: {', '.join(norms)})"
    if fnet.dropout is not None:
        return "dropout > 0"
    return None


class BaseRAFTStereo(AutoCalibrate, nn.Module):
    def __init__(self, iters: int = 12, fnet_dim: int = 256, hidden_dim: int = 128, context_dim: int = 128,
                 corr_levels: int = 4, corr_radius: int = 4, tracing: bool = False,
                 include_preprocessing: bool = False, weights: Optional[str] = None, strict_load: bool = True,
                 fused_loop: bool = True, hip_encoder: bool = True, arithmetic: str = "fp16x2", outputs: str = "all", **kwargs):
        super().__init__()
        self.arithmetic = arithmetic
        self.outputs = check_outputs(outputs)
        self.iters, self.fnet_dim, self.hidden_dim, self.context_dim = iters, fnet_dim, hidden_dim, context_dim
        self.corr_levels, self.corr_radius = corr_levels, corr_radius
        self.tracing, self.include_preprocessing = tracing, include_preprocessing
        self.fused_loop = fused_loop
        self.hip_encoder = hip_encoder
        self._enc_cache = ops.ParamCache()
        self.fnet = BasicEncoder(output_dim=fnet_dim)
        self.cnet_proj = nn.Sequential(nn.Conv2d(fnet_dim, context_dim + hidden_dim, 3, padding=1), nn.ReLU(False))
        self.update_block = BasicUpdateBlock(hidden_dim=hidden_dim, cor_planes=corr_levels * (2 * corr_radius + 1),
                                             flow_channel=1, context_dim=context_dim, spatial_scale=8, arithmetic=arithmetic)
        self.corr_fn = CorrBlock1D
        self.weights, self.strict_load = weights, strict_load
        if weights is not None:
            load_weights(self, weights, strict_load)

    def convex_upsample(self, flow, mask, rate=8):
        return convex_upsample(flow, mask, rate)

    def initialize_coords(self, fmap1):
        B, _, H, W = fmap1.shape
        return torch.arange(W, device=fmap1.device).float()[None, None, None, :].repeat(B, 1, H, 1)

    def _encoder_engine(self, device) -> "ops.EncoderEngine":
        def build():
            eng = ops.EncoderEngine(self.fnet_dim, self.fnet.norm_fn, self.context_dim + self.hidden_dim, self.arithmetic)
            return eng.load(self.fnet.state_dict(), self.cnet_proj.state_dict(), eps=1e-5, device=device)
        return self._enc_cache.get((self.fnet, self.cnet_proj), device, build)

    def _calibration_sites(self):
        sites = {}
        if self.hip_encoder and hip_encoder_blocker(self.fnet, ("batch", "none")) is None:
            sites["fnet"] = self._encoder_site(self._enc_cache, self.fnet_dim, self.context_dim + self.hidden_dim)
        sites.update(super()._calibration_sites())
        return sites

    def forward_fnet(self, frame1, frame2):
        if self.hip_encoder:
            why = hip_encoder_blocker(self.fnet, ("batch", "none"))
            if why:
                raise NndError(f"BaseRAFTStereo: the HIP encoder cannot run this fnet ({why}); pass hip_encoder=False to run "
                               "the encoder's PyTorch-ROCm modules explicitly")
            B = frame1.shape[0]
            fmaps, cnet = self._encoder_engine(frame1.device).forward(frame1.float(), n_cnet=B, frames_b=frame2.float())
            return fmaps[:B], fmaps[B:], cnet
        fmap1, fmap2 = self.fnet([frame1, frame2])
        return fmap1, fmap2, self.cnet_proj(fmap1)

    def forward(self, frame1: torch.Tensor, frame2: torch.Tensor, **kwargs) -> List[Dict[str, torch.Tensor]]:
        require_eval(self)
        with torch.no_grad():
            return self._forward_calibrated(frame1, frame2)

    def _forward(self, frame1: torch.Tensor, frame2: torch.Tensor) -> List[Dict[str, torch.Tensor]]:
        fmap1, fmap2, cnet = self.forward_fnet(frame1, frame2)
        rate = frame1.shape[-1] // fmap1.shape[-1]
        fmap1, fmap2 = fmap1.float(), fmap2.float()
        net, inp = ops.split_tanh_relu(cnet.float(), self.hidden_dim)
        corr = self.corr_fn(fmap1, fmap2, self.corr_levels, self.corr_radius)
        last = last_only(self)
        if self.fused_loop and isinstance(corr, CorrBlock1D):
            eng = self.update_block.sync_engine(frame1.device)
            up, _, _ = eng.refine(corr._pyr, self.corr_levels, self.corr_radius, net.float(), inp.float(),
                                  rate, self.iters, keep_all=not last, last_only=last)
            return [{"up_disp": up[i]} for i in range(up.shape[0])]
        coords1 = self.initialize_coords(fmap1)
        org = self.initialize_coords(fmap1)
        outs = []
        for i in range(self.iters):
            sampled = corr(coords1)
            net, mask, delta = self.update_block(net, inp, sampled, coords1 - org)
            coords1 = coords1 + delta
            if not last or i == self.iters - 1:
                outs.append({"up_disp": self.convex_upsample(coords1 - org, mask, rate=rate)})
        return outs


def frame_size_outputs(ups, frame_hw, stacked=None):
    h, w = ups[0].shape[-2:]
    rate = frame_hw[1] / w
    if rate == 1:
        return list(ups)
    if frame_hw[0] % h or frame_hw[1] % w or os.environ.get("NND_C2F_TORCH_RESIZE", "0") not in ("", "0"):
        return [nn.functional.interpolate(u, size=frame_hw) * rate for u in ups]
    if stacked is None:
        return [ops.resize_nearest_scaled(u, frame_hw, rate) for u in ups]
    big = ops.resize_nearest_scaled(stacked, frame_hw, rate)
    return [big[i] for i in range(big.shape[0])]


class Coarse2FineRAFTStereoBase(AutoCalibrate, nn.Module):

    def __init__(self, iters: int = 12, hidden_dim: int = 128, context_dim: int = 128, corr_levels: int = 1, corr_radius: int = 4,
                 num_groups: int = 4, weights: Optional[str] = None, strict_load: bool = True, fused_loop: bool = True,
                 arithmetic: str = "fp16x2", outputs: str = "all", **kwargs):
        super().__init__()
        assert corr_levels == 1, "Corr level must be 1 in Coarse2FineGroupRepViTRaftStereo"
        self.arithmetic = arithmetic
        self.outputs = check_outputs(outputs)
        self.iters, self.hidden_dim, self.context_dim = iters, hidden_dim, context_dim
        self.corr_levels, self.corr_radius, self.num_groups = corr_levels, corr_radius, num_groups
        self.fused_loop = fused_loop
        self.fnet = self._init_fnet()
        self.cnet_proj = self._init_cnet_proj()
        self.fusion_blocks = self._init_fusion_blocks()
        self.update_block = BasicUpdateBlock(hidden_dim=hidden_dim, cor_planes=num_groups * corr_levels * (2 * corr_radius + 1),
                                             flow_channel=1, context_dim=context_dim, gru="conv_gru", spatial_scale=(4, 4),
                                             arithmetic=arithmetic)
        self.corr_fn = GroupCorrBlock1D
        self.weights, self.strict_load = weights, strict_load
        if weights is not None:
            load_weights(self, weights, strict_load)

    def _init_fnet(self) -> nn.Module:
        raise NotImplementedError("Coarse2FineRAFTStereoBase: supply the encoder (reference: nndepth.encoders.rep_vit.RepViT)")

    def _init_cnet_proj(self) -> nn.ModuleList:
        raise NotImplementedError("Coarse2FineRAFTStereoBase: supply cnet_proj (reference: three 1x1 MobileOneBlocks, model.py:216-222)")

    def _init_fusion_blocks(self) -> nn.ModuleList:
        raise NotImplementedError("Coarse2FineRAFTStereoBase: supply fusion_blocks (reference: two FeatureFusionBlocks, model.py:223-228)")

    def convex_upsample(self, flow, mask, rate=(4, 4)):
        rate = rate if isinstance(rate, int) else rate[0]
        return convex_upsample(flow, mask, rate)

    def initialize_coords(self, fmap1):
        B, _, H, W = fmap1.shape
        return torch.arange(W, device=fmap1.device).float()[None, None, None, :].repeat(B, 1, H, 1)

    def forward_features(self, frame1: torch.Tensor, frame2: torch.Tensor):
        B = frame1.shape[0]
        features = self.fnet(torch.cat([frame1, frame2], dim=0))[::2][::-1]
        feats, cnets, previous = [], [], None
        for idx, feat in enumerate(features):
            if previous is not None:
                feat = self.fusion_blocks[idx - 1]([previous, feat])
            feats.append(feat)
            cnets.append(self.cnet_proj[idx](feat[:B].clone()))
            previous = feat
        return feats, cnets

    def forward(self, frame1: torch.Tensor, frame2: torch.Tensor, **kwargs) -> List[Dict[str, torch.Tensor]]:
        require_eval(self)
        with torch.no_grad():
            return self._forward_calibrated(frame1, frame2)

    def _forward(self, frame1: torch.Tensor, frame2: torch.Tensor) -> List[Dict[str, torch.Tensor]]:
        feats, cnets = self.forward_features(frame1, frame2)
        return self.refine_stages(feats, cnets, tuple(frame1.shape[-2:]))

    def refine_stages(self, feats, cnets, frame_hw) -> List[Dict[str, torch.Tensor]]:
        B = feats[0].shape[0] // 2
        last = last_only(self)
        outs: List[Dict[str, torch.Tensor]] = []
        up_last = None
        for idx, feat in enumerate(feats):
            fmap1, fmap2 = feat[:B].float().contiguous(), feat[B:].float().contiguous()
            cnet = cnets[idx].float()
            net, inp = ops.split_tanh_relu(cnet, cnet.shape[1] // 2)
            corr = self.corr_fn(fmap1, fmap2, self.corr_levels, self.corr_radius, self.num_groups)
            if up_last is not None and tuple(up_last.shape[-2:]) != tuple(fmap1.shape[-2:]):
                raise NndError(f"Coarse2FineRAFTStereoBase: stage {idx} is {tuple(fmap1.shape[-2:])} but the previous stage's "
                               f"upsampled disparity is {tuple(up_last.shape[-2:])} (frame size not divisible by the pyramid's strides)")
            if self.fused_loop and isinstance(corr, GroupCorrBlock1D):
                eng = self.update_block.sync_engine(fmap1.device)
                up, _, _ = eng.refine_group(corr._pyr, self.num_groups, self.corr_levels, self.corr_radius, net, inp, 4, self.iters,
                                            disp_init=up_last, keep_all=not last, last_only=last)
                ups, stacked = [up[i] for i in range(up.shape[0])], up
            else:
                org = self.initialize_coords(fmap1)
                coords1 = org if up_last is None else org + up_last
                ups, stacked = [], None
                for i in range(self.iters):
                    sampled = corr(coords1)
                    net, mask, delta = self.update_block(net, inp, sampled, coords1 - org)
                    coords1 = coords1 + delta
                    if not last or i == self.iters - 1:
                        ups.append(self.convex_upsample(coords1 - org, mask, rate=(4, 4)))
            if not last or idx == len(feats) - 1:
                outs.extend({"up_disp": u} for u in frame_size_outputs(ups, tuple(frame_hw), stacked))
            up_last = ups[-1]
        return outs


class FoldedEncoderSide:

    def __init__(self, engine_cls, track_modules: bool = False):
        self.engine_cls, self.track_modules, self.cache = engine_cls, track_modules, ops.ParamCache()

    def run(self, owner: nn.Module, modules, frame1: torch.Tensor, frame2: torch.Tensor):
        if owner.training or modules[0].training:
            raise NndError(f"{type(owner).__name__}: the HIP encoder side is inference-only (BatchNorm is folded with its running "
                           "statistics): call model.eval() first")

        def build():
            why = self.engine_cls.blocker(owner, *modules)
            if why:
                raise NndError(f"{type(owner).__name__}: the HIP encoder side cannot run this model ({why}); pass hip_encoder=False "
                               "to run the encoder side's PyTorch-ROCm modules explicitly")
            return self.engine_cls.from_modules(*modules, frame1.device)
        engine = self.cache.get(modules, frame1.device, build, track_modules=self.track_modules)
        return engine.forward(frame1.float(), frame2.float())


class Coarse2FineGroupRepViTRAFTStereo(Coarse2FineRAFTStereoBase):

    def __init__(self, num_groups: int = 4, downsample_ratios=((2, 2), (2, 2), (2, 2), (2, 2)), ffn_exp_ratios=(1.0, 3.0, 3.0, 4.0),
                 num_blocks_per_stage=(4, 4, 6, 2), patch_size: int = 7, stem_strides=((2, 2), (2, 2), (1, 1)),
                 token_mixer_types=("repmixer", "repmixer", "repmixer", "attention"), use_ffn_per_stage=(False, True, True, True),
                 width_multipliers=(1, 1, 1, 1), weights: Optional[str] = None, strict_load: bool = True, iters: int = 12,
                 fnet_dim: int = 256, hidden_dim: int = 128, context_dim: int = 128, corr_levels: int = 1, corr_radius: int = 4,
                 tracing: bool = False, include_preprocessing: bool = False, hip_encoder: bool = True, arithmetic: str = "fp16x2",
                 outputs: str = "all", fused_loop: bool = True, **kwargs):
        self.downsample_ratios, self.ffn_exp_ratios = downsample_ratios, ffn_exp_ratios
        self.num_blocks_per_stage, self.patch_size, self.stem_strides = num_blocks_per_stage, patch_size, stem_strides
        self.token_mixer_types, self.use_ffn_per_stage, self.width_multipliers = token_mixer_types, use_ffn_per_stage, width_multipliers
        self.fnet_dim, self.tracing, self.include_preprocessing = fnet_dim, tracing, include_preprocessing
# ... 78 lines not shown
```

Baseline: 155.5 pairs/s.

## Build loop state directly from cnet and merge context-term conv pair launches

Adds a refine entry point that takes the raw context tensor and builds the hidden state, context input, coords and flow in one kernel. This replaces the separate split_tanh_relu pass and the later copies into tiled layout. It also merges the two context-term convolutions (zr and q), which share an input, into one paired conv_split launch via a PAIR template that picks weights per grid row. The Python fused path now passes cnet and skips allocating the low-res and net_out state buffers. The cost is extra kernel instantiations and stricter eligibility checks that fall back to separate launches.

```diff
diff --git a/include/nndepth_amd.h b/include/nndepth_amd.h
--- a/include/nndepth_amd.h
+++ b/include/nndepth_amd.h
@@ -363,6 +363,11 @@
                            const float* net, const float* inp, const float* disp_init,
                            float* up_out, int64_t up_iter_stride, float* low_out, float* net_out,
                            float* workspace, int B, int H, int W, int rate, int iters, void* stream);
+int nnd_raft_stereo_refine_from_cnet(const nnd_update_block_desc* desc, const float* packed_dev,
+                                     const float* pyramid, int num_levels, int radius,
+                                     const float* cnet, int cnet_channels, const float* disp_init,
+                                     float* up_out, int64_t up_iter_stride, float* low_out, float* net_out,
+                                     float* workspace, int B, int H, int W, int rate, int iters, void* stream);
 int nnd_raft_stereo_group_refine(const nnd_update_block_desc* desc, const float* packed_dev, const float* group_pyramid, int num_groups,
                                  int num_levels, int radius, const float* net, const float* inp, const float* disp_init, float* up_out,
                                  int64_t up_iter_stride, float* low_out, float* net_out, float* workspace, int B, int H, int W, int rate,
diff --git a/nndepth_amd/_lib.py b/nndepth_amd/_lib.py
--- a/nndepth_amd/_lib.py
+++ b/nndepth_amd/_lib.py
@@ -135,6 +135,8 @@
     "nnd_mask_upsample_forward": (_I, [_P, _P, _P, _P, _I, _I, _I, _I, _I, _P]),
     "nnd_raft_stereo_refine": (_I, [C.POINTER(UpdateBlockDesc), _P, _P, _I, _I, _P, _P, _P, _P, C.c_int64, _P, _P, _P,
                                     _I, _I, _I, _I, _I, _P]),
+    "nnd_raft_stereo_refine_from_cnet": (_I, [C.POINTER(UpdateBlockDesc), _P, _P, _I, _I, _P, _I, _P, _P, C.c_int64, _P, _P, _P,
+                                              _I, _I, _I, _I, _I, _P]),
     "nnd_raft_stereo_group_refine": (_I, [C.POINTER(UpdateBlockDesc), _P, _P, _I, _I, _I, _P, _P, _P, _P, C.c_int64, _P, _P, _P,
                                           _I, _I, _I, _I, _I, _P]),
     "nnd_igev_interleaved_floats": (C.c_int64, [_I, _I, _I, _I, _I]),
diff --git a/nndepth_amd/csrc/cascade.hip b/nndepth_amd/csrc/cascade.hip
--- a/nndepth_amd/csrc/cascade.hip
+++ b/nndepth_amd/csrc/cascade.hip
@@ -14,6 +14,43 @@
     const float v = x[idx];
     if (rem < (long)Cn * HW) net[b * Cn * HW + rem] = tanhf_(v);
     else inp[b * Ci * HW + (rem - (long)Cn * HW)] = relu_nan(v);
+}
+
+__global__ void __launch_bounds__(256) loop_state_from_cnet_kernel(const float* __restrict__ cnet, float* __restrict__ hx, long hx_bs,
+                                                                   float* __restrict__ hx_flow, int hx_pm, float* __restrict__ coords,
+                                                                   float* __restrict__ flow, const float* __restrict__ disp_init, int hid,
+                                                                   int ctx, int H, int W, int absolute, long total, Lay lh, Lay lp) {
+    const long idx = (long)blockIdx.x * 256 + threadIdx.x;
+    if (idx >= total) return;
+    const long HW = (long)H * W;
+    const int G = (hid + ctx) >> 2;
+    const long pix = idx % HW, rest = idx / HW;
+    const int g = (int)(rest % (G + 1));
+    const long b = rest / (G + 1);
+    const int y = (int)(pix / W), x = (int)(pix - (long)y * W);
+    if (g == G) {
+        const long po = pix_off(lp, y, x);
+        const float c = (float)x + (disp_init ? disp_init[b * HW + pix] : 0.f);
+        const float f = absolute ? c : c - (float)x;
+        coords[b * lp.plane + po] = c;
+        flow[b * lp.plane + po] = f;
+        hx_flow[b * hx_bs + po * hx_pm] = f;
+        return;
+    }
+    const float* src = cnet + (b * (hid + ctx) + 4 * g) * HW + pix;
+    float v[4];
+#pragma unroll
+    for (int j = 0; j < 4; ++j) v[j] = src[j * HW];
+    const bool is_net = 4 * g < hid;
+#pragma unroll
+    for (int j = 0; j < 4; ++j) v[j] = is_net ? tanhf_(v[j]) : relu_nan(v[j]);
+    float* dst = hx + b * hx_bs + chan_off(lh, 4 * g) + pix_off(lh, y, x);
+    if (lh.ci == 4) {
+        *reinterpret_cast<float4*>(dst) = make_float4(v[0], v[1], v[2], v[3]);
+    } else {
+#pragma unroll
+        for (int j = 0; j < 4; ++j) dst[j * lh.plane] = v[j];
+    }
 }
 
 __global__ void __launch_bounds__(256) avg_pool_2x_4x_kernel(const float* __restrict__ x, float* __restrict__ o2, float* __restrict__ o4,
@@ -95,6 +132,26 @@
     else dst[0] = v[0];
 }
 
+int split_tanh_relu_launch(const float* x, float* net, float* inp, int B, int Cnet, int Cinp, int H, int W, hipStream_t stream) {
+    const long total = (long)B * (Cnet + Cinp) * H * W;
+    hipLaunchKernelGGL(split_tanh_relu_kernel, dim3((unsigned)cdiv64(total, 256)), dim3(256), 0, stream, x, net, inp, Cnet, Cinp,
+                       (long)H * W, total);
+    NND_LAUNCH_CHECK();
+    return NND_OK;
+}
+
+int loop_state_from_cnet_launch(const float* cnet, float* hx, int64_t hx_bs, bool hx_c4, float* hx_flow, float* coords, float* flow,
+                                const float* disp_init, int B, int hid, int ctx, int H, int W, bool absolute, hipStream_t stream) {
+    NND_REQUIRE(hid % 4 == 0 && ctx % 4 == 0, "loop state: hidden_dim %d and context_dim %d must be multiples of 4", hid, ctx);
+    const long total = (long)B * ((hid + ctx) / 4 + 1) * H * W;
+    NND_REQUIRE(cdiv64(total, 256) < (1L << 31), "loop state: grid of %ld workgroups too large", (long)cdiv64(total, 256));
+    hipLaunchKernelGGL(loop_state_from_cnet_kernel, dim3((unsigned)cdiv64(total, 256)), dim3(256), 0, stream, cnet, hx, (long)hx_bs, hx_flow,
+                       hx_c4 ? 4 : 1, coords, flow, disp_init, hid, ctx, H, W, absolute ? 1 : 0, total, make_lay(H, W, true, hx_c4),
+                       make_lay(H, W, true));
+    NND_LAUNCH_CHECK();
+    return NND_OK;
+}
+
 }
 
 using namespace nnd;
@@ -103,11 +160,7 @@
 
 int nnd_split_tanh_relu(const float* x, float* net, float* inp, int B, int Cnet, int Cinp, int H, int W, void* stream) {
     NND_REQUIRE(x && net && inp && B > 0 && Cnet > 0 && Cinp > 0 && H > 0 && W > 0, "split_tanh_relu: bad argument");
-    const long total = (long)B * (Cnet + Cinp) * H * W;
-    hipLaunchKernelGGL(split_tanh_relu_kernel, dim3((unsigned)cdiv64(total, 256)), dim3(256), 0, (hipStream_t)stream, x, net, inp, Cnet,
-                       Cinp, (long)H * W, total);
-    NND_LAUNCH_CHECK();
-    return NND_OK;
+    return split_tanh_relu_launch(x, net, inp, B, Cnet, Cinp, H, W, (hipStream_t)stream);
 }
 
 int nnd_avg_pool_2x_4x(const float* x, float* out2, float* out4, int N, int C, int H, int W, void* stream) {
diff --git a/nndepth_amd/csrc/common.h b/nndepth_amd/csrc/common.h
--- a/nndepth_amd/csrc/common.h
+++ b/nndepth_amd/csrc/common.h
@@ -65,6 +65,8 @@
     bool no_slab3d;
     int slab3d_rounds;
     bool no_fused_enc_block;
+    bool no_merged_ctx_terms;
+    bool no_loop_state_kernel;
 };
 const Switches& switches();
 
@@ -104,6 +106,10 @@
 
 int to_tiled(const float* src, float* dst, int64_t dbs, int B, int C, int H, int W, hipStream_t s, int c0 = 0, bool c4 = false);
 int from_tiled(const float* src, int64_t sbs, float* dst, int B, int C, int H, int W, hipStream_t s, int c0 = 0, bool c4 = false);
+
+int split_tanh_relu_launch(const float* x, float* net, float* inp, int B, int Cnet, int Cinp, int H, int W, hipStream_t stream);
+int loop_state_from_cnet_launch(const float* cnet, float* hx, int64_t hx_bs, bool hx_c4, float* hx_flow, float* coords, float* flow,
+                                const float* disp_init, int B, int hid, int ctx, int H, int W, bool absolute, hipStream_t stream);
 
 static inline int cdiv(int a, int b) { return (a + b - 1) / b; }
 static inline int64_t cdiv64(int64_t a, int64_t b) { return (a + b - 1) / b; }
@@ -174,6 +180,8 @@
 bool conv_split_supported(int KH, int KW, int Cin, int stride, int arith, int Cout = 0);
 int launch_conv_split(const ConvLayer& L, const float* blob, const ConvIO& io, int epi, int B, int H, int W, hipStream_t stream);
 bool conv_split_no_split_k(const ConvLayer& L, int B, int H, int W);
+int launch_conv_split_pair(const ConvLayer& L0, const ConvLayer& L1, const float* blob, const ConvIO& io0, const ConvIO& io1, int epi, int B,
+                           int H, int W, hipStream_t stream, bool* merged);
 bool flow_branch_supported(const ConvLayer& f2, int fc);
 int launch_flow_branch(const ConvLayer& f2, const float* blob, const float* w7t, const float* b7, const float* flow, int64_t fbs,
                        int fc, const ConvIO& io, int B, int H, int W, hipStream_t stream);
diff --git a/nndepth_amd/csrc/conv_split.hip b/nndepth_amd/csrc/conv_split.hip
--- a/nndepth_amd/csrc/conv_split.hip
+++ b/nndepth_amd/csrc/conv_split.hip
@@ -184,6 +184,56 @@
     return NND_OK;
 }
 
+extern template int launch_split_pair_ns<1>(const ConvArgs&, const ConvSecond&, dim3, const SplitCfg&, int, int, hipStream_t);
+extern template int launch_split_pair_ns<2>(const ConvArgs&, const ConvSecond&, dim3, const SplitCfg&, int, int, hipStream_t);
+extern template int launch_split_pair_ns<3>(const ConvArgs&, const ConvSecond&, dim3, const SplitCfg&, int, int, hipStream_t);
+
+int launch_conv_split_pair(const ConvLayer& L0, const ConvLayer& L1, const float* blob, const ConvIO& io0, const ConvIO& io1, int epi, int B,
+                           int H, int W, hipStream_t stream, bool* merged) {
+    *merged = false;
+    if (switches().no_merged_ctx_terms || calibrating()) return NND_OK;
+    if (L0.arith == 0 || L0.arith != L1.arith || L0.KH != L1.KH || L0.KW != L1.KW || L0.Cin != L1.Cin || L0.stride != 1 || L1.stride != 1 ||
+        L0.CI_T != 16 || L1.CI_T != 16 || L0.nchunks != L1.nchunks || L0.s_off >= 0 || L1.s_off >= 0)
+        return NND_OK;
+    if (!conv_split_supported(L0.KH, L0.KW, L0.Cin, 1, L0.arith, L0.Cout) || epi == EPI_AFFINE) return NND_OK;
+    for (const ConvIO* io : {&io0, &io1})
+        if (io->src1.C != 0 || io->out1.ptr || io->aux0.ptr || io->aux1.ptr || io->bmap.ptr || io->cout_need > 0 || io->force_ks > 0 ||
+            io->Hin > 0 || io->Win > 0)
+            return NND_OK;
+    if (io0.src0.ptr != io1.src0.ptr || io0.src0.bstride != io1.src0.bstride || io0.src0.C != io1.src0.C || io0.src_tiled != io1.src_tiled ||
+        io0.src_c4 != io1.src_c4 || io0.dst_tiled != io1.dst_tiled || io0.dst_c4 != io1.dst_c4 || io0.scale != io1.scale ||
+        io0.hidden != io1.hidden || io0.flags != io1.flags)
+        return NND_OK;
+    int rc, Hin, Win;
+    NND_TRY(conv_check_io("conv_split", L0, io0, epi, H, W, &Hin, &Win));
+    NND_TRY(conv_check_io("conv_split", L1, io1, epi, H, W, &Hin, &Win));
+    NND_REQUIRE((long)(L0.Cin + 64) * tiled_plane(Hin, Win) < (1L << 31), "conv_split: plane offsets exceed 32 bits");
+    SplitCfg c0, c1;
+    if (!plan_split(L0, io0, B, H, W, &c0) || !plan_split(L1, io1, B, H, W, &c1)) return NND_OK;
+    if (c0.wco != c1.wco || c0.ks != 1 || c1.ks != 1 || c0.P != c1.P || c0.nu != c1.nu || c0.fast != c1.fast || c0.lds != c1.lds ||
+        c0.ntiles != c1.ntiles || c0.grid.x != c1.grid.x || c0.block.x != c1.block.x || !split_pair_built(L0.KH, L0.KW, c0, io0.src_c4))
+        return NND_OK;
+    ConvArgs a, a1;
+    conv_fill_args(L0, blob, io0, epi, H, W, Hin, Win, &a);
+    conv_fill_args(L1, blob, io1, epi, H, W, Hin, Win, &a1);
+    a.tiles_x = c0.tiles_x; a.wco = c0.wco; a.ks = 1; a.npos = c0.ntiles;
+    const ConvSecond s2{a1.wpk, a1.bias, a1.out0, a1.obs0, a1.Cout, c0.ny};
+    const dim3 grid(c0.grid.x, c0.ny + c1.ny, B);
+    if (switches().conv_verbose) {
+        print_split_plan(L0, io0, c0);
+        print_split_plan(L1, io1, c1);
+        fprintf(stderr, "[nnd] ctx_terms_merged %dx%d Cin=%d Cout=%d+%d pieces=%d: one launch, grid %ux%ux%u (rows %d+%d)\n", L0.KH, L0.KW, L0.Cin,
+                L0.Cout, L1.Cout, L0.arith, grid.x, grid.y, grid.z, c0.ny, c1.ny);
+    }
+    rc = L0.arith == 3   ? launch_split_pair_ns<3>(a, s2, grid, c0, L0.KH, L0.KW, stream)
+         : L0.arith == 2 ? launch_split_pair_ns<2>(a, s2, grid, c0, L0.KH, L0.KW, stream)
+                         : launch_split_pair_ns<1>(a, s2, grid, c0, L0.KH, L0.KW, stream);
+    if (rc != NND_OK) return rc;
+    NND_LAUNCH_CHECK();
+    *merged = true;
+    return NND_OK;
+}
+
 void pack_conv_split(const ConvLayer& L, int nparts, const float* const* w, const float* const* bvec, const int* cout, float* blob,
                      const int* ci_map, int cin_src) {
     if (!ci_map) cin_src = L.Cin;
diff --git a/nndepth_amd/csrc/conv_split_kernel.h b/nndepth_amd/csrc/conv_split_kernel.h
--- a/nndepth_amd/csrc/conv_split_kernel.h
+++ b/nndepth_amd/csrc/conv_split_kernel.h
@@ -98,8 +98,29 @@
     static constexpr bool ON = NT >= 5 && P == 2;
 };
 
-template <int KH, int KW, int NS, int P, int NU, bool FAST, bool SRC4, int AD_, int MAXT, int STR = 1>
-__global__ void __launch_bounds__(MAXT) conv_split_kernel(ConvArgs a) {
+struct ConvSecond {
+    const float* wpk;
+    const float* bias;
+    float* out0;
+    long obs0;
+    int Cout;
+    int ny0;
+};
+struct ConvNoSecond {};
+
+template <int KH, int KW, int NS, int P, int NU, bool FAST, bool SRC4, int AD_, int MAXT, int STR = 1, bool PAIR = false>
+__global__ void __launch_bounds__(MAXT) conv_split_kernel(ConvArgs a, std::conditional_t<PAIR, ConvSecond, ConvNoSecond> s2) {
+    int by = blockIdx.y;
+    if constexpr (PAIR) {
+        if (by >= s2.ny0) {
+            by -= s2.ny0;
+            a.wpk = s2.wpk;
+            a.bias = s2.bias;
+            a.out0 = s2.out0;
+            a.obs0 = s2.obs0;
+            a.Cout = s2.Cout;
+        }
+    }
     static_assert(STR == 1 || (FAST && (KH * KW == 9 || KH * KW == 1)), "stride 2: 3x3 / 1x1, FAST regime");
     using Geo = SplitGeom<KH, KW, NS, STR>;
     constexpr int NT = KH * KW, PH = KH / 2, PW = KW / 2;
@@ -119,7 +140,7 @@
     const int cbi = wave % wco, kj = wave / wco;
     const int h2 = lane >> 5, l31 = lane & 31;
     const int pxl = lane_pixel(l31), r = pxl >> 3, c = pxl & 7;
-    const int cb = blockIdx.y * wco + cbi;
+    const int cb = by * wco + cbi;
     const bool active = cb * 32 < a.Cout;
     const int b = blockIdx.z;
     const int Hin = a.Hin, Win = a.Win;
@@ -579,7 +600,7 @@
 
 template <int KH, int KW, int NS, int P, int NU, bool FAST, bool SRC4, int AD, int MAXT, int STR = 1>
 int launch_split_kernel(const ConvArgs& a, dim3 grid, dim3 block, size_t lds, hipStream_t stream) {
-    auto kern = conv_split_kernel<KH, KW, NS, P, NU, FAST, SRC4, AD, MAXT, STR>;
+    auto kern = conv_split_kernel<KH, KW, NS, P, NU, FAST, SRC4, AD, MAXT, STR, false>;
     if ((int)block.x > MAXT) {
         set_error("conv_split: %u threads exceed the %d-thread bound of this instantiation", block.x, MAXT);
         return NND_ERR_INVALID;
@@ -589,7 +610,7 @@
         static std::atomic<unsigned> raised{0};
         if (int rc = raise_lds_limit(reinterpret_cast<const void*>(kern), raised)) return rc;
     }
-    hipLaunchKernelGGL(kern, grid, block, lds, stream, a);
+    hipLaunchKernelGGL(kern, grid, block, lds, stream, a, ConvNoSecond{});
     return NND_OK;
 }
 
@@ -624,6 +645,34 @@
     return src4 ? launch_split_nu<KH, KW, NS, true, true, 1>(a, cfg, stream) : launch_split_nu<KH, KW, NS, true, false, 1>(a, cfg, stream);
 }
 
+inline bool split_pair_built(int KH, int KW, const SplitCfg& cfg, bool src4) {
+    return ((KH == 1 && KW == 5) || (KH == 5 && KW == 1) || (KH == 3 && KW == 3)) && cfg.stride == 1 && cfg.fast && src4 && cfg.P == 2 &&
+           split_nu_variant(cfg.nu) == 2 && cfg.ks == 1;
+}
+template <int KH, int KW, int NS>
+int launch_split_pair_shape(const ConvArgs& a, const ConvSecond& s2, dim3 grid, const SplitCfg& cfg, hipStream_t stream) {
+    constexpr int AD = split_fast_ad<KH, KW, NS>();
+    auto kern = conv_split_kernel<KH, KW, NS, 2, 2, true, true, AD, 768, 1, true>;
+    if ((int)cfg.block.x > 768) {
+        set_error("conv_split: %u threads exceed the 768-thread bound of this instantiation", cfg.block.x);
+        return NND_ERR_INVALID;
+    }
+    const size_t lds = cfg.lds + switches().lds_slack;
+    if (lds > 64 * 1024) {
+        static std::atomic<unsigned> raised{0};
+        if (int rc = raise_lds_limit(reinterpret_cast<const void*>(kern), raised)) return rc;
+    }
+    hipLaunchKernelGGL(kern, grid, cfg.block, lds, stream, a, s2);
+    return NND_OK;
+}
+template <int NS>
+int launch_split_pair_ns(const ConvArgs& a, const ConvSecond& s2, dim3 grid, const SplitCfg& cfg, int KH, int KW, hipStream_t stream) {
+    if (!split_pair_built(KH, KW, cfg, a.ls.ci == 4)) return NND_ERR_UNSUPPORTED;
+    if (KH == 1 && KW == 5) return launch_split_pair_shape<1, 5, NS>(a, s2, grid, cfg, stream);
+    if (KH == 5 && KW == 1) return launch_split_pair_shape<5, 1, NS>(a, s2, grid, cfg, stream);
+    return launch_split_pair_shape<3, 3, NS>(a, s2, grid, cfg, stream);
+}
+
 template <int NS>
 int launch_split_ns(const ConvArgs& a, const SplitCfg& cfg, int KH, int KW, hipStream_t stream) {
     if (KH == 3 && KW == 3) return launch_split_shape<3, 3, NS>(a, cfg, stream);
diff --git a/nndepth_amd/csrc/conv_split_ns1.hip b/nndepth_amd/csrc/conv_split_ns1.hip
--- a/nndepth_amd/csrc/conv_split_ns1.hip
+++ b/nndepth_amd/csrc/conv_split_ns1.hip
@@ -2,6 +2,7 @@
 
 namespace nnd {
 template int launch_split_ns<1>(const ConvArgs&, const SplitCfg&, int, int, hipStream_t);
+template int launch_split_pair_ns<1>(const ConvArgs&, const ConvSecond&, dim3, const SplitCfg&, int, int, hipStream_t);
 #ifdef NND_DBG_STAMPS
 extern "C" int nnd_debug_read_split_stamps_ns1(unsigned long long* host, int n) {
     return hipMemcpyFromSymbol(host, HIP_SYMBOL(g_split_stamps), sizeof(unsigned long long) * n) == hipSuccess ? 0 : -1;
diff --git a/nndepth_amd/csrc/conv_split_ns2.hip b/nndepth_amd/csrc/conv_split_ns2.hip
--- a/nndepth_amd/csrc/conv_split_ns2.hip
+++ b/nndepth_amd/csrc/conv_split_ns2.hip
@@ -2,6 +2,7 @@
 
 namespace nnd {
 template int launch_split_ns<2>(const ConvArgs&, const SplitCfg&, int, int, hipStream_t);
+template int launch_split_pair_ns<2>(const ConvArgs&, const ConvSecond&, dim3, const SplitCfg&, int, int, hipStream_t);
 #ifdef NND_DBG_STAMPS
 extern "C" int nnd_debug_read_split_stamps_ns2(unsigned long long* host, int n) {
     return hipMemcpyFromSymbol(host, HIP_SYMBOL(g_split_stamps), sizeof(unsigned long long) * n) == hipSuccess ? 0 : -1;
diff --git a/nndepth_amd/csrc/conv_split_ns3.hip b/nndepth_amd/csrc/conv_split_ns3.hip
--- a/nndepth_amd/csrc/conv_split_ns3.hip
+++ b/nndepth_amd/csrc/conv_split_ns3.hip
@@ -2,6 +2,7 @@
 
 namespace nnd {
 template int launch_split_ns<3>(const ConvArgs&, const SplitCfg&, int, int, hipStream_t);
+template int launch_split_pair_ns<3>(const ConvArgs&, const ConvSecond&, dim3, const SplitCfg&, int, int, hipStream_t);
 #ifdef NND_DBG_STAMPS
 extern "C" int nnd_debug_read_split_stamps_ns3(unsigned long long* host, int n) {
     return hipMemcpyFromSymbol(host, HIP_SYMBOL(g_split_stamps), sizeof(unsigned long long) * n) == hipSuccess ? 0 : -1;
diff --git a/nndepth_amd/csrc/error.cpp b/nndepth_amd/csrc/error.cpp
--- a/nndepth_amd/csrc/error.cpp
+++ b/nndepth_amd/csrc/error.cpp
@@ -44,6 +44,8 @@
     s.no_slab3d = on("NND_NO_SLAB3D");
     s.slab3d_rounds = getenv("NND_SLAB3D_ROUNDS") ? atoi(getenv("NND_SLAB3D_ROUNDS")) : 0;
     s.no_fused_enc_block = on("NND_NO_FUSED_ENC_BLOCK");
+    s.no_merged_ctx_terms = on("NND_NO_MERGED_CTX_TERMS");
+    s.no_loop_state_kernel = on("NND_NO_LOOP_STATE_KERNEL");
     g_sw = s;
 }
 namespace {
diff --git a/nndepth_amd/csrc/update_block.hip b/nndepth_amd/csrc/update_block.hip
--- a/nndepth_amd/csrc/update_block.hip
+++ b/nndepth_amd/csrc/update_block.hip
@@ -706,7 +706,8 @@
                           int radius, const float* net, const float* inp, const float* disp_init, float* up_out,
                           int64_t up_iter_stride, float* low_out, float* net_out, float* workspace, int B, int H, int W,
                           int rate, int iters, void* stream, const float* geo_pyramid = nullptr, int groups = 1,
-                          const CreArgs* cre = nullptr, const float* interleaved = nullptr, int flat_groups = 0) {
+                          const CreArgs* cre = nullptr, const float* interleaved = nullptr, int flat_groups = 0,
+                          const float* cnet = nullptr) {
     Plan p;
     int rc = make_plan(desc, &p);
     if (rc != NND_OK) return rc;
@@ -714,7 +715,8 @@
     NND_REQUIRE(!last_flag || up_iter_stride == 0,
                 "refine: NND_FLAG_LAST_UPSAMPLE_ONLY writes one upsampled map, so up_iter_stride must be 0 (got %lld)", (long long)up_iter_stride);
     const bool last_only = last_flag && !(p.d.flags & NND_FLAG_CALIBRATE);
-    NND_REQUIRE(packed && (pyramid || cre) && net && inp && up_out && workspace, "refine: null pointer");
+    NND_REQUIRE(packed && (pyramid || cre) && ((net && inp) || cnet) && up_out && workspace, "refine: null pointer");
+    NND_REQUIRE(!cnet || (!net && !inp && !cre), "refine: the context tensor replaces net and inp (RAFT-Stereo / IGEV state only)");
     const bool igev = geo_pyramid != nullptr;
     const int fc = p.d.flow_channels;
     if (cre) {
@@ -739,11 +741,25 @@
     const int hid = p.d.hidden_dim, ctx = p.d.context_dim, hxC = 2 * hid + ctx;
     const Lay lay = make_lay(H, W, true);
     const int64_t n = lay.plane;
-    NND_TRY(to_tiled(net, w.hx, hxC * n, B, hid, H, W, s, 0, ws_c4()));
-    NND_TRY(to_tiled(inp, w.hx, hxC * n, B, ctx, H, W, s, hid, ws_c4()));
     float* hx_flow = w.hx + ws_chan(hxC - fc, n);
     const unsigned eg = (unsigned)cdiv64((int64_t)B * H * W, 256);
-    if (cre) {
+    const bool state_kernel = cnet && !switches().no_loop_state_kernel;
+    if (state_kernel) {
+        NND_TRY(loop_state_from_cnet_launch(cnet, w.hx, hxC * n, ws_c4(), hx_flow, w.coords, w.flow, disp_init, B, hid, ctx, H, W, igev, s));
+        if (switches().conv_verbose) fprintf(stderr, "[nnd] loop_state_from_cnet: hid=%d ctx=%d %dx%dx%d, one launch\n", hid, ctx, B, H, W);
+        NND_TRY(debug_sync("loop state from cnet", s));
+    } else if (cnet) {
+        NND_REQUIRE(hid <= 256 && ctx <= 256, "refine: NND_NO_LOOP_STATE_KERNEL needs hidden_dim and context_dim <= 256");
+        NND_TRY(split_tanh_relu_launch(cnet, w.c1, w.cf, B, hid, ctx, H, W, s));
+        net = w.c1;
+        inp = w.cf;
+    }
+    if (!state_kernel) {
+        NND_TRY(to_tiled(net, w.hx, hxC * n, B, hid, H, W, s, 0, ws_c4()));
+        NND_TRY(to_tiled(inp, w.hx, hxC * n, B, ctx, H, W, s, hid, ws_c4()));
+    }
+    if (state_kernel) {
+    } else if (cre) {
         if (disp_init) {
             NND_TRY(to_tiled(disp_init, w.flow, fc * n, B, fc, H, W, s));
             NND_TRY(to_tiled(disp_init, w.hx, hxC * n, B, fc, H, W, s, hxC - fc, ws_c4()));
@@ -775,8 +791,21 @@
         if (flat_groups > 0) return group_lookup_flat_launch(pyramid, w.coords, w.corr, B, flat_groups, H, W, num_levels, radius, st_, true);
         return corr1d_lookup_launch(pyramid, w.coords, w.corr, B, H, W, num_levels, radius, st_, true);
     };
-    for (int id : {(int)C_ZR1C, (int)C_Q1C, (int)C_ZR2C, (int)C_Q2C})
-        if (p.sep || id < C_ZR2C) NND_TRY(run_conv(p, packed, w, id, c, nullptr, nullptr, B, H, W, s));
+    for (int zr : {(int)C_ZR1C, (int)C_ZR2C}) {
+        if (!p.sep && zr == C_ZR2C) break;
+        const int q = zr + 1;
+        bool merged = false;
+        if (p.L[zr].arith != 0)
+            NND_TRY(launch_conv_split_pair(p.L[zr], p.L[q], packed, conv_io(p, w, zr, c, n, nullptr, nullptr), conv_io(p, w, q, c, n, nullptr, nullptr),
+                                           EPI_LINEAR, B, H, W, s, &merged));
+        if (merged) {
+            NND_TRY(debug_sync(kConvNames[zr], s));
+            NND_TRY(debug_sync(kConvNames[q], s));
+            continue;
+        }
+        NND_TRY(run_conv(p, packed, w, zr, c, nullptr, nullptr, B, H, W, s));
+        NND_TRY(run_conv(p, packed, w, q, c, nullptr, nullptr, B, H, W, s));
+    }
     const bool no_fuse_up = switches().no_fused_upsample;
     const bool no_fuse_lk = switches().no_fused_lookup;
     const bool fused_up = !no_fuse_up && mask_upsample_supported(rate, 2 * hid, fc);
@@ -966,6 +995,18 @@
                           net_out, workspace, B, H, W, rate, iters, stream);
 }
 
+int nnd_raft_stereo_refine_from_cnet(const nnd_update_block_desc* desc, const float* packed, const float* pyramid, int num_levels,
+                                     int radius, const float* cnet, int cnet_channels, const float* disp_init, float* up_out,
+                                     int64_t up_iter_stride, float* low_out, float* net_out, float* workspace, int B, int H, int W,
+                                     int rate, int iters, void* stream) {
+    NND_REQUIRE(desc && cnet, "raft_stereo_refine_from_cnet: null pointer");
+    NND_REQUIRE(cnet_channels == desc->hidden_dim + desc->context_dim,
+                "raft_stereo_refine_from_cnet: the context tensor has %d channels, the update block takes hidden_dim + context_dim = %d + %d",
+                cnet_channels, desc->hidden_dim, desc->context_dim);
+    return enqueue_refine(desc, packed, pyramid, num_levels, radius, nullptr, nullptr, disp_init, up_out, up_iter_stride, low_out, net_out,
+                          workspace, B, H, W, rate, iters, stream, nullptr, 1, nullptr, nullptr, 0, cnet);
+}
+
 int nnd_raft_stereo_group_refine(const nnd_update_block_desc* desc, const float* packed, const float* group_pyramid, int num_groups,
                                  int num_levels, int radius, const float* net, const float* inp, const float* disp_init, float* up_out,
                                  int64_t up_iter_stride, float* low_out, float* net_out, float* workspace, int B, int H, int W, int rate,
diff --git a/nndepth_amd/ops.py b/nndepth_amd/ops.py
--- a/nndepth_amd/ops.py
+++ b/nndepth_amd/ops.py
@@ -431,17 +431,18 @@
 class _RefineCall(NamedTuple):
     desc: UpdateBlockDesc
     d: torch.device
-    net: torch.Tensor
-    inp: torch.Tensor
+    net: Optional[torch.Tensor]
+    inp: Optional[torch.Tensor]
     init: Optional[torch.Tensor]
     up: torch.Tensor
     stride: int
-    low: torch.Tensor
-    net_out: torch.Tensor
+    low: Optional[torch.Tensor]
+    net_out: Optional[torch.Tensor]
     ws: torch.Tensor
     B: int
     H: int
     W: int
+    cnet: Optional[torch.Tensor] = None
 
 
 class UpdateBlockEngine(ScaleSlots):
@@ -554,30 +555,54 @@
         return net_out, mask, delta
 
     def _refine_call(self, what: str, tensors, net, inp, init, channels: int, rate: int, iters: int,
-                     keep_all: Optional[bool], last_only: bool) -> "_RefineCall":
+                     keep_all: Optional[bool], last_only: bool, cnet=None, want_state: bool = True) -> "_RefineCall":
         if self.packed is None:
             raise NndError("UpdateBlockEngine: parameters not loaded")
         keep_all = self._keep_all(keep_all, last_only)
         desc = _call_desc(self, NND_FLAG_LAST_UPSAMPLE_ONLY if last_only else 0)
-        d = _dev(*tensors, net, inp, self.packed)
-        net, inp = net.contiguous(), inp.contiguous()
-        B, _, H, W = net.shape
-        self._check_state(what, net, inp, init, channels)
+        ds = self.desc
+        if cnet is not None:
+            if net is not None or inp is not None:
+                raise NndError(f"{what}: pass either cnet or net and inp, not both")
+            if cnet.dim() != 4 or cnet.shape[1] != ds.hidden_dim + ds.context_dim:
+                raise NndError(f"{what}: cnet shape {tuple(cnet.shape)} != (B, hidden_dim + context_dim = "
+                               f"{ds.hidden_dim} + {ds.context_dim}, H, W)")
+            if cnet.dtype != torch.float32:
+                raise NndError(f"{what}: cnet must be float32, got {cnet.dtype}")
+            d = _dev(*tensors, cnet, self.packed)
+            cnet = cnet.contiguous()
+            B, _, H, W = cnet.shape
+            if init is not None and tuple(init.shape) != (B, channels, H, W):
+                raise NndError(f"{what}: initial disparity / flow shape {tuple(init.shape)} != {(B, channels, H, W)}")
+        else:
+            if net is None or inp is None:
+                raise NndError(f"{what}: net and inp (or cnet) are required")
+            d = _dev(*tensors, net, inp, self.packed)
+            net, inp = net.contiguous(), inp.contiguous()
+            B, _, H, W = net.shape
+            self._check_state(what, net, inp, init, channels)
         if init is not None:
             _dev(init)
             init = init.contiguous()
         up = torch.empty((iters if keep_all else 1, B, channels, rate * H, rate * W), dtype=torch.float32, device=d)
-        low = torch.empty((B, channels, H, W), dtype=torch.float32, device=d)
-        return _RefineCall(desc, d, net, inp, init, up, up[0].numel() if keep_all else 0, low, torch.empty_like(net),
-                           self.workspace(B, H, W, d), B, H, W)
+        low = torch.empty((B, channels, H, W), dtype=torch.float32, device=d) if want_state else None
+        net_out = torch.empty((B, ds.hidden_dim, H, W), dtype=torch.float32, device=d) if want_state else None
+        return _RefineCall(desc, d, net, inp, init, up, up[0].numel() if keep_all else 0, low, net_out,
+                           self.workspace(B, H, W, d), B, H, W, cnet)
 
     def refine(self, pyr, num_levels: int, radius: int, net, inp, rate: int, iters: int,
-               disp_init=None, keep_all: Optional[bool] = None, last_only: bool = False):
-        c = self._refine_call("refine", (pyr,), net, inp, disp_init, 1, rate, iters, keep_all, last_only)
+               disp_init=None, keep_all: Optional[bool] = None, last_only: bool = False, cnet=None, want_state: bool = True):
+        c = self._refine_call("refine", (pyr,), net, inp, disp_init, 1, rate, iters, keep_all, last_only, cnet, want_state)
         B, H, W = c.B, c.H, c.W
         if pyr.numel() != pyramid_layout(B, H, W, num_levels)[2]:
             raise NndError(f"refine: pyramid holds {pyr.numel()} floats, a {B}x{H}x{W} pyramid of {num_levels} levels has "
                            f"{pyramid_layout(B, H, W, num_levels)[2]}")
+        if c.cnet is not None:
+            with torch.cuda.device(c.d):
+                check(lib.nnd_raft_stereo_refine_from_cnet(C.byref(c.desc), _p(self.packed), _p(pyr), num_levels, radius, _p(c.cnet),
+                                                           int(c.cnet.shape[1]), _p(c.init), _p(c.up), c.stride, _p(c.low), _p(c.net_out),
+                                                           _p(c.ws), B, H, W, rate, iters, _stream(c.d)), "raft_stereo_refine_from_cnet")
+            return c.up, c.low, c.net_out
         with torch.cuda.device(c.d):
             check(lib.nnd_raft_stereo_refine(C.byref(c.desc), _p(self.packed), _p(pyr), num_levels, radius,
                                              _p(c.net), _p(c.inp), _p(c.init), _p(c.up), c.stride, _p(c.low), _p(c.net_out),
diff --git a/nndepth_amd/raft_stereo.py b/nndepth_amd/raft_stereo.py
--- a/nndepth_amd/raft_stereo.py
+++ b/nndepth_amd/raft_stereo.py
@@ -325,14 +325,14 @@
         fmap1, fmap2, cnet = self.forward_fnet(frame1, frame2)
         rate = frame1.shape[-1] // fmap1.shape[-1]
         fmap1, fmap2 = fmap1.float(), fmap2.float()
-        net, inp = ops.split_tanh_relu(cnet.float(), self.hidden_dim)
         corr = self.corr_fn(fmap1, fmap2, self.corr_levels, self.corr_radius)
         last = last_only(self)
         if self.fused_loop and isinstance(corr, CorrBlock1D):
             eng = self.update_block.sync_engine(frame1.device)
-            up, _, _ = eng.refine(corr._pyr, self.corr_levels, self.corr_radius, net.float(), inp.float(),
-                                  rate, self.iters, keep_all=not last, last_only=last)
+            up, _, _ = eng.refine(corr._pyr, self.corr_levels, self.corr_radius, None, None, rate, self.iters,
+                                  keep_all=not last, last_only=last, cnet=cnet.float(), want_state=False)
             return [{"up_disp": up[i]} for i in range(up.shape[0])]
+        net, inp = ops.split_tanh_relu(cnet.float(), self.hidden_dim)
         coords1 = self.initialize_coords(fmap1)
         org = self.initialize_coords(fmap1)
         outs = []
```

Result: no change. 156.6 pairs/s, median of 6 (+0.7%).
